# nv-tlabs/GEN3C

Hardware: AMD Instinct MI355X
Metric: denoise-steps/sec (121x1280x704 latent, Cosmos-7B) (higher is better)
Workload: dtype bf16

## Files before the change

### gen3c_amd/_lib.py

```python
from __future__ import annotations

import ctypes as C
from pathlib import Path

_LIB_PATH = Path(__file__).resolve().parent / "lib" / "libgen3c_hip.so"
_lib = None

vp, i64, i32, f32 = C.c_void_p, C.c_int64, C.c_int, C.c_float

G3_OK, G3_ERR_ARG, G3_ERR_LAUNCH, G3_ERR_RESOURCE = 0, 1, 2, 3

SIGNATURES = {
    "g3_last_error": [],
    "g3_abi_version": [],
    "g3_set_option": [C.c_char_p, i32],
    "g3_device_info": [i32, C.POINTER(i32), C.POINTER(i32), C.c_char_p, i32],
    "g3_event_create": [C.POINTER(vp)],
    "g3_event_record": [vp, vp],
    "g3_event_elapsed_ms": [vp, vp, C.POINTER(f32)],
    "g3_event_destroy": [vp],
    "g3_gemm_bf16_nt": [vp, i64, vp, i64, vp, i64, i32, i32, i32, i32, vp, i32, i64, vp, i64, vp],
    "g3_flash_attn_fwd_kvseg_bf16": [vp, i64, i64, i64, vp, i64, i64, i64, vp, i64, i64, i64, i32, i64, vp, i64, i64, i64, i32, i32, i32,
                                     i32, i32, f32, vp],
    "g3_gemm_kernel_name": [i32, i32, i32, i32],
    "g3_quant_mxfp8_bf16": [vp, i64, vp, i64, vp, i64, i32, i32, vp],
    "g3_gemm_mxfp8_nt": [vp, i64, vp, i64, vp, i64, vp, i64, vp, i64, i32, i32, i32, i32, vp, i32, i64, vp, i64, vp],
    "g3_gemm_mxfp8_kernel_name": [i32, i32, i32, i32],
    "g3_gemv_bf16": [vp, i64, vp, i64, vp, i64, vp, i64, i32, i32, i32, i32, vp],
    "g3_flash_attn_kernel_name": [i32, i32, i32, i32],
    "g3_flash_attn_fwd_bf16": [vp, i64, i64, i64, vp, i64, i64, i64, vp, i64, i64, i64, vp, i64, i64, i64, i32, i32, i32,
                               i32, i32, f32, vp],
    "g3_cross_attn_fwd_bf16": [vp, i64, i64, i64, vp, f32, vp, i64, i64, i64, vp, i64, i64, i64, vp, i64, i64, i64, i32, i32, i32, i32, i32,
                               i32, f32, vp],
    "g3_flash_attn_fwd_ex_bf16": [vp, i64, i64, i64, vp, i64, i64, i64, vp, i64, i64, i64, i32, i64, vp, vp, vp, i64, i64, i64, i32, i32, i32,
                                  i32, i32, f32, i32, vp],
    "g3_flash_attn_fwd_carry_bf16": [vp, i64, i64, i64, vp, i64, i64, i64, vp, i64, i64, i64, i32, i64, i32, i32, vp, vp, vp, vp, vp, i64, i64,
                                     i64, i32, i32, i32, i32, i32, f32, i32, vp],
    "g3_flash_attn_kernel_name_ex": [i32, i32, i32, i32, i32],
    "g3_attn_merge_partials_bf16": [vp, vp, i32, i64, i64, i64, vp, i64, i64, i64, i32, i32, i32, i32, vp],
    "g3_transpose_v_bf16": [vp, i64, vp, i64, i32, i32, i32, i32, vp],
    "g3_layernorm_modulate_bf16": [vp, i64, vp, vp, i64, i32, vp, i64, i32, i32, f32, vp],
    "g3_posemb_layernorm_modulate_bf16": [vp, i64, vp, vp, vp, vp, i32, i32, i32, i32, vp, vp, i64, i32, vp, i64, i32, f32, vp],
    "g3_qk_rmsnorm_rope_bf16": [vp, i64, vp, vp, vp, vp, i64, i32, i32, i32, i32, f32, vp],
    "g3_qk_rmsnorm_rope_pair_bf16": [vp, i64, vp, i32, vp, i32, vp, vp, vp, i64, i32, i32, i32, f32, vp],
    "g3_gemm_qk_norm_rope_bf16": [vp, i64, vp, i64, vp, i64, i32, i32, i32, i32, i32, vp, vp, vp, vp, i32, f32, vp, i64, vp],
    "g3_add_inplace_bf16": [vp, vp, i64, vp],
    "g3_warp_project_f32": [vp, vp, vp, vp, vp, vp, vp, vp, vp, i32, i32, i32, i32, vp],
    "g3_warp_splat_f32": [vp, vp, vp, vp, vp, vp, i32, i32, i32, i32, vp],
    "g3_warp_resolve_f32": [vp, vp, vp, vp, i32, i32, i32, vp],
    "g3_warp_windows_workspace_bytes": [i32, i32, i32],
    "g3_warp_splat_resolve_f32": [vp, vp, vp, vp, vp, vp, vp, vp, vp, vp, i32, i32, i32, i32, vp],
    "g3_render_workspace_bytes": [i32, i32, i32, i32],
    "g3_render_workspace_init": [vp, i32, i32, i32, i32, vp],
    "g3_render_items_f32": [vp, vp, vp, vp, vp, vp, vp, vp, vp, vp, vp, vp, vp, i32, i32, i32, i32, i32, vp],
    "g3_mesh_occlusion_f32": [vp, vp, vp, vp, vp, vp, vp, vp, vp, vp, i32, i32, i32, i32, vp],
    "g3_unproject_points_f32": [vp, vp, vp, vp, i32, i32, i32, vp],
    "g3_dit_patchify_bf16": [vp, vp, vp, i32, vp, i32, i32, i32, i32, i32, i32, vp],
    "g3_dit_unpatchify_bf16": [vp, i64, vp, i32, i32, i32, i32, i32, i32, i32, vp],
    "g3_timestep_embedding_bf16": [vp, vp, vp, vp, i32, i32, vp],
    "g3_reliable_depth_mask_f32": [vp, vp, i32, i32, i32, i32, f32, f32, vp],
    "g3_align_depth_workspace_bytes": [i32, i32],
    "g3_align_depth_f32": [vp, vp, vp, vp, vp, i32, i32, f32, f32, vp, vp, C.c_size_t, i32, i32, vp],
    "g3_conv3d_cl_bf16": [vp, i64, vp, i64, vp, vp, i64, vp, i64] + [i32] * 17 + [vp],
    "g3_conv3d_cl_gnstats_bf16": [vp, i64, vp, i64, vp, vp, i64, vp, i64] + [i32] * 17 + [vp, i32, vp],
    "g3_groupnorm_stats_cl_bf16": [vp, i64, vp, i32, i32, i32, vp],
    "g3_groupnorm_apply_cl_bf16": [vp, i64, vp, vp, vp, vp, i64, i32, i32, i32, f32, i32, vp],
    "g3_groupnorm_swish_cl_bf16": [vp, i64, vp, vp, vp, vp, i64, i32, i32, i32, f32, i32, vp],
    "g3_haar3d_patch_bf16": [vp, vp, i32, i32, i32, vp],
    "g3_haar3d_unpatch_bf16": [vp, i64, vp, i32, i32, i32, vp],
    "g3_resample_cl_bf16": [vp, vp, i32, i32, i32, i32, i32, vp],
    "g3_softmax_rows_bf16": [vp, i64, i32, i32, f32, vp],
    "g3_transpose2d_bf16": [vp, i64, vp, i64, i32, i32, vp],
    "g3_temporal_attn_cl_bf16": [vp, vp, vp, vp, i32, i32, i32, f32, vp],
    "g3_spatial_attn_d512_bf16": [vp, vp, vp, i64, i64, vp, i32, i32, f32, vp],
    "g3_edm_prepare_input_bf16": [vp, vp, vp, vp, vp, vp, i64, i32, i32, f32, f32, f32, f32, vp],
    "g3_edm_cfg_euler_step_bf16": [vp, vp, vp, vp, vp, vp, i64, i32, i32, f32, f32, f32, f32, f32, f32, f32, vp],
}
_RESTYPES = {"g3_last_error": C.c_char_p, "g3_flash_attn_kernel_name": C.c_char_p, "g3_gemm_kernel_name": C.c_char_p, "g3_gemm_mxfp8_kernel_name": C.c_char_p, "g3_flash_attn_kernel_name_ex": C.c_char_p, "g3_align_depth_workspace_bytes": C.c_size_t,
             "g3_warp_windows_workspace_bytes": C.c_size_t, "g3_render_workspace_bytes": C.c_size_t}


class Gen3cHipError(RuntimeError):
    pass


def lib_path() -> Path:
    return _LIB_PATH


def load():
    global _lib
    if _lib is not None:
        return _lib
    import torch
    if not _LIB_PATH.exists():
        raise Gen3cHipError(
            f"{_LIB_PATH} is missing: build it with `python -m gen3c_amd.build` (or __graft_entry__.build()). "
            "gen3c_amd has no CPU/PyTorch fallback for its HIP kernels."
        )
    lib = C.CDLL(str(_LIB_PATH))
    for name, argtypes in SIGNATURES.items():
        fn = getattr(lib, name)
        fn.argtypes = argtypes
        fn.restype = _RESTYPES.get(name, C.c_int)
    _lib = lib
    return lib


def last_error() -> str:
    msg = load().g3_last_error()
    return msg.decode() if msg else "?"


def check(rc: int, what: str = ""):
    if rc != 0:
        msg = load().g3_last_error()
# ... 2 lines not shown
```

### gen3c_amd/csrc/api.hip

```cpp
#include "common.hpp"
#include <stdarg.h>
#include <stdio.h>
#include <stdlib.h>
#include <string.h>

namespace {
thread_local char g_err[512] = "";
}

int g3_set_error(int code, const char* fmt, ...) {
    va_list ap;
    va_start(ap, fmt);
    vsnprintf(g_err, sizeof(g_err), fmt, ap);
    va_end(ap);
    return code;
}

int g3_check_launch(const char* what) {
    hipError_t e = hipGetLastError();
    if (e != hipSuccess) return g3_set_error(G3_ERR_LAUNCH, "%s: launch failed: %s", what, hipGetErrorString(e));
    return G3_OK;
}

static int env_int(const char* name, int dflt) {
    const char* e = getenv(name);
    return (e && *e) ? atoi(e) : dflt;
}
int g3_opt_gemm_regstage = env_int("G3_GEMM_REGSTAGE", 0);
int g3_opt_attn_xcd_heads = env_int("G3_ATTN_XCD_HEADS", 1);
int g3_opt_attn_variant = env_int("G3_ATTN_VARIANT", 0);
int g3_opt_gemm_rowmajor_tiles = env_int("G3_GEMM_ROWMAJOR_TILES", 0);
int g3_opt_gemm_wide_store = env_int("G3_GEMM_WIDE_STORE", 1);
int g3_opt_splat_tiled = env_int("G3_SPLAT_TILED", 1);
int g3_opt_render_overlap = env_int("G3_RENDER_OVERLAP", 1);
int g3_opt_render_exclusive = env_int("G3_RENDER_EXCLUSIVE", 0);
int g3_opt_render_full_extent = env_int("G3_RENDER_FULL_EXTENT", 1);
int g3_opt_render_fused = env_int("G3_RENDER_FUSED", 1);
int g3_opt_gemm_pingpong = env_int("G3_GEMM_PINGPONG", 3);
int g3_opt_tok_tattn_px = env_int("G3_TOK_TATTN_PX", 1);
int g3_opt_gemm_persistent = env_int("G3_GEMM_PERSISTENT", 0);
int g3_opt_gemm_deferred = env_int("G3_GEMM_DEFERRED", 1);
int g3_opt_gemm_deferred_grid = env_int("G3_GEMM_DEFERRED_GRID", 0);
int g3_opt_gemm_tokens_first = env_int("G3_GEMM_TOKENS_FIRST", 2);
int g3_opt_conv_w4 = env_int("G3_CONV_W4", 1);
int g3_opt_ln_wave_rows = env_int("G3_LN_WAVE_ROWS", 0);
int g3_opt_norm_octets = env_int("G3_NORM_OCTETS", 1);
int g3_opt_gemm_unpinned = env_int("G3_GEMM_UNPINNED", 1);

extern "C" int g3_set_option(const char* name, int value) {
    if (!name) return g3_set_error(G3_ERR_ARG, "g3_set_option: null name");
    if (!strcmp(name, "gemm_regstage")) { g3_opt_gemm_regstage = value; return G3_OK; }
    if (!strcmp(name, "gemm_wide_store")) { g3_opt_gemm_wide_store = value; return G3_OK; }
    if (!strcmp(name, "splat_tiled")) { g3_opt_splat_tiled = value; return G3_OK; }
    if (!strcmp(name, "render_overlap")) { g3_opt_render_overlap = value; return G3_OK; }
    if (!strcmp(name, "render_fused")) { g3_opt_render_fused = value; return G3_OK; }
    if (!strcmp(name, "render_exclusive")) { g3_opt_render_exclusive = value; return G3_OK; }
    if (!strcmp(name, "render_full_extent")) { g3_opt_render_full_extent = value; return G3_OK; }
    if (!strcmp(name, "gemm_pingpong")) { g3_opt_gemm_pingpong = value; return G3_OK; }
    if (!strcmp(name, "gemm_unpinned")) { g3_opt_gemm_unpinned = value; return G3_OK; }
    if (!strcmp(name, "conv_w4")) { g3_opt_conv_w4 = value; return G3_OK; }
    if (!strcmp(name, "gemm_persistent")) { g3_opt_gemm_persistent = value; return G3_OK; }
    if (!strcmp(name, "gemm_deferred")) { g3_opt_gemm_deferred = value; return G3_OK; }
    if (!strcmp(name, "gemm_tokens_first")) { g3_opt_gemm_tokens_first = value; return G3_OK; }
    if (!strcmp(name, "gemm_deferred_grid")) { g3_opt_gemm_deferred_grid = value; return G3_OK; }
    if (!strcmp(name, "tok_tattn_px")) { g3_opt_tok_tattn_px = value; return G3_OK; }
    if (!strcmp(name, "gemm_rowmajor_tiles")) { g3_opt_gemm_rowmajor_tiles = value; return G3_OK; }
    if (!strcmp(name, "ln_wave_rows")) { g3_opt_ln_wave_rows = value; return G3_OK; }
    if (!strcmp(name, "norm_octets")) { g3_opt_norm_octets = value; return G3_OK; }
    if (!strcmp(name, "attn_variant")) { g3_opt_attn_variant = value; return G3_OK; }
    if (!strcmp(name, "attn_xcd_heads")) { g3_opt_attn_xcd_heads = value; return G3_OK; }
    return g3_set_error(G3_ERR_ARG, "g3_set_option: unknown option %s", name);
}

extern "C" const char* g3_last_error(void) { return g_err; }
extern "C" int g3_abi_version(void) { return 1; }

extern "C" int g3_device_info(int device, int* cu_count, int* is_gfx950, char* arch_name, int arch_name_len) {
    hipDeviceProp_t prop;
    hipError_t e = hipGetDeviceProperties(&prop, device);
    if (e != hipSuccess) return g3_set_error(G3_ERR_LAUNCH, "g3_device_info: %s", hipGetErrorString(e));
    if (cu_count) *cu_count = prop.multiProcessorCount;
    if (is_gfx950) *is_gfx950 = (strncmp(prop.gcnArchName, "gfx950", 6) == 0) ? 1 : 0;
    if (arch_name && arch_name_len > 0) snprintf(arch_name, arch_name_len, "%s", prop.gcnArchName);
    return G3_OK;
}

extern "C" int g3_event_create(void** ev) {
    hipEvent_t e;
    hipError_t r = hipEventCreate(&e);
    if (r != hipSuccess) return g3_set_error(G3_ERR_LAUNCH, "g3_event_create: %s", hipGetErrorString(r));
    *ev = (void*)e;
    return G3_OK;
}
extern "C" int g3_event_record(void* ev, void* stream) {
    hipError_t r = hipEventRecord((hipEvent_t)ev, (hipStream_t)stream);
    if (r != hipSuccess) return g3_set_error(G3_ERR_LAUNCH, "g3_event_record: %s", hipGetErrorString(r));
    return G3_OK;
}
extern "C" int g3_event_elapsed_ms(void* start, void* stop, float* ms) {
    hipError_t r = hipEventSynchronize((hipEvent_t)stop);
    if (r == hipSuccess) r = hipEventElapsedTime(ms, (hipEvent_t)start, (hipEvent_t)stop);
    if (r != hipSuccess) return g3_set_error(G3_ERR_LAUNCH, "g3_event_elapsed_ms: %s", hipGetErrorString(r));
    return G3_OK;
}
extern "C" int g3_event_destroy(void* ev) {
    (void)hipEventDestroy((hipEvent_t)ev);
    return G3_OK;
}
```

### gen3c_amd/csrc/attention.hip

```cpp
#include "common.hpp"
#include <stdlib.h>
#include <mutex>
#include <type_traits>

namespace {

constexpr int HD = 128;
constexpr int QB = 32;
constexpr int NWAVES = 8;
constexpr int BQ = QB * NWAVES;
constexpr int KVB = 64;
constexpr int NTHREADS = 64 * NWAVES;

struct AttnParams {
    const bf16_t* Q; int64_t q_row, q_batch, q_head;
    const bf16_t* K; int64_t k_row, k_batch, k_head;
    const bf16_t* Vt; int64_t vt_row, vt_batch, vt_head;
    bf16_t* O; int64_t o_row, o_batch, o_head;
    int Sq, Skv;
    float scale_log2;
    int vt_seg_len;
    int64_t vt_seg_stride;
    int grid_q, n_hb, n_heads, xcd_heads;
    float* O32;
    float* LSE;
    int kv_dense;
    const bf16_t* q_norm_w;
    float q_norm_eps;
    const float* carry_o;
    const float* carry_lse;
    int kv_skip_begin, kv_skip_len;
    uint32_t kv_skip_vt_bytes;
};

G3_DEVICE int k_off(int row, int chunk) { return row * HD + ((chunk ^ (row & 15)) << 3); }
G3_DEVICE int v_off(int row, int chunk) { return row * KVB + ((chunk ^ ((row >> 1) & 7)) << 3); }
G3_DEVICE int swap23(int i) { return (i & ~12) | ((i & 4) << 1) | ((i & 8) >> 1); }

template <int CTX>
__global__ __launch_bounds__(NTHREADS, 2) void flash_attn_fwd_kernel(AttnParams p) {
    extern __shared__ __attribute__((aligned(16))) char smem_raw[];
    bf16_t* sK = reinterpret_cast<bf16_t*>(smem_raw);
    bf16_t* sV = sK + 2 * KVB * HD;

    const int tid = threadIdx.x;
    const int lane = tid & 63;
    const int wave = tid >> 6;
    const int l31 = lane & 31;
    const int g = lane >> 5;
    const int head = blockIdx.y;
    const int batch = blockIdx.z;

    const bf16_t* Qb = p.Q + batch * p.q_batch + head * p.q_head;
    const bf16_t* Kb = p.K + batch * p.k_batch + head * p.k_head;
    const bf16_t* Vb = p.Vt + batch * p.vt_batch + head * p.vt_head;
    bf16_t* Ob = p.O + batch * p.o_batch + head * p.o_head;

    const int q_idx = blockIdx.x * BQ + wave * QB + l31;
    const bool q_ok = q_idx < p.Sq;
    bf16x8 qf[8];
    {
        const bf16_t* qrow = Qb + (int64_t)(q_ok ? q_idx : 0) * p.q_row + 8 * g;
#pragma unroll
        for (int ks = 0; ks < 8; ++ks) qf[ks] = q_ok ? load_bf16x8(qrow + 16 * ks) : zero_bf16x8();
    }

    bf16x8 rk[2], rv[2];
    auto stage_load = [&](int kv0) {
#pragma unroll
        for (int i = 0; i < 2; ++i) {
            const int idx = tid + NTHREADS * i;
            {
                const int row = idx >> 4, chunk = idx & 15;
                const bool ok = (kv0 + row) < p.Skv;
                rk[i] = ok ? load_bf16x8(Kb + (int64_t)(kv0 + row) * p.k_row + chunk * 8) : zero_bf16x8();
            }
            {
                const int row = idx >> 3, chunk = idx & 7;
                const bool ok = (kv0 + chunk * 8) < p.Skv;
                rv[i] = ok ? load_bf16x8(Vb + (int64_t)row * p.vt_row + kv0 + chunk * 8) : zero_bf16x8();
            }
        }
    };
    auto stage_write = [&](int buf) {
        bf16_t* dK = sK + buf * KVB * HD;
        bf16_t* dV = sV + buf * HD * KVB;
#pragma unroll
        for (int i = 0; i < 2; ++i) {
            const int idx = tid + NTHREADS * i;
            store_bf16x8(dK + k_off(idx >> 4, idx & 15), rk[i]);
            store_bf16x8(dV + v_off(idx >> 3, idx & 7), rv[i]);
        }
    };

    f32x16 accO[4];
#pragma unroll
    for (int d = 0; d < 4; ++d)
#pragma unroll
        for (int r = 0; r < 16; ++r) accO[d][r] = 0.f;
    float m_run = -1e30f;
    float l_run = 0.f;

    const int krow_perm = swap23(l31);
    const int nt = (p.Skv + KVB - 1) / KVB;
    stage_load(0);
    stage_write(0);
    __syncthreads();

    for (int t = 0; t < nt; ++t) {
        const int buf = t & 1;
        const int kv0 = t * KVB;
// ... 19 lines not shown
            for (int mb = 0; mb < 2; ++mb)
#pragma unroll
                for (int r = 0; r < 16; ++r) {
                    const int kv = kv0 + 32 * mb + 16 * (r >> 3) + 8 * g + (r & 7);
                    if (kv >= p.Skv) accS[mb][r] = -INFINITY;
                }
        }

        float mx = accS[0][0];
#pragma unroll
        for (int r = 1; r < 16; ++r) mx = fmaxf(mx, accS[0][r]);
#pragma unroll
        for (int r = 0; r < 16; ++r) mx = fmaxf(mx, accS[1][r]);
        mx = fmaxf(mx, wave_xor_f32(mx, 32));
        const float m_new = fmaxf(m_run, mx * p.scale_log2);
        const float alpha = __builtin_amdgcn_exp2f(m_run - m_new);
        m_run = m_new;

        float psum = 0.f;
        bf16x8 pb[4];
#pragma unroll
        for (int mb = 0; mb < 2; ++mb)
#pragma unroll
            for (int r = 0; r < 16; ++r) {
                const float pv = __builtin_amdgcn_exp2f(__builtin_fmaf(accS[mb][r], p.scale_log2, -m_new));
                psum += pv;
                pb[2 * mb + (r >> 3)][r & 7] = f32_to_bf16(pv);
            }
        l_run = l_run * alpha + psum;
#pragma unroll
        for (int d = 0; d < 4; ++d)
#pragma unroll
            for (int r = 0; r < 16; ++r) accO[d][r] *= alpha;

#pragma unroll
        for (int s = 0; s < 4; ++s) {
#pragma unroll
            for (int d = 0; d < 4; ++d) {
                const bf16x8 vf = load_bf16x8(cV + v_off(32 * d + l31, 2 * s + g));
                accO[d] = __builtin_amdgcn_mfma_f32_32x32x16_bf16(vf, pb[s], accO[d], 0, 0, 0);
            }
        }

        if (t + 1 < nt) stage_write(buf ^ 1);
        __syncthreads();
    }

    const float l_tot = l_run + wave_xor_f32(l_run, 32);
    const float inv = 1.0f / l_tot;
    if (q_ok) {
        bf16_t* orow = Ob + (int64_t)q_idx * p.o_row;
#pragma unroll
        for (int d = 0; d < 4; ++d)
#pragma unroll
            for (int q4 = 0; q4 < 4; ++q4) {
                bf16x4 o;
#pragma unroll
                for (int e = 0; e < 4; ++e) o[e] = f32_to_bf16(accO[d][4 * q4 + e] * inv);
                *reinterpret_cast<bf16x4*>(orow + 32 * d + 8 * q4 + 4 * g) = o;
            }
    }
}


constexpr float RESCALE_THR = 8.0f;

G3_DEVICE float max3(float a, float b, float c) {
    float r;
    asm("v_max3_f32 %0, %1, %2, %3" : "=v"(r) : "v"(a), "v"(b), "v"(c));
    return r;
}
G3_DEVICE void swap_halves(float& a, float& b) {
    asm volatile("s_nop 1\n\tv_permlane32_swap_b32 %0, %1" : "+v"(a), "+v"(b));
}
G3_DEVICE float xor32_max(float x) {
    float a = x, b = x;
    swap_halves(a, b);
    return max3(a, b, b);
}
G3_DEVICE float xor32_sum(float x) {
    float a = x, b = x;
    swap_halves(a, b);
    return a + b;
}

template <int CTX>
__global__ __launch_bounds__(NTHREADS, 2) void flash_attn_fwd_v2_kernel(AttnParams p) {
    extern __shared__ __attribute__((aligned(16))) char smem_raw[];
    bf16_t* sK = reinterpret_cast<bf16_t*>(smem_raw);
    bf16_t* sV = sK + 2 * KVB * HD;

    const int tid = threadIdx.x;
    const int lane = tid & 63;
    const int wave = tid >> 6;
    const int l31 = lane & 31;
    const int g = lane >> 5;
    const int head = blockIdx.y;
    const int batch = blockIdx.z;

    const bf16_t* Qb = p.Q + batch * p.q_batch + head * p.q_head;
    const bf16_t* Kb = p.K + batch * p.k_batch + head * p.k_head;
    const bf16_t* Vb = p.Vt + batch * p.vt_batch + head * p.vt_head;
    bf16_t* Ob = p.O + batch * p.o_batch + head * p.o_head;

    const int q_idx = blockIdx.x * BQ + wave * QB + l31;
    const bool q_ok = q_idx < p.Sq;
    bf16x8 qf[8];
    {
        const bf16_t* qrow = Qb + (int64_t)(q_ok ? q_idx : 0) * p.q_row + 8 * g;
#pragma unroll
        for (int ks = 0; ks < 8; ++ks) qf[ks] = q_ok ? load_bf16x8(qrow + 16 * ks) : zero_bf16x8();
    }

    bf16x8 rk[2], rv[2];
    auto load_k = [&](int kv0) {
#pragma unroll
        for (int i = 0; i < 2; ++i) {
            const int idx = tid + NTHREADS * i;
            const int row = idx >> 4, chunk = idx & 15;
            rk[i] = (kv0 + row) < p.Skv ? load_bf16x8(Kb + (int64_t)(kv0 + row) * p.k_row + chunk * 8) : zero_bf16x8();
        }
    };
    auto load_v = [&](int kv0) {
#pragma unroll
        for (int i = 0; i < 2; ++i) {
            const int idx = tid + NTHREADS * i;
            const int row = idx >> 3, chunk = idx & 7;
            rv[i] = (kv0 + chunk * 8) < p.Skv ? load_bf16x8(Vb + (int64_t)row * p.vt_row + kv0 + chunk * 8) : zero_bf16x8();
        }
    };
    auto write_k = [&](int buf) {
        bf16_t* dK = sK + buf * KVB * HD;
#pragma unroll
        for (int i = 0; i < 2; ++i) {
            const int idx = tid + NTHREADS * i;
            store_bf16x8(dK + k_off(idx >> 4, idx & 15), rk[i]);
        }
    };
    auto write_v = [&](int buf) {
        bf16_t* dV = sV + buf * HD * KVB;
#pragma unroll
        for (int i = 0; i < 2; ++i) {
            const int idx = tid + NTHREADS * i;
            store_bf16x8(dV + v_off(idx >> 3, idx & 7), rv[i]);
        }
    };

    const int krow_perm = swap23(l31);
    int koff[8], voff[4];
#pragma unroll
    for (int ks = 0; ks < 8; ++ks) koff[ks] = k_off(krow_perm, 2 * ks + g);
#pragma unroll
    for (int s4 = 0; s4 < 4; ++s4) voff[s4] = v_off(l31, 2 * s4 + g);
    auto qk = [&](f32x16 (&S)[2], int kbuf) {
        const bf16_t* cK = sK + kbuf * KVB * HD;
#pragma unroll
        for (int mb = 0; mb < 2; ++mb) {
#pragma unroll
            for (int r = 0; r < 16; ++r) S[mb][r] = 0.f;
#pragma unroll
            for (int ks = 0; ks < 8; ++ks) {
                const bf16x8 kf = load_bf16x8(cK + 32 * mb * HD + koff[ks]);
                S[mb] = __builtin_amdgcn_mfma_f32_32x32x16_bf16(kf, qf[ks], S[mb], 0, 0, 0);
            }
        }
    };
// ... 87 lines not shown
            write_v(par ^ 1);
            __syncthreads();
        }
    };

    using True = std::integral_constant<bool, true>;
    using False = std::integral_constant<bool, false>;
    using P0 = std::integral_constant<int, 0>;
    using P1 = std::integral_constant<int, 1>;
    int t = 0;
    for (; t + 2 < nt; t += 2) {
        tile(SA, SB, t, True{}, P0{});
        tile(SB, SA, t + 1, True{}, P1{});
    }
    if (t + 1 < nt) {
        tile(SA, SB, t, True{}, P0{});
        tile(SB, SA, t + 1, False{}, P1{});
    } else {
        tile(SA, SB, t, False{}, P0{});
    }

    const float l_tot = xor32_sum(l_run);
    const float inv = 1.0f / l_tot;
    if (q_ok) {
        bf16_t* orow = Ob + (int64_t)q_idx * p.o_row;
#pragma unroll
        for (int d = 0; d < 4; ++d)
#pragma unroll
            for (int q4 = 0; q4 < 4; ++q4) {
                bf16x4 o;
#pragma unroll
                for (int e = 0; e < 4; ++e) o[e] = f32_to_bf16(accO[d][4 * q4 + e] * inv);
                *reinterpret_cast<bf16x4*>(orow + 32 * d + 8 * q4 + 4 * g) = o;
            }
    }
}


template <int OFF> G3_DEVICE void lds_read_frag(bf16x8& dst, uint32_t addr) {
    static_assert(OFF >= 0 && OFF < 65536, "ds_read offset field is 16 bits");
    asm volatile("ds_read_b128 %0, %1 offset:%2" : "=v"(dst) : "v"(addr), "n"(OFF));
}
G3_DEVICE uint32_t lds_addr_flip128(uint32_t a) {
    uint32_t r;
    asm volatile("v_xor_b32 %0, 0x80, %1" : "=v"(r) : "v"(a));
    return r;
}
template <int N> G3_DEVICE void lds_wait_frag(bf16x8& frag) { asm volatile("s_waitcnt lgkmcnt(%1)" : "+v"(frag) : "n"(N)); }

#define G3_SGB(mask, n) __builtin_amdgcn_sched_group_barrier((mask), (n), 0)
constexpr int SGB_VALU = 0x2, SGB_MFMA = 0x8, SGB_DSR = 0x100, SGB_TRANS = 0x400;

#ifndef G3_AB_ATTN_ABLATE
#define G3_AB_ATTN_ABLATE 0
#endif
template <int CTX, int QA, int QBV, bool FOLD, bool MW = false, int MW_RD = 4, int MW_KREGS = 8>
__global__ __launch_bounds__(NTHREADS, 2) void flash_attn_fwd_v3_kernel(AttnParams p) {
    constexpr bool CP = (CTX & 2) != 0;
    extern __shared__ __attribute__((aligned(16))) char smem_raw[];
    bf16_t* sK = reinterpret_cast<bf16_t*>(smem_raw);
    bf16_t* sV = sK + 2 * KVB * HD;

    const int tid = threadIdx.x;
    const int lane = tid & 63;
    const int wave = tid >> 6;
    const int l31 = lane & 31;
    const int g = lane >> 5;
    const int Skv = p.kv_dense > 0 ? p.kv_dense : p.Skv;
    const int head = blockIdx.y;
    const int batch = blockIdx.z;

    const bf16_t* Qb = p.Q + batch * p.q_batch + head * p.q_head;
    const bf16_t* Kb = p.K + batch * p.k_batch + head * p.k_head;
    const bf16_t* Vb = p.Vt + batch * p.vt_batch + head * p.vt_head;
    bf16_t* Ob = p.O + batch * p.o_batch + head * p.o_head;

    const int q_idx = blockIdx.x * BQ + wave * QB + l31;
    const bool q_ok = q_idx < p.Sq;
    bf16x8 qf[8];
    {
        const bf16_t* qrow = Qb + (int64_t)(q_ok ? q_idx : 0) * p.q_row + 8 * g;
#pragma unroll
        for (int ks = 0; ks < 8; ++ks) qf[ks] = q_ok ? load_bf16x8(qrow + 16 * ks) : zero_bf16x8();
        if (p.q_norm_w) {
            float ss = 0.f;
#pragma unroll
            for (int ks = 0; ks < 8; ++ks)
#pragma unroll
                for (int e = 0; e < 8; ++e) { const float f = (float)qf[ks][e]; ss += f * f; }
            ss = xor32_sum(ss);
            const float rinv = rsqrtf(ss * (1.0f / 128.0f) + p.q_norm_eps);
#pragma unroll
            for (int ks = 0; ks < 8; ++ks) {
                const bf16x8 w8 = load_bf16x8(p.q_norm_w + 16 * ks + 8 * g);
#pragma unroll
                for (int e = 0; e < 8; ++e) qf[ks][e] = f32_to_bf16((float)qf[ks][e] * rinv * (float)w8[e]);
            }
        }
        if (FOLD) {
#pragma unroll
            for (int ks = 0; ks < 8; ++ks)
#pragma unroll
                for (int e = 0; e < 8; ++e) qf[ks][e] = f32_to_bf16((float)qf[ks][e] * p.scale_log2);
        }
    }

    const int k_row0 = tid >> 4, k_src_chunk = (tid & 15) ^ (k_row0 & 15);
    const int v_row0 = tid >> 3, v_src_chunk = (tid & 7) ^ ((v_row0 >> 1) & 7);
    const char* Kbytes = reinterpret_cast<const char*>(Kb);
    const char* Vbytes = reinterpret_cast<const char*>(Vb);
    const uint32_t k_row_bytes = (uint32_t)p.k_row * 2u;
    const uint32_t k_lane = (uint32_t)k_row0 * k_row_bytes + (uint32_t)k_src_chunk * 16u;
    const uint32_t v_lane0 = (uint32_t)v_row0 * (uint32_t)p.vt_row * 2u + (uint32_t)v_src_chunk * 16u;
    const uint32_t v_lane1 = v_lane0 + 64u * (uint32_t)p.vt_row * 2u;
    auto kv_phys = [&](int kv) -> int {
        if constexpr (CP) return kv + (kv >= p.kv_skip_begin ? p.kv_skip_len : 0);
        else return kv;
    };
    const uint32_t k_last = (uint32_t)kv_phys(Skv - 1) * k_row_bytes + (uint32_t)k_src_chunk * 16u;
    auto dma_k = [&](int kv0, int slot) {
        bf16_t* d = sK + slot * KVB * HD + wave * 64 * 8;
        kv0 = kv_phys(kv0);
        uint32_t o0 = k_lane + (uint32_t)kv0 * k_row_bytes;
        uint32_t o1 = o0 + 32u * k_row_bytes;
        o0 = min(o0, k_last | 0u);
        o1 = min(o1, k_last | 0u);
        __builtin_amdgcn_global_load_lds((const __attribute__((address_space(1))) void*)(Kbytes + o0),
                                         (__attribute__((address_space(3))) void*)d, 16, 0, 0);
        __builtin_amdgcn_global_load_lds((const __attribute__((address_space(1))) void*)(Kbytes + o1),
                                         (__attribute__((address_space(3))) void*)(d + 512 * 8), 16, 0, 0);
    };
    const uint32_t seg_len = (uint32_t)p.vt_seg_len, seg_bytes = (uint32_t)p.vt_seg_stride * 2u;
    auto dma_v = [&](int kv0, int slot) {
        bf16_t* d = sV + slot * HD * KVB + wave * 64 * 8;
        kv0 = kv_phys(kv0);
        uint32_t tile_off = (uint32_t)kv0 * 2u;
        if (seg_len) {
            const uint32_t sg = (uint32_t)kv0 / seg_len;
            tile_off = sg * seg_bytes + ((uint32_t)kv0 - sg * seg_len) * 2u;
        }
        const uint32_t o0 = v_lane0 + tile_off, o1 = v_lane1 + tile_off;
        __builtin_amdgcn_global_load_lds((const __attribute__((address_space(1))) void*)(Vbytes + o0),
                                         (__attribute__((address_space(3))) void*)d, 16, 0, 0);
        __builtin_amdgcn_global_load_lds((const __attribute__((address_space(1))) void*)(Vbytes + o1),
                                         (__attribute__((address_space(3))) void*)(d + 512 * 8), 16, 0, 0);
    };

    const int krow_perm = swap23(l31);
    int koff[8], voff[4];
#pragma unroll
    for (int ks = 0; ks < 8; ++ks) koff[ks] = k_off(krow_perm, 2 * ks + g);
#pragma unroll
    for (int s4 = 0; s4 < 4; ++s4) voff[s4] = v_off(l31, 2 * s4 + g);
    const uint32_t lds_k0 = (uint32_t)(uintptr_t)(__attribute__((address_space(3))) bf16_t*)sK;
    const uint32_t lds_v0 = (uint32_t)(uintptr_t)(__attribute__((address_space(3))) bf16_t*)sV;
    uint32_t kaddr[8], vaddr[4];
    if (MW && MW_KREGS < 8 && (lds_k0 & 255u)) __builtin_trap();
#pragma unroll
    for (int ks = 0; ks < 8; ++ks) kaddr[ks] = lds_k0 + 2u * (uint32_t)koff[ks];
#pragma unroll
    for (int s4 = 0; s4 < 4; ++s4) vaddr[s4] = lds_v0 + 2u * (uint32_t)voff[s4];

    f32x16 accO[4];
#pragma unroll
    for (int d = 0; d < 4; ++d)
#pragma unroll
        for (int r = 0; r < 16; ++r) accO[d][r] = 0.f;
    float m_run = -1e30f;
    float l_run = 0.f;
    const float c = p.scale_log2;
    const int nt = (Skv + KVB - 1) / KVB;

    auto row_max = [&](const f32x16 (&S)[2]) -> float {
        if (G3_AB_ATTN_ABLATE & 4) return 0.f;
        float ma = max3(S[0][0], S[0][1], S[0][2]);
        float mb2 = max3(S[1][0], S[1][1], S[1][2]);
#pragma unroll
        for (int r = 3; r < 15; r += 2) {
            ma = max3(ma, S[0][r], S[0][r + 1]);
            mb2 = max3(mb2, S[1][r], S[1][r + 1]);
        }
        return xor32_max(max3(ma, mb2, max3(S[0][15], S[1][15], S[1][15]))) * (FOLD ? 1.0f : c);
    };
    auto mask_tail = [&](f32x16 (&S)[2], int kv0) {
#pragma unroll
        for (int mb = 0; mb < 2; ++mb)
#pragma unroll
            for (int r = 0; r < 16; ++r) {
                const int kv = kv0 + 32 * mb + 16 * (r >> 3) + 8 * g + (r & 7);
                if (kv >= Skv) S[mb][r] = -INFINITY;
            }
    };

    G3_JITTER(wave, blockIdx.x + 5);
    dma_k(0, 0);
    dma_v(0, 0);
    if (nt > 1) dma_k(KVB, 1);
    lds_dma_publish_barrier();
    G3_JITTER(wave + 2, blockIdx.x);
    f32x16 SA[2], SB[2];
    {
        const bf16_t* cK = sK;
#pragma unroll
        for (int mb = 0; mb < 2; ++mb) {
#pragma unroll
            for (int r = 0; r < 16; ++r) SA[mb][r] = 0.f;
#pragma unroll
            for (int ks = 0; ks < 8; ++ks)
                SA[mb] = __builtin_amdgcn_mfma_f32_32x32x16_bf16(load_bf16x8(cK + 32 * mb * HD + koff[ks]), qf[ks], SA[mb], 0, 0, 0);
        }
    }
    G3_JITTER(wave + 1, blockIdx.x);
#ifndef G3_AB_OMIT_PROLOGUE_BARRIER
    __syncthreads();
#endif
    if (nt == 1 && KVB > Skv) mask_tail(SA, 0);
    float mx_cur = row_max(SA);
    f32x16 negm;
    if (FOLD) {
        m_run = mx_cur;
#pragma unroll
        for (int mb = 0; mb < 2; ++mb)
#pragma unroll
            for (int r = 0; r < 16; ++r) SA[mb][r] -= m_run;
#pragma unroll
        for (int r = 0; r < 16; ++r) negm[r] = -m_run;
        mx_cur = 0.f;
    }
#ifndef G3_AB_NO_ATTN_SETPRIO
    if (__builtin_amdgcn_readfirstlane(threadIdx.x) >= 256) __builtin_amdgcn_s_setprio(1);
#endif

    auto tile = [&](f32x16 (&S_cur)[2], f32x16 (&S_next)[2], int t, auto has_next_c, auto par_c) {
        constexpr bool has_next = decltype(has_next_c)::value;
        constexpr int par = decltype(par_c)::value;
        const int kv0 = t * KVB;
        G3_JITTER(wave + blockIdx.x, t);
        if (!has_next && kv0 + KVB > Skv) {
            mask_tail(S_cur, kv0);
            mx_cur = row_max(S_cur);
        }
        if (has_next) {
            if (t + 2 < nt) dma_k(kv0 + 2 * KVB, par);
            dma_v(kv0 + KVB, par ^ 1);
        }
        if (FOLD) {
            if (__any(mx_cur > RESCALE_THR)) {
                const float delta = fmaxf(mx_cur, 0.f);
                const float alpha = __builtin_amdgcn_exp2f(-delta);
                m_run += delta;
                l_run *= alpha;
#pragma unroll
                for (int d = 0; d < 4; ++d)
#pragma unroll
                    for (int r = 0; r < 16; ++r) accO[d][r] *= alpha;
#pragma unroll
                for (int mb = 0; mb < 2; ++mb)
#pragma unroll
                    for (int r = 0; r < 16; ++r) S_cur[mb][r] -= delta;
#pragma unroll
                for (int r = 0; r < 16; ++r) negm[r] = -m_run;
            }
        } else if (__any(mx_cur - m_run > RESCALE_THR)) {
            const float m_new = fmaxf(m_run, mx_cur);
            const float alpha = __builtin_amdgcn_exp2f(m_run - m_new);
            m_run = m_new;
            l_run *= alpha;
#pragma unroll
            for (int d = 0; d < 4; ++d)
#pragma unroll
                for (int r = 0; r < 16; ++r) accO[d][r] *= alpha;
        }
        const float neg_m = -m_run;
        float psum[4] = {0.f, 0.f, 0.f, 0.f};
        bf16x8 pb[4];
        auto softmax_slice = [&](int sl) {
            const int mb = sl >> 1, r0 = (sl & 1) * 8;
#pragma unroll
            for (int j = 0; j < 8; ++j) {
                const float sv = FOLD ? S_cur[mb][r0 + j] : __builtin_fmaf(S_cur[mb][r0 + j], c, neg_m);
// ... 89 lines not shown
                G3_SGB(SGB_TRANS, 1);
            }
            l_run += (psum[0] + psum[1]) + (psum[2] + psum[3]);
            mx_cur = mx_next;
        } else {
            const bf16_t* cV = sV + par * HD * KVB;
            bf16x8 vf[4];
#pragma unroll
            for (int i = 0; i < 3; ++i) vf[i] = load_bf16x8(cV + 32 * (i & 3) * KVB + voff[i >> 2]);
            if (G3_AB_ATTN_ABLATE & 8) vf[3] = vf[0];
            softmax_slice(2);
            float mx_next = 0.f;
#pragma unroll
            for (int i = 0; i < 16; ++i) {
                if (i + 3 < 16 && !(G3_AB_ATTN_ABLATE & 8)) vf[(i + 3) & 3] = load_bf16x8(cV + 32 * ((i + 3) & 3) * KVB + voff[(i + 3) >> 2]);
                accO[i & 3] = __builtin_amdgcn_mfma_f32_32x32x16_bf16(vf[i & 3], pb[i >> 2], accO[i & 3], 0, 0, 0);
                if (i == 3) softmax_slice(3);
                if (has_next && i == 7) mx_next = row_max(S_next);
            }
            G3_SGB(SGB_DSR, 3);
#pragma unroll
            for (int i = 0; i < 16; ++i) {
                G3_SGB(SGB_MFMA, 1);
                if (i + 3 < 16) G3_SGB(SGB_DSR, 1);
                G3_SGB(SGB_VALU, QBV);
                G3_SGB(SGB_TRANS, 1);
            }
            l_run += (psum[0] + psum[1]) + (psum[2] + psum[3]);
            mx_cur = mx_next;
        }
        if (has_next) lds_dma_publish_barrier();
    };

    using True = std::integral_constant<bool, true>;
    using False = std::integral_constant<bool, false>;
    using P0 = std::integral_constant<int, 0>;
    using P1 = std::integral_constant<int, 1>;
    int t = 0;
    for (; t + 2 < nt; t += 2) {
        tile(SA, SB, t, True{}, P0{});
        tile(SB, SA, t + 1, True{}, P1{});
    }
    if (t + 1 < nt) {
        tile(SA, SB, t, True{}, P0{});
        tile(SB, SA, t + 1, False{}, P1{});
    } else {
        tile(SA, SB, t, False{}, P0{});
    }

    float l_tot = xor32_sum(l_run);
    float o_scale = 1.0f;
    if (p.kv_dense > 0 && p.kv_dense < p.Skv) {
        const float m_new = fmaxf(m_run, 0.f);
        o_scale = __builtin_amdgcn_exp2f(m_run - m_new);
        l_tot = l_tot * o_scale + (float)(p.Skv - p.kv_dense) * __builtin_amdgcn_exp2f(-m_new);
        m_run = m_new;
    }
    const float inv = o_scale / l_tot;
    if constexpr (CP) {
        const int q_ld = q_ok ? q_idx : p.Sq - 1;
        const int64_t li = ((int64_t)blockIdx.z * p.n_heads + blockIdx.y) * p.Sq + q_ld;
        const int64_t o_hb = (int64_t)blockIdx.z * p.o_batch + (int64_t)blockIdx.y * p.o_head;
        const float lse_k = m_run + __builtin_amdgcn_logf(l_tot);
        f32x4 oc[4][4];
        float lse_c = -INFINITY;
        if (p.carry_lse) {
            const float* crow = p.carry_o + o_hb + (int64_t)q_ld * p.o_row + 4 * g;
#pragma unroll
            for (int d = 0; d < 4; ++d)
#pragma unroll
                for (int q4 = 0; q4 < 4; ++q4) oc[d][q4] = *reinterpret_cast<const f32x4*>(crow + 32 * d + 8 * q4);
            lse_c = p.carry_lse[li];
        } else {
#pragma unroll
            for (int d = 0; d < 4; ++d)
#pragma unroll
                for (int q4 = 0; q4 < 4; ++q4) oc[d][q4] = f32x4{0.f, 0.f, 0.f, 0.f};
        }
        const float mm = fmaxf(lse_c, lse_k);
        const float wc = __builtin_amdgcn_exp2f(lse_c - mm), wk = __builtin_amdgcn_exp2f(lse_k - mm);
        const float rs = 1.0f / (wc + wk);
        const float fc = wc * rs, fk = (wk * rs) * inv;
        const bool use_c = fc > 0.f;
        if (q_ok) {
            const int64_t ro = o_hb + (int64_t)q_idx * p.o_row;
#pragma unroll
            for (int d = 0; d < 4; ++d)
#pragma unroll
                for (int q4 = 0; q4 < 4; ++q4) {
                    const int64_t off = ro + 32 * d + 8 * q4 + 4 * g;
                    f32x4 o;
#pragma unroll
                    for (int e = 0; e < 4; ++e) o[e] = (use_c ? fc * oc[d][q4][e] : 0.f) + fk * accO[d][4 * q4 + e];
                    if (p.O32) {
                        *reinterpret_cast<f32x4*>(p.O32 + off) = o;
                    } else {
                        bf16x4 ob;
#pragma unroll
                        for (int e = 0; e < 4; ++e) ob[e] = f32_to_bf16(o[e]);
                        *reinterpret_cast<bf16x4*>(p.O + off) = ob;
                    }
                }
            if (p.O32 && g == 0) p.LSE[li] = mm + __builtin_amdgcn_logf(wc + wk);
        }
        return;
    }
    if (p.O32) {
        if (q_ok) {
            float* orow = p.O32 + (int64_t)blockIdx.z * p.o_batch + (int64_t)blockIdx.y * p.o_head + (int64_t)q_idx * p.o_row;
#pragma unroll
            for (int d = 0; d < 4; ++d)
#pragma unroll
                for (int q4 = 0; q4 < 4; ++q4) {
                    f32x4 o;
#pragma unroll
                    for (int e = 0; e < 4; ++e) o[e] = accO[d][4 * q4 + e] * inv;
                    *reinterpret_cast<f32x4*>(orow + 32 * d + 8 * q4 + 4 * g) = o;
                }
            if (g == 0) p.LSE[((int64_t)blockIdx.z * p.n_heads + blockIdx.y) * p.Sq + q_idx] = m_run + __builtin_amdgcn_logf(l_tot);
        }
        return;
    }
    if (q_ok) {
        bf16_t* orow = Ob + (int64_t)q_idx * p.o_row;
#pragma unroll
        for (int d = 0; d < 4; ++d)
#pragma unroll
            for (int q4 = 0; q4 < 4; ++q4) {
                bf16x4 o;
#pragma unroll
                for (int e = 0; e < 4; ++e) o[e] = f32_to_bf16(accO[d][4 * q4 + e] * inv);
                *reinterpret_cast<bf16x4*>(orow + 32 * d + 8 * q4 + 4 * g) = o;
            }
    }
}



#include "attention_w4.hpp"
#define W4B_CP 0
#include "attention_w4b.hpp"
#undef W4B_CP
#define W4B_CP 1
#include "attention_w4b.hpp"
#undef W4B_CP

}

static int attn_resolve_variant(int Sq, int Skv, int B, int H, int requested = 0) {
    int variant = requested ? requested : g3_opt_attn_variant;
    if (variant == 0) {
        const long n_wg = (long)((Sq + 255) / 256) * H * B;
        const long rounds = (n_wg + 255) / 256;
        const bool even_fill = n_wg * 100 >= rounds * 256 * 93;
        variant = (Skv > 2048 && (Skv % KVB) == 0 && even_fill) ? 11 : 4;
    }
    if ((variant == 10 || variant == 11) && (Skv % KVB)) variant = 9;
    return variant;
}

extern "C" const char* g3_flash_attn_kernel_name_ex(int Sq, int Skv, int B, int H, int variant_req) {
    const bool long_ctx = Skv > 2048;
    switch (attn_resolve_variant(Sq, Skv, B, H, variant_req)) {
        case 1: return long_ctx ? "flash_attn_fwd_kernel<0>" : "flash_attn_fwd_kernel<1>";
        case 2: return long_ctx ? "flash_attn_fwd_v2_kernel<0>" : "flash_attn_fwd_v2_kernel<1>";
        case 3: return long_ctx ? "flash_attn_fwd_v3_kernel<0, 6, 8, false>" : "flash_attn_fwd_v3_kernel<1, 6, 8, false>";
        case 5: return long_ctx ? "flash_attn_fwd_v3_kernel<0, 6, 8, true>" : "flash_attn_fwd_v3_kernel<1, 6, 8, true>";
        case 6: return long_ctx ? "flash_attn_fwd_v3_kernel<0, 6, 8, true, true, 4, 4>" : "flash_attn_fwd_v3_kernel<1, 6, 8, false, true>";
        case 7: return long_ctx ? "flash_attn_fwd_v3_kernel<0, 6, 8, true, true, 4, 4>" : "flash_attn_fwd_v3_kernel<1, 6, 8, true, true, 4, 4>";
        case 8: return long_ctx ? "flash_attn_fwd_v3_kernel<0, 6, 8, false, true>" : "flash_attn_fwd_v3_kernel<1, 6, 8, false, true>";
        case 9: return long_ctx ? "flash_attn_fwd_w4_kernel<0>" : "flash_attn_fwd_w4_kernel<1>";
        case 10: return "flash_attn_fwd_w4b_kernel<false>";
        case 11: return "flash_attn_fwd_w4b_kernel<true>";
        default: return long_ctx ? "flash_attn_fwd_v3_kernel<0, 6, 8, true>" : "flash_attn_fwd_v3_kernel<1, 6, 8, false>";
    }
}

extern "C" const char* g3_flash_attn_kernel_name(int Sq, int Skv, int B, int H) { return g3_flash_attn_kernel_name_ex(Sq, Skv, B, H, 0); }

static int flash_attn_launch(const void* q, int64_t q_row, int64_t q_batch, int64_t q_head, const void* k, int64_t k_row, int64_t k_batch,
                             int64_t k_head, const void* vt, int64_t vt_row, int64_t vt_batch, int64_t vt_head, int vt_seg_len,
                             int64_t vt_seg_stride, void* o, int64_t o_row, int64_t o_batch, int64_t o_head, int Sq, int Skv, int B, int H,
                             int head_dim, float softmax_scale, void* stream, int variant_req = 0, float* o_partial = nullptr, float* lse = nullptr, int kv_dense = 0,
                             const void* q_norm_w = nullptr, float q_norm_eps = 0.f, bool cp_form = false, const float* carry_o = nullptr,
                             const float* carry_lse = nullptr, int kv_skip_begin = 0, int kv_skip_len = 0, uint32_t kv_skip_vt_bytes = 0) {
    if (!q || !k || !vt || (!o && !o_partial)) return g3_set_error(G3_ERR_ARG, "g3_flash_attn_fwd_bf16: null operand");
    if ((o_partial != nullptr) != (lse != nullptr)) return g3_set_error(G3_ERR_ARG, "g3_flash_attn_fwd_ex_bf16: o_partial and lse go together");
    if (o_partial && (((uintptr_t)o_partial & 15) || ((uintptr_t)lse & 3))) return g3_set_error(G3_ERR_ARG, "g3_flash_attn_fwd_ex_bf16: misaligned o_partial / lse");
    if (head_dim != HD) return g3_set_error(G3_ERR_ARG, "g3_flash_attn_fwd_bf16: head_dim %d unsupported (128 only)", head_dim);
    if (Sq <= 0 || Skv <= 0 || B <= 0 || H <= 0) return g3_set_error(G3_ERR_ARG, "g3_flash_attn_fwd_bf16: bad shape");
    if ((q_row & 7) || (k_row & 7) || (vt_row & 7) || (o_row & 3) || (q_batch & 7) || (k_batch & 7) || (vt_batch & 7) ||
        (q_head & 7) || (k_head & 7) || (vt_head & 7) || (o_batch & 3) || (o_head & 3))
        return g3_set_error(G3_ERR_ARG, "g3_flash_attn_fwd_bf16: strides must keep 16-byte (q,k,vt) / 8-byte (o) alignment");
    if ((((uintptr_t)q | (uintptr_t)k | (uintptr_t)vt) & 15) || ((uintptr_t)o & 7))
        return g3_set_error(G3_ERR_ARG, "g3_flash_attn_fwd_bf16: misaligned pointer");
    const int skv_phys = Skv + kv_skip_len;
    const int kv_span = vt_seg_len > 0 ? vt_seg_len : skv_phys;
    if (vt_seg_len < 0 || (vt_seg_len > 0 && ((vt_seg_len % KVB) || (skv_phys % vt_seg_len) || (vt_seg_stride & 7) || vt_seg_stride <= 0)))
        return g3_set_error(G3_ERR_ARG, "g3_flash_attn_fwd_kvseg_bf16: segments must be a multiple of 64 keys, tile S_kv exactly, 16-byte aligned stride");
    if (vt_row < ((kv_span + 7) & ~7)) return g3_set_error(G3_ERR_ARG, "g3_flash_attn_fwd_bf16: vt leading dim %lld < keys per row rounded to 8", (long long)vt_row);
    AttnParams p;
    p.Q = (const bf16_t*)q; p.q_row = q_row; p.q_batch = q_batch; p.q_head = q_head;
    p.K = (const bf16_t*)k; p.k_row = k_row; p.k_batch = k_batch; p.k_head = k_head;
    p.Vt = (const bf16_t*)vt; p.vt_row = vt_row; p.vt_batch = vt_batch; p.vt_head = vt_head;
    p.O = (bf16_t*)o; p.o_row = o_row; p.o_batch = o_batch; p.o_head = o_head;
    p.Sq = Sq; p.Skv = Skv;
    p.scale_log2 = softmax_scale * 1.4426950408889634f;
    p.vt_seg_len = vt_seg_len; p.vt_seg_stride = vt_seg_stride;
    p.grid_q = 0; p.n_hb = 0; p.n_heads = H; p.xcd_heads = 0;
    p.O32 = o_partial; p.LSE = lse;
    p.kv_dense = 0;
    if (kv_dense > 0) {
        const int kd = ((kv_dense + KVB - 1) / KVB) * KVB;
        if (kv_dense > Skv) return g3_set_error(G3_ERR_ARG, "g3_cross_attn_fwd_bf16: kv_dense %d > S_kv %d", kv_dense, Skv);
        if (kd < Skv) p.kv_dense = kd;
    }
    p.q_norm_w = (const bf16_t*)q_norm_w; p.q_norm_eps = q_norm_eps;
    p.carry_o = carry_o; p.carry_lse = carry_lse;
    p.kv_skip_begin = kv_skip_begin; p.kv_skip_len = kv_skip_len; p.kv_skip_vt_bytes = kv_skip_vt_bytes;
    if (q_norm_w && ((uintptr_t)q_norm_w & 15)) return g3_set_error(G3_ERR_ARG, "g3_cross_attn_fwd_bf16: misaligned q_norm_weight");
    const size_t smem = (size_t)2 * (KVB * HD + HD * KVB) * sizeof(bf16_t);
    static bool attr_set[64] = {};
    static std::mutex attr_mu;
    int variant = attn_resolve_variant(Sq, Skv, B, H, variant_req);
    if (cp_form && variant != 4 && variant != 11)
        return g3_set_error(G3_ERR_ARG, "g3_flash_attn_fwd_carry_bf16: the carry / key-skip form exists for the 8-wave (4) and one-wave-per-SIMD (11) kernels only "
                                        "(variant %d chosen; 11 needs S_kv %% 64 == 0)", variant);
    if (o_partial && variant == 9) variant = 4;
    if ((p.kv_dense || p.q_norm_w) && (variant < 3 || variant >= 9)) variant = 4;
    if (variant >= 3 && vt_row < ((kv_span + KVB - 1) / KVB) * KVB) variant = 2;
    if (variant >= 3) {
        const uint64_t k_max = (uint64_t)(skv_phys - 1 + 2 * KVB) * (uint64_t)k_row * 2u + 256u;
        const uint64_t n_seg = vt_seg_len > 0 ? (uint64_t)(skv_phys / vt_seg_len) : 1u;
        const uint64_t v_max = (uint64_t)(HD - 1) * (uint64_t)vt_row * 2u + (n_seg - 1) * (uint64_t)vt_seg_stride * 2u + ((uint64_t)kv_span + KVB) * 2u + 256u;
        if (k_max > 0xFFFFFFFFull || v_max > 0xFFFFFFFFull) {
            if (cp_form)
                return g3_set_error(G3_ERR_ARG, "g3_flash_attn_fwd_carry_bf16: K / V^T span (skipped keys included) exceeds the kernel's 32-bit byte offsets (k %llu, vt %llu bytes); "
                                                "the 64-bit-addressing kernel has no carry form", (unsigned long long)k_max, (unsigned long long)v_max);
            if (vt_seg_len > 0)
                return g3_set_error(G3_ERR_ARG, "g3_flash_attn_fwd_kvseg_bf16: K / V^T span exceeds the kernel's 32-bit byte offsets (k %llu, vt %llu bytes)",
                                    (unsigned long long)k_max, (unsigned long long)v_max);
            variant = 2;
        }
    }
    if (cp_form && variant < 3)
        return g3_set_error(G3_ERR_ARG, "g3_flash_attn_fwd_carry_bf16: V^T leading dimension %lld below ceil64 of the keys it spans forces the 64-bit-addressing kernel, which has "
                                        "no carry form", (long long)vt_row);
    if (vt_seg_len > 0 && variant < 3)
        return g3_set_error(G3_ERR_ARG, "g3_flash_attn_fwd_kvseg_bf16: segmented V^T is implemented by the default (v3) kernel only");
    if (o_partial && variant < 3)
        return g3_set_error(G3_ERR_ARG, "g3_flash_attn_fwd_ex_bf16: split-KV partial outputs are implemented by the v3 / w4b kernels only (variant %d chosen)", variant);
    if ((p.kv_dense || p.q_norm_w) && variant < 3)
        return g3_set_error(G3_ERR_ARG, "g3_cross_attn_fwd_bf16: the Q norm / zero-tail form is implemented by the v3 kernels only (variant %d chosen: V^T leading dimension below "
                                        "ceil64(S_kv), or operands beyond the kernel's 32-bit byte offsets)", variant);
    int dev_id = 0;
    if (hipGetDevice(&dev_id) != hipSuccess || dev_id < 0 || dev_id >= 64) return g3_set_error(G3_ERR_LAUNCH, "flash_attn: hipGetDevice failed");
    {
      std::lock_guard<std::mutex> attr_lock(attr_mu);
      if (!attr_set[dev_id]) {
        const void* fns[19] = {reinterpret_cast<const void*>(&flash_attn_fwd_w4b_carry_kernel<true>),
                               reinterpret_cast<const void*>(&flash_attn_fwd_v3_kernel<2, 6, 8, true>), reinterpret_cast<const void*>(&flash_attn_fwd_v3_kernel<3, 6, 8, false>),
                               reinterpret_cast<const void*>(&flash_attn_fwd_w4b_kernel<false>), reinterpret_cast<const void*>(&flash_attn_fwd_w4b_kernel<true>),
                               reinterpret_cast<const void*>(&flash_attn_fwd_kernel<0>), reinterpret_cast<const void*>(&flash_attn_fwd_kernel<1>),
                               reinterpret_cast<const void*>(&flash_attn_fwd_v2_kernel<0>), reinterpret_cast<const void*>(&flash_attn_fwd_v2_kernel<1>),
                               reinterpret_cast<const void*>(&flash_attn_fwd_v3_kernel<0, 6, 8, false>), reinterpret_cast<const void*>(&flash_attn_fwd_v3_kernel<1, 6, 8, false>),
                               reinterpret_cast<const void*>(&flash_attn_fwd_v3_kernel<0, 6, 8, true>), reinterpret_cast<const void*>(&flash_attn_fwd_v3_kernel<1, 6, 8, true>),
                               reinterpret_cast<const void*>(&flash_attn_fwd_v3_kernel<0, 6, 8, true, true, 4, 4>), reinterpret_cast<const void*>(&flash_attn_fwd_v3_kernel<1, 6, 8, true, true, 4, 4>),
                               reinterpret_cast<const void*>(&flash_attn_fwd_v3_kernel<0, 6, 8, false, true>), reinterpret_cast<const void*>(&flash_attn_fwd_v3_kernel<1, 6, 8, false, true>),
                               reinterpret_cast<const void*>(&flash_attn_fwd_w4_kernel<0>), reinterpret_cast<const void*>(&flash_attn_fwd_w4_kernel<1>)};
        for (int i = 0; i < 19; ++i) {
            hipError_t e = hipFuncSetAttribute(fns[i], hipFuncAttributeMaxDynamicSharedMemorySize, (int)smem);
            if (e != hipSuccess) return g3_set_error(G3_ERR_LAUNCH, "flash_attn: hipFuncSetAttribute: %s", hipGetErrorString(e));
        }
        attr_set[dev_id] = true;
      }
    }
    dim3 grid((Sq + BQ - 1) / BQ, H, B);
    const bool long_ctx = Skv > 2048;
    hipStream_t st = (hipStream_t)stream;
    if (variant == 10 || variant == 11) {
        dim3 grid4((Sq + W4_BQ - 1) / W4_BQ, H, B);
        p.grid_q = (int)grid4.x; p.n_hb = H * B; p.n_heads = H;
        p.xcd_heads = (g3_opt_attn_xcd_heads && (H * B) % 8 == 0) ? 1 : 0;
        if (p.xcd_heads) grid4 = dim3(grid4.x * H * B, 1, 1);
        if (cp_form) hipLaunchKernelGGL(flash_attn_fwd_w4b_carry_kernel<true>, grid4, dim3(W4_THREADS), smem, st, p);
        else if (variant == 11) hipLaunchKernelGGL(flash_attn_fwd_w4b_kernel<true>, grid4, dim3(W4_THREADS), smem, st, p);
        else hipLaunchKernelGGL(flash_attn_fwd_w4b_kernel<false>, grid4, dim3(W4_THREADS), smem, st, p);
        return g3_check_launch("g3_flash_attn_fwd_bf16");
    }
    if (variant == 9) {
        dim3 grid4((Sq + W4_BQ - 1) / W4_BQ, H, B);
        if (long_ctx) hipLaunchKernelGGL(flash_attn_fwd_w4_kernel<0>, grid4, dim3(W4_THREADS), smem, st, p);
        else hipLaunchKernelGGL(flash_attn_fwd_w4_kernel<1>, grid4, dim3(W4_THREADS), smem, st, p);
        return g3_check_launch("g3_flash_attn_fwd_bf16");
    }
#define G3_LAUNCH_ATTN(KERNEL0, KERNEL1) do { if (long_ctx) hipLaunchKernelGGL(KERNEL0, grid, dim3(NTHREADS), smem, st, p); else hipLaunchKernelGGL(KERNEL1, grid, dim3(NTHREADS), smem, st, p); } while (0)
    if (cp_form) G3_LAUNCH_ATTN((flash_attn_fwd_v3_kernel<2, 6, 8, true>), (flash_attn_fwd_v3_kernel<3, 6, 8, false>));
    else if (variant == 1) G3_LAUNCH_ATTN(flash_attn_fwd_kernel<0>, flash_attn_fwd_kernel<1>);
    else if (variant == 2) G3_LAUNCH_ATTN(flash_attn_fwd_v2_kernel<0>, flash_attn_fwd_v2_kernel<1>);
    else if (variant == 3) G3_LAUNCH_ATTN((flash_attn_fwd_v3_kernel<0, 6, 8, false>), (flash_attn_fwd_v3_kernel<1, 6, 8, false>));
    else if (variant == 5) G3_LAUNCH_ATTN((flash_attn_fwd_v3_kernel<0, 6, 8, true>), (flash_attn_fwd_v3_kernel<1, 6, 8, true>));
    else if (variant == 6) G3_LAUNCH_ATTN((flash_attn_fwd_v3_kernel<0, 6, 8, true, true, 4, 4>), (flash_attn_fwd_v3_kernel<1, 6, 8, false, true>));
    else if (variant == 7) G3_LAUNCH_ATTN((flash_attn_fwd_v3_kernel<0, 6, 8, true, true, 4, 4>), (flash_attn_fwd_v3_kernel<1, 6, 8, true, true, 4, 4>));
    else if (variant == 8) G3_LAUNCH_ATTN((flash_attn_fwd_v3_kernel<0, 6, 8, false, true>), (flash_attn_fwd_v3_kernel<1, 6, 8, false, true>));
    else G3_LAUNCH_ATTN((flash_attn_fwd_v3_kernel<0, 6, 8, true>), (flash_attn_fwd_v3_kernel<1, 6, 8, false>));
#undef G3_LAUNCH_ATTN
    return g3_check_launch("g3_flash_attn_fwd_bf16");
}

extern "C" int g3_flash_attn_fwd_bf16(const void* q, int64_t q_row, int64_t q_batch, int64_t q_head, const void* k,
                                      int64_t k_row, int64_t k_batch, int64_t k_head, const void* vt, int64_t vt_row,
                                      int64_t vt_batch, int64_t vt_head, void* o, int64_t o_row, int64_t o_batch,
                                      int64_t o_head, int Sq, int Skv, int B, int H, int head_dim, float softmax_scale,
                                      void* stream) {
    return flash_attn_launch(q, q_row, q_batch, q_head, k, k_row, k_batch, k_head, vt, vt_row, vt_batch, vt_head, 0, 0, o, o_row, o_batch, o_head,
                             Sq, Skv, B, H, head_dim, softmax_scale, stream);
}

extern "C" int g3_flash_attn_fwd_kvseg_bf16(const void* q, int64_t q_row, int64_t q_batch, int64_t q_head, const void* k, int64_t k_row,
                                            int64_t k_batch, int64_t k_head, const void* vt, int64_t vt_row, int64_t vt_batch,
                                            int64_t vt_head, int vt_seg_len, int64_t vt_seg_stride, void* o, int64_t o_row, int64_t o_batch,
                                            int64_t o_head, int Sq, int Skv, int B, int H, int head_dim, float softmax_scale, void* stream) {
    if (vt_seg_len <= 0) return g3_set_error(G3_ERR_ARG, "g3_flash_attn_fwd_kvseg_bf16: vt_seg_len must be positive");
    return flash_attn_launch(q, q_row, q_batch, q_head, k, k_row, k_batch, k_head, vt, vt_row, vt_batch, vt_head, vt_seg_len, vt_seg_stride, o, o_row,
                             o_batch, o_head, Sq, Skv, B, H, head_dim, softmax_scale, stream);
}

extern "C" int g3_cross_attn_fwd_bf16(const void* q, int64_t q_row, int64_t q_batch, int64_t q_head, const void* q_norm_weight, float q_norm_eps, const void* k,
                                      int64_t k_row, int64_t k_batch, int64_t k_head, const void* vt, int64_t vt_row, int64_t vt_batch, int64_t vt_head, void* o,
                                      int64_t o_row, int64_t o_batch, int64_t o_head, int Sq, int Skv, int kv_dense, int B, int H, int head_dim,
                                      float softmax_scale, void* stream) {
    if (kv_dense < 0) return g3_set_error(G3_ERR_ARG, "g3_cross_attn_fwd_bf16: kv_dense must be >= 0 (0 = every key through the loop)");
    return flash_attn_launch(q, q_row, q_batch, q_head, k, k_row, k_batch, k_head, vt, vt_row, vt_batch, vt_head, 0, 0, o, o_row, o_batch, o_head, Sq, Skv, B, H,
                             head_dim, softmax_scale, stream, 0, nullptr, nullptr, kv_dense, q_norm_weight, q_norm_eps);
}

extern "C" int g3_flash_attn_fwd_ex_bf16(const void* q, int64_t q_row, int64_t q_batch, int64_t q_head, const void* k, int64_t k_row,
                                         int64_t k_batch, int64_t k_head, const void* vt, int64_t vt_row, int64_t vt_batch, int64_t vt_head,
                                         int vt_seg_len, int64_t vt_seg_stride, void* o, float* o_partial, float* lse, int64_t o_row,
                                         int64_t o_batch, int64_t o_head, int Sq, int Skv, int B, int H, int head_dim, float softmax_scale,
                                         int variant, void* stream) {
    if (variant < 0 || variant > 11) return g3_set_error(G3_ERR_ARG, "g3_flash_attn_fwd_ex_bf16: variant %d out of range", variant);
    if (o && o_partial) return g3_set_error(G3_ERR_ARG, "g3_flash_attn_fwd_ex_bf16: pass either o (bf16 result) or o_partial + lse, not both");
    if (o_partial && ((o_row & 3) || (o_batch & 3) || (o_head & 3))) return g3_set_error(G3_ERR_ARG, "g3_flash_attn_fwd_ex_bf16: o_partial strides must be multiples of 4");
    return flash_attn_launch(q, q_row, q_batch, q_head, k, k_row, k_batch, k_head, vt, vt_row, vt_batch, vt_head, vt_seg_len, vt_seg_stride, o, o_row,
                             o_batch, o_head, Sq, Skv, B, H, head_dim, softmax_scale, stream, variant, o_partial, lse);
}

extern "C" int g3_flash_attn_fwd_carry_bf16(const void* q, int64_t q_row, int64_t q_batch, int64_t q_head, const void* k, int64_t k_row,
                                            int64_t k_batch, int64_t k_head, const void* vt, int64_t vt_row, int64_t vt_batch, int64_t vt_head,
                                            int vt_seg_len, int64_t vt_seg_stride, int kv_skip_begin, int kv_skip_len, const float* carry_o,
                                            const float* carry_lse, void* o, float* o_partial, float* lse, int64_t o_row, int64_t o_batch,
                                            int64_t o_head, int Sq, int Skv, int B, int H, int head_dim, float softmax_scale, int variant,
                                            void* stream) {
    const char* fn = "g3_flash_attn_fwd_carry_bf16";
    if (variant < 0 || variant > 11) return g3_set_error(G3_ERR_ARG, "%s: variant %d out of range", fn, variant);
    if (o && o_partial) return g3_set_error(G3_ERR_ARG, "%s: pass either o (bf16 result) or o_partial + lse, not both", fn);
    if (!q || !k || !vt || (!o && !o_partial)) return g3_set_error(G3_ERR_ARG, "%s: null operand", fn);
    if ((o_row & 3) || (o_batch & 3) || (o_head & 3)) return g3_set_error(G3_ERR_ARG, "%s: o / o_partial / carry_o strides must be multiples of 4", fn);
    if ((carry_o != nullptr) != (carry_lse != nullptr)) return g3_set_error(G3_ERR_ARG, "%s: carry_o and carry_lse go together", fn);
    if (carry_o && (((uintptr_t)carry_o & 15) || ((uintptr_t)carry_lse & 3))) return g3_set_error(G3_ERR_ARG, "%s: misaligned carry_o (16 B) / carry_lse (4 B)", fn);
    if (Skv <= 0) return g3_set_error(G3_ERR_ARG, "%s: bad shape", fn);
    if (kv_skip_begin < 0 || kv_skip_len < 0 || (kv_skip_begin % KVB) || (kv_skip_len % KVB) || kv_skip_begin > Skv)
        return g3_set_error(G3_ERR_ARG, "%s: kv_skip (begin %d, len %d) must be multiples of 64 with 0 <= begin <= S_kv %d", fn, kv_skip_begin, kv_skip_len, Skv);
    if (vt_seg_len > 0 && kv_skip_len > 0 && ((kv_skip_begin % vt_seg_len) || (kv_skip_len % vt_seg_len)))
        return g3_set_error(G3_ERR_ARG, "%s: kv_skip (begin %d, len %d) must cover whole V^T segments of %d keys", fn, kv_skip_begin, kv_skip_len, vt_seg_len);
    if ((int64_t)Skv + kv_skip_len > 0x7fffffff) return g3_set_error(G3_ERR_ARG, "%s: S_kv + kv_skip_len overflows", fn);
    const int64_t vt_jump = vt_seg_len > 0 ? (int64_t)(kv_skip_len / vt_seg_len) * vt_seg_stride : (int64_t)kv_skip_len;
    if (vt_seg_len > 0 && vt_seg_stride <= 0) return g3_set_error(G3_ERR_ARG, "%s: vt_seg_stride must be positive", fn);
    if (vt_seg_len == 0 && vt_row < ((int64_t)Skv + kv_skip_len + KVB - 1) / KVB * KVB)
        return g3_set_error(G3_ERR_ARG, "%s: V^T leading dim %lld below ceil64(S_kv + kv_skip_len) forces the 64-bit-addressing kernel, which has no carry form", fn,
                            (long long)vt_row);
    if (kv_skip_len > 0 && kv_skip_begin == 0) {
        k = (const bf16_t*)k + (int64_t)kv_skip_len * k_row;
        vt = (const bf16_t*)vt + vt_jump;
        kv_skip_len = 0;
    }
    if (kv_skip_begin == Skv) kv_skip_len = 0;
    if (kv_skip_len == 0) kv_skip_begin = 0;
    const int64_t vt_jump_bytes = (vt_seg_len > 0 ? (int64_t)(kv_skip_len / vt_seg_len) * vt_seg_stride : (int64_t)kv_skip_len) * 2;
    if (vt_jump_bytes > 0xFFFFFFFFll) return g3_set_error(G3_ERR_ARG, "%s: the skipped V^T range exceeds the kernel's 32-bit byte offsets", fn);
    return flash_attn_launch(q, q_row, q_batch, q_head, k, k_row, k_batch, k_head, vt, vt_row, vt_batch, vt_head, vt_seg_len, vt_seg_stride, o, o_row,
                             o_batch, o_head, Sq, Skv, B, H, head_dim, softmax_scale, stream, variant, o_partial, lse, 0, nullptr, 0.f, true, carry_o,
                             carry_lse, kv_skip_begin, kv_skip_len, (uint32_t)vt_jump_bytes);
}

namespace {
constexpr int MERGE_MAX_PARTS = 8;
struct MergeParams {
    const float* o[MERGE_MAX_PARTS];
    const float* lse[MERGE_MAX_PARTS];
    int n_parts;
    int64_t p_row, p_batch, p_head;
    bf16_t* out; int64_t o_row, o_batch, o_head;
    int Sq, B, H;
};
__global__ __launch_bounds__(256) void attn_merge_partials_kernel(MergeParams p) {
    const int64_t idx = (int64_t)blockIdx.x * 256 + threadIdx.x;
    const int c = (int)(idx & 15);
    int64_t r = idx >> 4;
    const int h = (int)(r % p.H); r /= p.H;
    const int b = (int)(r % p.B);
    const int64_t qi = r / p.B;
    if (qi >= p.Sq) return;
    const int64_t li = ((int64_t)b * p.H + h) * p.Sq + qi;
    float l[MERGE_MAX_PARTS], mx = -INFINITY;
#pragma unroll
    for (int i = 0; i < MERGE_MAX_PARTS; ++i)
        if (i < p.n_parts) { l[i] = p.lse[i][li]; mx = fmaxf(mx, l[i]); }
    float wsum = 0.f;
#pragma unroll
    for (int i = 0; i < MERGE_MAX_PARTS; ++i)
        if (i < p.n_parts) { l[i] = __builtin_amdgcn_exp2f(l[i] - mx); wsum += l[i]; }
    const float inv = 1.0f / wsum;
    float acc[8] = {0.f, 0.f, 0.f, 0.f, 0.f, 0.f, 0.f, 0.f};
    const int64_t poff = qi * p.p_row + (int64_t)b * p.p_batch + (int64_t)h * p.p_head + 8 * c;
#pragma unroll
// ... 36 lines not shown
```

### gen3c_amd/csrc/attention_w4b.hpp

```cpp

#ifndef G3_ATTENTION_W4B_HELPERS
#define G3_ATTENTION_W4B_HELPERS
#define W4B_RING_AGPRS "a192","a193","a194","a195","a196","a197","a198","a199","a200","a201","a202","a203","a204","a205","a206","a207","a208","a209","a210","a211","a212","a213","a214","a215","a216","a217","a218","a219","a220","a221","a222","a223","a224","a225","a226","a227","a228","a229","a230","a231","a232","a233","a234","a235","a236","a237","a238","a239","a240","a241","a242","a243","a244","a245","a246","a247","a248","a249","a250","a251","a252","a253","a254","a255"
#define W4B_OWNED W4_OWNED_AGPRS, W4B_RING_AGPRS
constexpr int W4B_RING0 = 192;
constexpr int W4B_D = 6;

#if G3_AB_ATTN_ABLATE & 32
#define W4B_READ ""
#else
#define W4B_READ "ds_read_b128 a[%c[ra]:%c[rb]], %[addr] offset:%c[off]\n\t"
#endif
#define W4B_QK(h) "v_mfma_f32_32x32x16_bf16 %[s" #h "], a[%c[fa]:%c[fb]], a[%c[q" #h "]:%c[e" #h "]], %[s" #h "]\n\t"
#define W4B_QK0(h) "v_mfma_f32_32x32x16_bf16 %[s" #h "], a[%c[fa]:%c[fb]], a[%c[q" #h "]:%c[e" #h "]], %[c" #h "]\n\t"
#define W4B_PV(h) "v_mfma_f32_32x32x16_bf16 a[%c[o" #h "]:%c[g" #h "]], a[%c[fa]:%c[fb]], %[pf" #h "], a[%c[o" #h "]:%c[g" #h "]]\n\t"
#if G3_AB_ATTN_ABLATE & 128
#define W4B_M0 ""
#define W4B_DMA ""
#else
#define W4B_M0 "s_mov_b32 m0, %[m0v]\n\t"
#define W4B_DMA "global_load_lds_dwordx4 %[voff], %[sbase]\n\t"
#endif
#if G3_AB_ATTN_ABLATE & 256
#define W4B_MAXP(k) ""
// ... 89 lines not shown
        static_assert(!READ && !UNIT && MX == 0, "w4b_step_pv: combination not laid out");
        asm volatile(W4_WAIT W4B_PV(0) W4B_PV(1) : : W4B_B_IN);
    }
#undef W4B_B_RD
#undef W4B_B_UO
#undef W4B_B_UI
#undef W4B_B_M0
}
template <int I, int WN, bool READ = false, int ROFF = 0>
G3_DEVICE void w4b_step_pv_fold(const u32x4& pf0, const u32x4& pf1, float& a0, float& b0, float& c0, float& d0, float& a1, float& b1, float& c1, float& d1, float& t0,
                                 float& t1, uint32_t addr = 0u) {
    constexpr int D = I & 3;
    constexpr int o0 = 16 * D, o1 = 16 * (4 + D);
    constexpr int fa = W4B_RING0 + 4 * ((16 + I) & 15), ra = W4B_RING0 + 4 * ((16 + I + W4B_D) & 15);
    if constexpr (READ && I == 14)
        asm volatile(W4B_READ W4_WAIT W4B_PV(0) "v_max3_f32 %[a0], %[a0], %[b0], %[c0]\n\tv_max3_f32 %[a1], %[a1], %[b1], %[c1]\n\tv_max_f32 %[a0], %[a0], %[d0]\n\tv_max_f32 %[a1], %[a1], %[d1]\n\t"
                     W4B_PV(1) "v_mov_b32 %[t0], %[a0]\n\tv_mov_b32 %[t1], %[a1]\n\t"
                     : [a0] "+v"(a0), [a1] "+v"(a1), [t0] "=&v"(t0), [t1] "=&v"(t1)
                     : W4B_B_IN, [b0] "v"(b0), [c0] "v"(c0), [d0] "v"(d0), [b1] "v"(b1), [c1] "v"(c1), [d1] "v"(d1), [addr] "v"(addr), [off] "n"(ROFF), [ra] "n"(ra), [rb] "n"(ra + 3));
    else if constexpr (READ)
        asm volatile(W4B_READ W4_WAIT W4B_PV(0) "v_permlane32_swap_b32 %[t0], %[a0]\n\tv_permlane32_swap_b32 %[t1], %[a1]\n\t" W4B_PV(1)
                     "v_max_f32 %[a0], %[a0], %[t0]\n\tv_max_f32 %[a1], %[a1], %[t1]\n\t"
                     : [a0] "+v"(a0), [a1] "+v"(a1), [t0] "+v"(t0), [t1] "+v"(t1) : W4B_B_IN, [addr] "v"(addr), [off] "n"(ROFF), [ra] "n"(ra), [rb] "n"(ra + 3));
    else if constexpr (I == 14)
        asm volatile(W4_WAIT W4B_PV(0) "v_max3_f32 %[a0], %[a0], %[b0], %[c0]\n\tv_max3_f32 %[a1], %[a1], %[b1], %[c1]\n\tv_max_f32 %[a0], %[a0], %[d0]\n\tv_max_f32 %[a1], %[a1], %[d1]\n\t"
                     W4B_PV(1) "v_mov_b32 %[t0], %[a0]\n\tv_mov_b32 %[t1], %[a1]\n\t"
                     : [a0] "+v"(a0), [a1] "+v"(a1), [t0] "=&v"(t0), [t1] "=&v"(t1)
                     : W4B_B_IN, [b0] "v"(b0), [c0] "v"(c0), [d0] "v"(d0), [b1] "v"(b1), [c1] "v"(c1), [d1] "v"(d1));
    else
        asm volatile(W4_WAIT W4B_PV(0) "v_permlane32_swap_b32 %[t0], %[a0]\n\tv_permlane32_swap_b32 %[t1], %[a1]\n\t" W4B_PV(1)
                     "v_max_f32 %[a0], %[a0], %[t0]\n\tv_max_f32 %[a1], %[a1], %[t1]\n\t"
                     : [a0] "+v"(a0), [a1] "+v"(a1), [t0] "+v"(t0), [t1] "+v"(t1) : W4B_B_IN);
}
#undef W4B_B_IN

G3_DEVICE void w4b_fence_acc() { asm volatile("s_nop 7\n\ts_nop 3" ::: W4B_OWNED); }
template <int R> G3_DEVICE void w4b_sub_inplace(f32x16& x, float d) {
    float t = x[R];
    asm volatile("v_sub_f32 %0, %0, %1" : "+v"(t) : "v"(d));
    x[R] = t;
}
template <int R> G3_DEVICE void w4b_set_inplace(f32x16& x, float v) {
    float t = x[R];
    asm volatile("v_mov_b32 %0, %1" : "+v"(t) : "v"(v));
    x[R] = t;
}
G3_DEVICE void w4b_mul_inplace(float& x, float a) { asm volatile("v_mul_f32 %0, %0, %1" : "+v"(x) : "v"(a)); }

#endif

#if W4B_CP
#define W4B_KERNEL flash_attn_fwd_w4b_carry_kernel
#else
#define W4B_KERNEL flash_attn_fwd_w4b_kernel
#endif
template <bool XB>
__global__ __launch_bounds__(W4_THREADS, 1) void W4B_KERNEL(AttnParams p) {
    constexpr bool CP = W4B_CP;
    extern __shared__ __attribute__((aligned(16))) char smem_raw[];
    bf16_t* sK = reinterpret_cast<bf16_t*>(smem_raw);
    bf16_t* sV = sK + 2 * KVB * HD;

    const int tid = threadIdx.x;
    const int lane = tid & 63;
    const int wave = __builtin_amdgcn_readfirstlane(tid >> 6);
    const int l31 = lane & 31;
    const int g = lane >> 5;
    int qblk = blockIdx.x, head = blockIdx.y, batch = blockIdx.z;
    if (p.xcd_heads) {
        const int xcd = blockIdx.x & 7, slot = blockIdx.x >> 3;
        const int hb = xcd + 8 * (slot / p.grid_q);
        qblk = slot - (slot / p.grid_q) * p.grid_q;
        head = hb % p.n_heads;
        batch = hb / p.n_heads;
    }

    const bf16_t* Qb = p.Q + batch * p.q_batch + head * p.q_head;
    const bf16_t* Kb = p.K + batch * p.k_batch + head * p.k_head;
    const bf16_t* Vb = p.Vt + batch * p.vt_batch + head * p.vt_head;
    bf16_t* Ob = p.O + batch * p.o_batch + head * p.o_head;
    float* o32_base = p.O32;
    float* lse_base = p.LSE;
    asm volatile("" : "+s"(o32_base), "+s"(lse_base));
    const float* carry_o = nullptr;
    const float* carry_lse = nullptr;
    uint32_t skip_t0 = 0u, skip_nt = 0u, v_skip = 0u;
    if constexpr (CP) {
        carry_o = p.carry_o;
        carry_lse = p.carry_lse;
        skip_t0 = (uint32_t)p.kv_skip_begin / KVB;
        skip_nt = (uint32_t)p.kv_skip_len / KVB;
        v_skip = p.kv_skip_vt_bytes;
        asm volatile("" : "+s"(carry_o), "+s"(carry_lse), "+s"(skip_t0), "+s"(skip_nt), "+s"(v_skip));
    }
    auto k_tile = [&](uint32_t t) -> uint32_t {
        if constexpr (CP) return t + (t >= skip_t0 ? skip_nt : 0u);
        else return t;
    };

    static_for<0, 16>([&](auto fc) {
        constexpr int f = decltype(fc)::value, h = f >> 3, ks = f & 7;
        const int q_idx = qblk * W4_BQ + wave * 64 + 32 * h + l31;
        const bool q_ok = q_idx < p.Sq;
        bf16x8 qv = q_ok ? load_bf16x8(Qb + (int64_t)q_idx * p.q_row + 8 * g + 16 * ks) : zero_bf16x8();
#pragma unroll
        for (int e = 0; e < 8; ++e) qv[e] = f32_to_bf16((float)qv[e] * p.scale_log2);
        const u32x4 qw = __builtin_bit_cast(u32x4, qv);
        w4_acc_write<W4_QBASE + 4 * f + 0>(qw[0]);
        w4_acc_write<W4_QBASE + 4 * f + 1>(qw[1]);
        w4_acc_write<W4_QBASE + 4 * f + 2>(qw[2]);
        w4_acc_write<W4_QBASE + 4 * f + 3>(qw[3]);
    });
    static_for<0, 128>([&](auto rc) { w4_acc_zero<decltype(rc)::value>(); });

    const int k_row0 = tid >> 4, k_src_chunk = (tid & 15) ^ (k_row0 & 15);
    const int v_row0 = tid >> 3, v_src_chunk = (tid & 7) ^ ((v_row0 >> 1) & 7);
    const char* Kbytes = reinterpret_cast<const char*>(Kb);
    const char* Vbytes = reinterpret_cast<const char*>(Vb);
    const uint32_t k_row_bytes = (uint32_t)p.k_row * 2u;
    const uint32_t v_row_bytes = (uint32_t)p.vt_row * 2u;
    uint32_t dma_off[8];
#pragma unroll
    for (int j = 0; j < 4; ++j) {
        dma_off[j] = ((uint32_t)k_row0 + 16u * j) * k_row_bytes + (uint32_t)k_src_chunk * 16u;
        dma_off[4 + j] = ((uint32_t)v_row0 + 32u * j) * v_row_bytes + (uint32_t)v_src_chunk * 16u;
    }
#pragma unroll
    for (int j = 0; j < 8; ++j) asm volatile("" : "+v"(dma_off[j]));
    const uint32_t k_tile_bytes = (uint32_t)KVB * k_row_bytes;
    const uint32_t seg_len = (uint32_t)p.vt_seg_len, seg_bytes = (uint32_t)p.vt_seg_stride * 2u;
    auto v_tile_off = [&](uint32_t kv0) -> uint32_t {
        if (!seg_len) return kv0 * 2u;
        const uint32_t sg = kv0 / seg_len;
        return sg * seg_bytes + (kv0 - sg * seg_len) * 2u;
    };
    auto dma_tile_builtin = [&](const char* base, const uint32_t* off, bf16_t* dst) {
#pragma unroll
        for (int i = 0; i < 4; ++i)
            __builtin_amdgcn_global_load_lds((const __attribute__((address_space(1))) void*)(base + off[i]),
                                             (__attribute__((address_space(3))) void*)(dst + wave * 64 * 8 + 256 * 8 * i), 16, 0, 0);
    };

    const int krow_perm = swap23(l31);
    const uint32_t lds_k0 = (uint32_t)(uintptr_t)(__attribute__((address_space(3))) bf16_t*)sK;
    const uint32_t lds_v0 = (uint32_t)(uintptr_t)(__attribute__((address_space(3))) bf16_t*)sV;
    uint32_t kaddr[8], vaddr[4];
#pragma unroll
    for (int ks = 0; ks < 8; ++ks) kaddr[ks] = lds_k0 + 2u * (uint32_t)k_off(krow_perm, 2 * ks + g);
#pragma unroll
    for (int s4 = 0; s4 < 4; ++s4) vaddr[s4] = lds_v0 + 2u * (uint32_t)v_off(l31, 2 * s4 + g);

    float m_run[2], mx_cur[2];
    float psum[2][4];
#pragma unroll
    for (int h = 0; h < 2; ++h)
#pragma unroll
        for (int k = 0; k < 4; ++k) psum[h][k] = 0.f;
    float ta[2] = {0.f, 0.f}, tb[2] = {0.f, 0.f};
    float pe[2][2] = {{0.f, 0.f}, {0.f, 0.f}};
    float xa[2], xb[2];
    const int nt = p.Skv / KVB;

    dma_tile_builtin(Kbytes, dma_off, sK);
    dma_tile_builtin(Vbytes, dma_off + 4, sV);
    if (nt > 1) dma_tile_builtin(Kbytes + k_tile(1u) * k_tile_bytes, dma_off, sK + KVB * HD);
    G3_JITTER(wave, blockIdx.x + 5);
    lds_dma_publish_barrier();
    G3_JITTER(wave + 2, blockIdx.x);
    f32x16 SA[2][2], SB[2][2];
    f32x16 negm[2];
    {
        f32x16 zero;
#pragma unroll
        for (int r = 0; r < 16; ++r) zero[r] = 0.f;
        static_for<0, 16>([&](auto ic) {
            constexpr int i = decltype(ic)::value, mb = i >> 3, ks = i & 7;
            const bf16x8 kf = load_bf16x8(sK + 32 * mb * HD + k_off(krow_perm, 2 * ks + g));
            if constexpr (ks == 0) {
                w4_qk0<0, -1>(SA[0][mb], kf, zero);
                w4_qk0<8, -1>(SA[1][mb], kf, zero);
            } else {
                w4_qk<ks, -1>(SA[0][mb], kf);
                w4_qk<8 + ks, -1>(SA[1][mb], kf);
            }
        });
    }
    w4_fence_v(SA[0][0], SA[0][1], SA[1][0], SA[1][1]);
    __syncthreads();
#pragma unroll
    for (int h = 0; h < 2; ++h) {
        float ma = max3(SA[h][0][0], SA[h][0][1], SA[h][0][2]);
        float mb2 = max3(SA[h][1][0], SA[h][1][1], SA[h][1][2]);
#pragma unroll
        for (int r = 3; r < 15; r += 2) {
            ma = max3(ma, SA[h][0][r], SA[h][0][r + 1]);
// ... 141 lines not shown
#define W4B_SN(mb, r) (has_next ? sn(H{}, std::integral_constant<int, mb>{}, std::integral_constant<int, (r)>{}) : 0.f)
                if constexpr (XB && has_next && I == 10) {
                    if (!(G3_AB_ATTN_ABLATE & 64)) asm volatile("s_waitcnt vmcnt(0)\n\ts_barrier" ::: "memory");
                }
                uint32_t k1 = 0;
                w4b_step_pv<I, rd_off(NR{}), rd, rd ? D : 15 - I, unit, mxk>(rd_addr(NR{}), pb[0][I >> 2], pb[1][I >> 2], ux(U{}), uy(U{}), k1, psum[hu][pa], psum[hu][pa + 1],
                                                                          cx[mh][I & 1], cy[mh][I & 1], W4B_SN(0, 2 * k0), W4B_SN(0, 2 * k0 + 1), W4B_SN(1, 2 * k0),
                                                                          W4B_SN(1, 2 * k0 + 1), W4B_SN(0, 2 * k1i), W4B_SN(0, 2 * k1i + 1), W4B_SN(1, 2 * k1i),
                                                                          W4B_SN(1, 2 * k1i + 1), W4B_SN(0, 2 * k2i), W4B_SN(0, 2 * k2i + 1), W4B_SN(1, 2 * k2i),
                                                                          W4B_SN(1, 2 * k2i + 1), ta[I & 1], tb[I & 1]);
#undef W4B_SN
                if constexpr (unit) uput(U{}, k1);
            });
            if constexpr (has_next) {
                if constexpr (XB) {
                    using N14 = std::integral_constant<int, 16 + 14 + D>;
                    using N15 = std::integral_constant<int, 16 + 15 + D>;
                    w4b_step_pv_fold<14, D, true, rd_off(N14{})>(pb[0][3], pb[1][3], cx[0][0], cy[0][0], cx[0][1], cy[0][1], cx[1][0], cy[1][0], cx[1][1], cy[1][1], tx[0], tx[1],
                                                                 rd_addr(N14{}));
                    w4b_step_pv_fold<15, D, true, rd_off(N15{})>(pb[0][3], pb[1][3], cx[0][0], cy[0][0], cx[0][1], cy[0][1], cx[1][0], cy[1][0], cx[1][1], cy[1][1], tx[0], tx[1],
                                                                 rd_addr(N15{}));
                } else {
                    w4b_step_pv_fold<14, 1>(pb[0][3], pb[1][3], cx[0][0], cy[0][0], cx[0][1], cy[0][1], cx[1][0], cy[1][0], cx[1][1], cy[1][1], tx[0], tx[1]);
                    w4b_step_pv_fold<15, 0>(pb[0][3], pb[1][3], cx[0][0], cy[0][0], cx[0][1], cy[0][1], cx[1][0], cy[1][0], cx[1][1], cy[1][1], tx[0], tx[1]);
                }
                mx_cur[0] = cx[0][0];
                mx_cur[1] = cx[1][0];
            } else {
                float d0 = 0.f, d1 = 0.f;
                uint32_t kd = 0;
                w4b_step_pv<14, 0, false, 1, false, 0>(0u, pb[0][3], pb[1][3], 0.f, 0.f, kd, d0, d1, d0, d1, 0, 0, 0, 0, 0, 0, 0, 0, 0, 0, 0, 0, d0, d1);
                w4b_step_pv<15, 0, false, 0, false, 0>(0u, pb[0][3], pb[1][3], 0.f, 0.f, kd, d0, d1, d0, d1, 0, 0, 0, 0, 0, 0, 0, 0, 0, 0, 0, 0, d0, d1);
            }
        }
        if (!XB && has_next && !(G3_AB_ATTN_ABLATE & 64)) lds_dma_publish_barrier();
    };

    using True = std::integral_constant<bool, true>;
    using False = std::integral_constant<bool, false>;
    using P0 = std::integral_constant<int, 0>;
    using P1 = std::integral_constant<int, 1>;
    int t = 0;
    for (; t + 2 < nt; t += 2) {
        tile(SA, SB, t, True{}, P0{});
        tile(SB, SA, t + 1, True{}, P1{});
    }
    if (t + 1 < nt) {
        tile(SA, SB, t, True{}, P0{});
        tile(SB, SA, t + 1, False{}, P1{});
    } else {
        tile(SA, SB, t, False{}, P0{});
    }

    w4b_fence_acc();
    static_for<0, 2>([&](auto hc) {
        constexpr int h = decltype(hc)::value;
        const float extra = (XB && h == 0) ? (pe[0][0] + pe[0][1]) + (pe[1][0] + pe[1][1]) : 0.f;
        const float inv = 1.0f / xor32_sum(((psum[h][0] + psum[h][1]) + (psum[h][2] + psum[h][3])) + extra);
        const int q_idx = qblk * W4_BQ + wave * 64 + 32 * h + l31;
        if constexpr (CP) {
            const bool q_ok = q_idx < p.Sq;
            const int q_ld = q_ok ? q_idx : p.Sq - 1;
            const int64_t li = ((int64_t)batch * p.n_heads + head) * p.Sq + q_ld;
            const int64_t ro = (int64_t)batch * p.o_batch + (int64_t)head * p.o_head + (int64_t)q_idx * p.o_row;
            const int64_t ro_ld = (int64_t)batch * p.o_batch + (int64_t)head * p.o_head + (int64_t)q_ld * p.o_row;
            const float lse_k = m_run[h] - __builtin_amdgcn_logf(inv);
            f32x4 oc[16];
            float lse_c = -INFINITY;
            if (carry_lse) {
                using gf32x4 = const __attribute__((address_space(1))) f32x4;
                gf32x4* crow = (gf32x4*)(carry_o + ro_ld + 4 * g);
#pragma unroll
                for (int c = 0; c < 16; ++c) oc[c] = crow[(32 * (c >> 2) + 8 * (c & 3)) / 4];
                lse_c = ((const __attribute__((address_space(1))) float*)carry_lse)[li];
            } else {
#pragma unroll
                for (int c = 0; c < 16; ++c) oc[c] = f32x4{0.f, 0.f, 0.f, 0.f};
            }
            const float mm = fmaxf(lse_c, lse_k);
            const float wc = __builtin_amdgcn_exp2f(lse_c - mm), wk = __builtin_amdgcn_exp2f(lse_k - mm);
            const float rs = 1.0f / (wc + wk);
            const float fc = wc * rs, fk = (wk * rs) * inv;
            const bool use_c = fc > 0.f;
            static_for<0, 16>([&](auto cc) {
                constexpr int c = decltype(cc)::value, d = c >> 2, q4 = c & 3;
                constexpr int R = 16 * (4 * h + d) + 4 * q4;
                const int64_t off = ro + 32 * d + 8 * q4 + 4 * g;
                float o[4];
                o[0] = (use_c ? fc * oc[c][0] : 0.f) + fk * w4_acc_read<R + 0>();
                o[1] = (use_c ? fc * oc[c][1] : 0.f) + fk * w4_acc_read<R + 1>();
                o[2] = (use_c ? fc * oc[c][2] : 0.f) + fk * w4_acc_read<R + 2>();
                o[3] = (use_c ? fc * oc[c][3] : 0.f) + fk * w4_acc_read<R + 3>();
                if (!q_ok) return;
                if (o32_base) {
                    *reinterpret_cast<f32x4*>(o32_base + off) = f32x4{o[0], o[1], o[2], o[3]};
                } else {
                    bf16x4 ob;
#pragma unroll
                    for (int e = 0; e < 4; ++e) ob[e] = f32_to_bf16(o[e]);
                    *reinterpret_cast<bf16x4*>(p.O + off) = ob;
                }
            });
            if (o32_base && g == 0 && q_ok) lse_base[li] = mm + __builtin_amdgcn_logf(wc + wk);
            return;
        }
        if (o32_base) {
            float* prow = o32_base + (int64_t)batch * p.o_batch + (int64_t)head * p.o_head + (int64_t)q_idx * p.o_row;
            static_for<0, 16>([&](auto cc) {
                constexpr int d = decltype(cc)::value >> 2, q4 = decltype(cc)::value & 3;
                constexpr int R = 16 * (4 * h + d) + 4 * q4;
                f32x4 o;
                o[0] = w4_acc_read<R + 0>() * inv;
                o[1] = w4_acc_read<R + 1>() * inv;
                o[2] = w4_acc_read<R + 2>() * inv;
                o[3] = w4_acc_read<R + 3>() * inv;
                if (q_idx < p.Sq) *reinterpret_cast<f32x4*>(prow + 32 * d + 8 * q4 + 4 * g) = o;
            });
            if (g == 0 && q_idx < p.Sq) lse_base[((int64_t)batch * p.n_heads + head) * p.Sq + q_idx] = m_run[h] - __builtin_amdgcn_logf(inv);
            return;
        }
        bf16_t* orow = Ob + (int64_t)q_idx * p.o_row;
        static_for<0, 16>([&](auto cc) {
            constexpr int d = decltype(cc)::value >> 2, q4 = decltype(cc)::value & 3;
            constexpr int R = 16 * (4 * h + d) + 4 * q4;
            bf16x4 o;
            o[0] = f32_to_bf16(w4_acc_read<R + 0>() * inv);
            o[1] = f32_to_bf16(w4_acc_read<R + 1>() * inv);
            o[2] = f32_to_bf16(w4_acc_read<R + 2>() * inv);
            o[3] = f32_to_bf16(w4_acc_read<R + 3>() * inv);
            if (q_idx < p.Sq) *reinterpret_cast<bf16x4*>(orow + 32 * d + 8 * q4 + 4 * g) = o;
        });
    });
}
#undef W4B_KERNEL
```

### gen3c_amd/csrc/common.hpp

```cpp
#pragma once
#include <type_traits>
#include <hip/hip_runtime.h>
#include <stdint.h>

typedef __bf16 bf16_t;
typedef __bf16 bf16x2 __attribute__((ext_vector_type(2)));
typedef __bf16 bf16x4 __attribute__((ext_vector_type(4)));
typedef __bf16 bf16x8 __attribute__((ext_vector_type(8)));
typedef float f32x2 __attribute__((ext_vector_type(2)));
typedef float f32x4 __attribute__((ext_vector_type(4)));
typedef float f32x16 __attribute__((ext_vector_type(16)));
typedef uint32_t u32x2 __attribute__((ext_vector_type(2)));
typedef uint32_t u32x4 __attribute__((ext_vector_type(4)));

#define G3_DEVICE __device__ __forceinline__

#define G3_OK 0
#define G3_ERR_ARG 1
#define G3_ERR_LAUNCH 2
#define G3_ERR_RESOURCE 3

int g3_set_error(int code, const char* fmt, ...);
int g3_check_launch(const char* what);

extern int g3_opt_gemm_regstage;
extern int g3_opt_gemm_rowmajor_tiles;
extern int g3_opt_gemm_unpinned;
extern int g3_opt_tok_tattn_px;
extern int g3_opt_gemm_persistent;
extern int g3_opt_gemm_deferred;
extern int g3_opt_gemm_deferred_grid;
extern int g3_opt_gemm_tokens_first;
extern int g3_opt_conv_w4;
extern int g3_opt_gemm_pingpong;
extern int g3_opt_gemm_wide_store;
extern int g3_opt_render_exclusive;
extern int g3_opt_render_full_extent;
extern int g3_opt_render_fused;
extern int g3_opt_render_overlap;
extern int g3_opt_splat_tiled;
extern int g3_opt_attn_xcd_heads;
extern int g3_opt_ln_wave_rows;
extern int g3_opt_norm_octets;
extern int g3_opt_attn_variant;

G3_DEVICE float bf16_to_f32(bf16_t v) { return (float)v; }
G3_DEVICE bf16_t f32_to_bf16(float v) { return (bf16_t)v; }

G3_DEVICE bf16x8 load_bf16x8(const bf16_t* p) { return *reinterpret_cast<const bf16x8*>(p); }
G3_DEVICE void store_bf16x8(bf16_t* p, bf16x8 v) { *reinterpret_cast<bf16x8*>(p) = v; }
G3_DEVICE bf16x8 zero_bf16x8() {
    u32x4 z = {0u, 0u, 0u, 0u};
    return __builtin_bit_cast(bf16x8, z);
}

G3_DEVICE float wave_xor_f32(float v, int mask) { return __shfl_xor(v, mask, 64); }

G3_DEVICE float gelu_erf(float x) { return 0.5f * x * (1.0f + erff(x * 0.70710678118654752440f)); }
G3_DEVICE float gelu_erf_fast(float x) {
    const float ax = fabsf(x);
    const float t = __builtin_amdgcn_rcpf(__builtin_fmaf(0.3275911f * 0.70710678118654752440f, ax, 1.0f));
    float poly = __builtin_fmaf(0.5f * 1.061405429f, t, 0.5f * -1.453152027f);
    poly = __builtin_fmaf(poly, t, 0.5f * 1.421413741f);
    poly = __builtin_fmaf(poly, t, 0.5f * -0.284496736f);
    poly = __builtin_fmaf(poly, t, 0.5f * 0.254829592f);
    const float ex = __builtin_amdgcn_exp2f((x * x) * (-0.5f * 1.44269504088896340736f));
    const float a = ((poly * t) * ex) * ax;
    return fmaxf(x, 0.0f) - a;
}
template <int I, int N, class F> G3_DEVICE void static_for(F&& f) {
    if constexpr (I < N) {
        f(std::integral_constant<int, I>{});
        static_for<I + 1, N>(f);
    }
}

#ifdef G3_AB_JITTER
#define G3_JITTER(a, b) do { if (((((int)(a)) * 7 + ((int)(b)) * 3) & 15) == 5) __builtin_amdgcn_s_sleep(G3_AB_JITTER); } while (0)
#else
#define G3_JITTER(a, b) ((void)0)
#endif

G3_DEVICE void lds_dma_publish_barrier() {
    asm volatile("s_waitcnt vmcnt(0)" ::: "memory");
    __syncthreads();
}
G3_DEVICE float silu(float x) { return x / (1.0f + __expf(-x)); }
```

### gen3c_amd/csrc/norm_rope.hip

```cpp
#include "common.hpp"

namespace {

constexpr int LN_THREADS = 256;
constexpr int LN_MAX_CHUNKS = 4;

struct PosEmbArgs {
    const bf16_t* pe_t; const bf16_t* pe_h; const bf16_t* pe_w; const bf16_t* norm;
    int Hp, Wp, B;
};

template <int POS>
__global__ __launch_bounds__(LN_THREADS) void ln_modulate_kernel(bf16_t* __restrict__ x, int64_t ldx,
                                                                 const bf16_t* __restrict__ shift,
                                                                 const bf16_t* __restrict__ scale, int64_t ldmod,
                                                                 int mod_rows, bf16_t* __restrict__ out, int64_t ldo,
                                                                 int rows, int D, float eps, PosEmbArgs pe) {
    __shared__ float red[2][LN_THREADS / 64];
    const int row = blockIdx.x;
    if (row >= rows) return;
    const int tid = threadIdx.x;
    const int nchunk = D >> 3;
    bf16_t* xr = x + (int64_t)row * ldx;
    const bf16_t *pt = nullptr, *ph = nullptr, *pw = nullptr;
// ... 212 lines not shown
        rmsnorm_rope_head<false>(a, b, wa, wb, t, eps, oa, ob);
    }
    bf16_t* dst = out + row * ld_out + head * 128;
    store_bf16x8(dst + sl * 8, oa);
    store_bf16x8(dst + 64 + sl * 8, ob);
}

template <bool ROPE>
__global__ __launch_bounds__(256) void qk_rmsnorm_rope_octet_kernel(const bf16_t* in, int64_t ld_in, const bf16_t* __restrict__ w_a, int h_a,
                                                                    const bf16_t* __restrict__ w_b, int h_b, const float* __restrict__ cos_t,
                                                                    const float* __restrict__ sin_t, bf16_t* out, int64_t ld_out, int64_t rows, int B,
                                                                    float eps) {
    const int sl = threadIdx.x & 7;
    const int noct = (h_a + h_b) >> 3;
    const int64_t gid = (int64_t)blockIdx.x * 32 + (threadIdx.x >> 3);
    const int64_t row = gid / noct;
    if (row >= rows) return;
    const int oct = (int)(gid - row * noct);
    const int head0 = oct * 8;
    const bf16_t* w = head0 < h_a ? w_a : w_b;
    const bf16x8 wa = load_bf16x8(w + sl * 8);
    const bf16x8 wb = load_bf16x8(w + 64 + sl * 8);
    RopeRow t{};
    if (ROPE) t = load_rope_row(cos_t, sin_t, row / B, sl);
    const bf16_t* src = in + row * ld_in + head0 * 128 + sl * 8;
    bf16_t* dst = out + row * ld_out + head0 * 128 + sl * 8;
#pragma unroll
    for (int half = 0; half < 2; ++half) {
        bf16x8 a[4], b[4];
#pragma unroll
        for (int hh = 0; hh < 4; ++hh) {
            a[hh] = load_bf16x8(src + (half * 4 + hh) * 128);
            b[hh] = load_bf16x8(src + (half * 4 + hh) * 128 + 64);
        }
#pragma unroll
        for (int hh = 0; hh < 4; ++hh) {
            bf16x8 oa, ob;
            rmsnorm_rope_head<ROPE>(a[hh], b[hh], wa, wb, t, eps, oa, ob);
            store_bf16x8(dst + (half * 4 + hh) * 128, oa);
            store_bf16x8(dst + (half * 4 + hh) * 128 + 64, ob);
        }
    }
}

__global__ __launch_bounds__(256) void transpose_v_kernel(const bf16_t* __restrict__ v, int64_t ld_in,
                                                          bf16_t* __restrict__ vt, int64_t ldvt, int S, int B, int H) {
    __shared__ bf16_t tile[64][128 + 2];
    const int tid = threadIdx.x;
    const int kv0 = blockIdx.x * 64;
    const int head = blockIdx.y;
    const int batch = blockIdx.z;
#pragma unroll
    for (int i = 0; i < 4; ++i) {
        const int idx = tid + 256 * i;
        const int r = idx >> 4, c = idx & 15;
        const int s = kv0 + r;
        bf16x8 t = zero_bf16x8();
        if (s < S) t = load_bf16x8(v + ((int64_t)s * B + batch) * ld_in + head * 128 + c * 8);
#pragma unroll
        for (int e = 0; e < 8; ++e) tile[r][c * 8 + e] = t[e];
    }
    __syncthreads();
    bf16_t* dst = vt + ((int64_t)batch * H + head) * 128 * ldvt;
#pragma unroll
    for (int i = 0; i < 4; ++i) {
        const int idx = tid + 256 * i;
        const int d = idx >> 3, c = idx & 7;
        const int kv = kv0 + c * 8;
        if (kv < ldvt) {
            bf16x8 t;
#pragma unroll
            for (int e = 0; e < 8; ++e) t[e] = tile[c * 8 + e][d];
            store_bf16x8(dst + (int64_t)d * ldvt + kv, t);
        }
    }
}

constexpr int GEMV_MAX_M = 8;

template <int ACT_IN>
__global__ __launch_bounds__(256) void gemv_kernel(const bf16_t* __restrict__ a, int64_t lda,
                                                   const bf16_t* __restrict__ w, int64_t ldw,
                                                   const bf16_t* __restrict__ add, int64_t ldadd,
                                                   bf16_t* __restrict__ out, int64_t ldo, int M, int N, int K) {
    const int wave = threadIdx.x >> 6;
    const int lane = threadIdx.x & 63;
    const int n = blockIdx.x * 4 + wave;
    if (n >= N) return;
    float acc[GEMV_MAX_M];
#pragma unroll
    for (int m = 0; m < GEMV_MAX_M; ++m) acc[m] = 0.f;
    const bf16_t* wr = w + (int64_t)n * ldw;
    for (int k = lane * 8; k < K; k += 64 * 8) {
        const bf16x8 wv = load_bf16x8(wr + k);
        float wf[8];
#pragma unroll
        for (int e = 0; e < 8; ++e) wf[e] = (float)wv[e];
#pragma unroll
        for (int m = 0; m < GEMV_MAX_M; ++m) {
            if (m < M) {
                const bf16x8 av = load_bf16x8(a + (int64_t)m * lda + k);
#pragma unroll
                for (int e = 0; e < 8; ++e) {
                    float x = (float)av[e];
                    if (ACT_IN == 1) x = (float)f32_to_bf16(silu(x));
                    acc[m] += x * wf[e];
                }
            }
        }
    }
#pragma unroll
    for (int m = 0; m < GEMV_MAX_M; ++m) {
        if (m < M) {
            float s = acc[m];
#pragma unroll
            for (int o = 32; o > 0; o >>= 1) s += __shfl_xor(s, o, 64);
            if (lane == 0) {
                if (add) s = (float)f32_to_bf16(s) + (float)add[(int64_t)m * ldadd + n];
                out[(int64_t)m * ldo + n] = f32_to_bf16(s);
            }
        }
    }
}

__global__ __launch_bounds__(256) void add_inplace_kernel(bf16_t* __restrict__ x, const bf16_t* __restrict__ y,
                                                          int64_t nchunks) {
    for (int64_t c = (int64_t)blockIdx.x * 256 + threadIdx.x; c < nchunks; c += (int64_t)gridDim.x * 256) {
        const bf16x8 a = load_bf16x8(x + c * 8);
        const bf16x8 b = load_bf16x8(y + c * 8);
        bf16x8 o;
#pragma unroll
        for (int e = 0; e < 8; ++e) o[e] = f32_to_bf16((float)a[e] + (float)b[e]);
        store_bf16x8(x + c * 8, o);
    }
}

}

extern "C" int g3_layernorm_modulate_bf16(const void* x, int64_t ldx, const void* shift, const void* scale,
                                          int64_t ldmod, int mod_rows, void* out, int64_t ldo, int rows, int D,
                                          float eps, void* stream) {
    if (!x || !shift || !scale || !out) return g3_set_error(G3_ERR_ARG, "g3_layernorm_modulate_bf16: null operand");
    if (rows <= 0 || D <= 0 || (D & 7) || D > LN_THREADS * 8 * LN_MAX_CHUNKS)
        return g3_set_error(G3_ERR_ARG, "g3_layernorm_modulate_bf16: D=%d must be a multiple of 8 and <= %d", D, LN_THREADS * 8 * LN_MAX_CHUNKS);
    if ((ldx & 7) || (ldo & 7) || (ldmod & 7) || mod_rows <= 0)
        return g3_set_error(G3_ERR_ARG, "g3_layernorm_modulate_bf16: leading dims must be multiples of 8");
    if (D == 4096 && g3_opt_ln_wave_rows)
        hipLaunchKernelGGL(ln_modulate_wave_kernel<0>, dim3((rows + 3) / 4), dim3(256), 0, (hipStream_t)stream, (bf16_t*)const_cast<void*>(x), ldx,
                           (const bf16_t*)shift, (const bf16_t*)scale, ldmod, mod_rows, (bf16_t*)out, ldo, rows, eps, PosEmbArgs{});
    else
        hipLaunchKernelGGL(ln_modulate_kernel<0>, dim3(rows), dim3(LN_THREADS), 0, (hipStream_t)stream, (bf16_t*)const_cast<void*>(x), ldx,
                           (const bf16_t*)shift, (const bf16_t*)scale, ldmod, mod_rows, (bf16_t*)out, ldo, rows, D, eps, PosEmbArgs{});
    return g3_check_launch("g3_layernorm_modulate_bf16");
}

extern "C" int g3_posemb_layernorm_modulate_bf16(void* x, int64_t ldx, const void* pe_t, const void* pe_h, const void* pe_w,
                                                 const void* pos_norm, int T, int Hp, int Wp, int B, const void* shift,
                                                 const void* scale, int64_t ldmod, int mod_rows, void* out, int64_t ldo, int D,
                                                 float eps, void* stream) {
    const bool materialised = pe_t && !pe_h && !pe_w && !pos_norm;
    if (!x || !pe_t || !shift || !scale || !out || (!materialised && (!pe_h || !pe_w || !pos_norm)))
        return g3_set_error(G3_ERR_ARG, "g3_posemb_layernorm_modulate_bf16: null operand");
    if (T <= 0 || Hp <= 0 || Wp <= 0 || B <= 0 || D <= 0 || (D & 7) || D > LN_THREADS * 8 * LN_MAX_CHUNKS)
        return g3_set_error(G3_ERR_ARG, "g3_posemb_layernorm_modulate_bf16: bad shape (T=%d Hp=%d Wp=%d B=%d D=%d)", T, Hp, Wp, B, D);
    if ((ldx & 7) || (ldo & 7) || (ldmod & 7) || mod_rows <= 0)
        return g3_set_error(G3_ERR_ARG, "g3_posemb_layernorm_modulate_bf16: leading dims must be multiples of 8");
    const int64_t rows64 = (int64_t)T * Hp * Wp * B;
    if (rows64 > 0x7fffffff) return g3_set_error(G3_ERR_ARG, "g3_posemb_layernorm_modulate_bf16: too many rows");
    const int rows = (int)rows64;
    PosEmbArgs pe{(const bf16_t*)pe_t, (const bf16_t*)pe_h, (const bf16_t*)pe_w, (const bf16_t*)pos_norm, Hp, Wp, B};
    if (materialised && D == 4096 && g3_opt_ln_wave_rows)
        hipLaunchKernelGGL(ln_modulate_wave_kernel<2>, dim3((rows + 3) / 4), dim3(256), 0, (hipStream_t)stream, (bf16_t*)x, ldx, (const bf16_t*)shift, (const bf16_t*)scale,
                           ldmod, mod_rows, (bf16_t*)out, ldo, rows, eps, pe);
    else if (materialised)
        hipLaunchKernelGGL(ln_modulate_kernel<2>, dim3(rows), dim3(LN_THREADS), 0, (hipStream_t)stream, (bf16_t*)x, ldx,
                           (const bf16_t*)shift, (const bf16_t*)scale, ldmod, mod_rows, (bf16_t*)out, ldo, rows, D, eps, pe);
    else
        hipLaunchKernelGGL(ln_modulate_kernel<1>, dim3(rows), dim3(LN_THREADS), 0, (hipStream_t)stream, (bf16_t*)x, ldx,
                           (const bf16_t*)shift, (const bf16_t*)scale, ldmod, mod_rows, (bf16_t*)out, ldo, rows, D, eps, pe);
    return g3_check_launch("g3_posemb_layernorm_modulate_bf16");
}

static int qk_rmsnorm_rope_launch(const char* what, const void* in, int64_t ld_in, const void* w_a, int h_a, const void* w_b, int h_b, const float* cos_table,
                                  const float* sin_table, void* out, int64_t ld_out, int S, int B, int head_dim, float eps, void* stream) {
    if (!in || !w_a || !out || (h_b > 0 && !w_b)) return g3_set_error(G3_ERR_ARG, "%s: null operand", what);
    if (head_dim != 128) return g3_set_error(G3_ERR_ARG, "%s: head_dim must be 128", what);
    if ((cos_table == nullptr) != (sin_table == nullptr)) return g3_set_error(G3_ERR_ARG, "%s: need both cos and sin tables or neither", what);
    if ((ld_in & 7) || (ld_out & 7)) return g3_set_error(G3_ERR_ARG, "%s: leading dims must be multiples of 8", what);
    if (S <= 0 || B <= 0 || h_a <= 0 || h_b < 0) return g3_set_error(G3_ERR_ARG, "%s: bad shape", what);
    const int64_t rows = (int64_t)S * B;
    if (g3_opt_norm_octets && (h_a % 8) == 0 && (h_b % 8) == 0) {
        const int64_t ngroups = rows * ((h_a + h_b) >> 3);
        const int64_t nblk = (ngroups + 31) / 32;
        if (nblk > 0x7fffffff) return g3_set_error(G3_ERR_ARG, "%s: too many rows", what);
        if (cos_table)
            hipLaunchKernelGGL(qk_rmsnorm_rope_octet_kernel<true>, dim3((unsigned)nblk), dim3(256), 0, (hipStream_t)stream, (const bf16_t*)in, ld_in, (const bf16_t*)w_a, h_a,
                               (const bf16_t*)w_b, h_b, cos_table, sin_table, (bf16_t*)out, ld_out, rows, B, eps);
        else
            hipLaunchKernelGGL(qk_rmsnorm_rope_octet_kernel<false>, dim3((unsigned)nblk), dim3(256), 0, (hipStream_t)stream, (const bf16_t*)in, ld_in, (const bf16_t*)w_a, h_a,
                               (const bf16_t*)w_b, h_b, cos_table, sin_table, (bf16_t*)out, ld_out, rows, B, eps);
        return g3_check_launch(what);
    }
    for (int region = 0; region < (h_b > 0 ? 2 : 1); ++region) {
        const int H = region ? h_b : h_a;
        const int64_t col0 = region ? (int64_t)h_a * 128 : 0;
        const int64_t n_pairs = rows * H;
        const int64_t nblk = (n_pairs * 8 + 255) / 256;
        hipLaunchKernelGGL(qk_rmsnorm_rope_kernel, dim3((unsigned)nblk), dim3(256), 0, (hipStream_t)stream, (const bf16_t*)in + col0, ld_in,
                           (const bf16_t*)(region ? w_b : w_a), cos_table, sin_table, (bf16_t*)out + col0, ld_out, n_pairs, H, B, eps);
        const int rc = g3_check_launch(what);
        if (rc) return rc;
    }
    return G3_OK;
}

extern "C" int g3_qk_rmsnorm_rope_bf16(const void* in, int64_t ld_in, const void* weight, const float* cos_table,
                                       const float* sin_table, void* out, int64_t ld_out, int S, int B, int H,
                                       int head_dim, float eps, void* stream) {
    return qk_rmsnorm_rope_launch("g3_qk_rmsnorm_rope_bf16", in, ld_in, weight, H, nullptr, 0, cos_table, sin_table, out, ld_out, S, B, head_dim, eps, stream);
}

extern "C" int g3_qk_rmsnorm_rope_pair_bf16(const void* in, int64_t ld_in, const void* weight_q, int H_q, const void* weight_k, int H_k, const float* cos_table,
                                            const float* sin_table, void* out, int64_t ld_out, int S, int B, int head_dim, float eps, void* stream) {
    if (H_k <= 0) return g3_set_error(G3_ERR_ARG, "g3_qk_rmsnorm_rope_pair_bf16: H_k must be positive (one region: g3_qk_rmsnorm_rope_bf16)");
    return qk_rmsnorm_rope_launch("g3_qk_rmsnorm_rope_pair_bf16", in, ld_in, weight_q, H_q, weight_k, H_k, cos_table, sin_table, out, ld_out, S, B, head_dim, eps, stream);
}

extern "C" int g3_transpose_v_bf16(const void* v, int64_t ld_in, void* vt, int64_t ldvt, int S, int B, int H,
                                   int head_dim, void* stream) {
    if (!v || !vt) return g3_set_error(G3_ERR_ARG, "g3_transpose_v_bf16: null operand");
    if (head_dim != 128) return g3_set_error(G3_ERR_ARG, "g3_transpose_v_bf16: head_dim must be 128");
    if ((ld_in & 7) || (ldvt & 7) || ldvt < S) return g3_set_error(G3_ERR_ARG, "g3_transpose_v_bf16: bad leading dims");
    dim3 grid((unsigned)((ldvt + 63) / 64), H, B);
    hipLaunchKernelGGL(transpose_v_kernel, grid, dim3(256), 0, (hipStream_t)stream, (const bf16_t*)v, ld_in, (bf16_t*)vt,
                       ldvt, S, B, H);
    return g3_check_launch("g3_transpose_v_bf16");
}

extern "C" int g3_gemv_bf16(const void* a, int64_t lda, const void* w, int64_t ldw, const void* add, int64_t ldadd,
                            void* out, int64_t ldo, int M, int N, int K, int act_in, void* stream) {
    if (!a || !w || !out) return g3_set_error(G3_ERR_ARG, "g3_gemv_bf16: null operand");
    if (M <= 0 || M > GEMV_MAX_M || N <= 0 || K <= 0 || (K & 7) || (lda & 7) || (ldw & 7))
        return g3_set_error(G3_ERR_ARG, "g3_gemv_bf16: need 1<=M<=8, K,lda,ldw %% 8 == 0 (M=%d N=%d K=%d)", M, N, K);
    dim3 grid((N + 3) / 4);
    if (act_in == 0)
        hipLaunchKernelGGL(gemv_kernel<0>, grid, dim3(256), 0, (hipStream_t)stream, (const bf16_t*)a, lda, (const bf16_t*)w, ldw,
                           (const bf16_t*)add, ldadd, (bf16_t*)out, ldo, M, N, K);
    else if (act_in == 1)
        hipLaunchKernelGGL(gemv_kernel<1>, grid, dim3(256), 0, (hipStream_t)stream, (const bf16_t*)a, lda, (const bf16_t*)w, ldw,
                           (const bf16_t*)add, ldadd, (bf16_t*)out, ldo, M, N, K);
    else
        return g3_set_error(G3_ERR_ARG, "g3_gemv_bf16: unknown act_in %d", act_in);
    return g3_check_launch("g3_gemv_bf16");
}

extern "C" int g3_add_inplace_bf16(void* x, const void* y, int64_t n, void* stream) {
    if (!x || !y) return g3_set_error(G3_ERR_ARG, "g3_add_inplace_bf16: null operand");
    if (n <= 0 || (n & 7)) return g3_set_error(G3_ERR_ARG, "g3_add_inplace_bf16: n must be a positive multiple of 8");
    const int64_t nchunks = n >> 3;
    int64_t nblk = (nchunks + 255) / 256;
    if (nblk > 256 * 16) nblk = 256 * 16;
    hipLaunchKernelGGL(add_inplace_kernel, dim3((unsigned)nblk), dim3(256), 0, (hipStream_t)stream, (bf16_t*)x, (const bf16_t*)y, nchunks);
    return g3_check_launch("g3_add_inplace_bf16");
}
```

### gen3c_amd/dit.py

```python
from __future__ import annotations

import math
from enum import Enum
from typing import Dict, List, Optional, Tuple

import torch
from torch import nn

from . import ops
from .parallel import ContextParallelAttention, split_inputs_cp

_FUSE_QKV_EPILOGUE = __import__("os").environ.get("G3_FUSE_QKV_EPILOGUE", "0") != "0"


_V_OPERAND_SWAP = __import__("os").environ.get("G3_V_OPERAND_SWAP", "1") != "0"


_CROSS_Q_NORM_IN_ATTENTION = __import__("os").environ.get("G3_CROSS_Q_NORM_IN_ATTENTION", "1") != "0"


def _project_norm_rope(h, w, n_q, n_k, norm_q, norm_k, cos, sin, S, B, nH_total, hq=None, wq=None):
    if wq is not None:
        y = ops.gemm_mxfp8_nt(hq[0], hq[1], wq[0], wq[1])
    elif _FUSE_QKV_EPILOGUE:
        return ops.gemm_qk_norm_rope(h, w, n_q, n_k, norm_q, norm_k, cos, sin, S, B)
    else:
        y = ops.gemm_nt(h, w)
    if n_q and n_k:
        ops.qk_rmsnorm_rope_pair(y[:, :n_q + n_k], norm_q, n_q // 128, norm_k, n_k // 128, cos, sin, S, B)
    elif n_q:
        ops.qk_rmsnorm_rope(y[:, :n_q], norm_q, cos, sin, S, B, n_q // 128, out=y[:, :n_q])
    elif n_k:
        ops.qk_rmsnorm_rope(y[:, n_q:n_q + n_k], norm_k, cos, sin, S, B, n_k // 128, out=y[:, n_q:n_q + n_k])
    return y


LINEAR_PRECISIONS = ("bf16", "mxfp8")
MXFP8_LINEARS = ("fa_qkv", "fa_out", "ca_q", "ca_out", "w1", "w2")


def _mx_rows(blk: dict, name: str, rows: slice):
    mx = blk.get("mx")
    return None if mx is None else (mx[name][0][rows], mx[name][1][rows])


class DataType(Enum):
    IMAGE = "image"
    VIDEO = "video"


def tensor_version(t: torch.Tensor) -> Optional[int]:
    return None if t.is_inference() else t._version


def cacheable(*tensors) -> bool:
    return all(not (isinstance(t, torch.Tensor) and t.is_inference()) for t in tensors)


def _is_video(data_type) -> bool:
    v = getattr(data_type, "value", data_type)
    return str(v).lower().endswith("video")


class _Node(nn.Module):
    """Anonymous container used to reproduce the reference's parameter names (e.g. `to_q.0.weight`)."""


def _register(root: nn.Module, dotted: str, tensor: torch.Tensor, buffer: bool = False):
    *path, leaf = dotted.split(".")
    mod = root
    for p in path:
        if p not in mod._modules:
            mod.add_module(p, _Node())
        mod = mod._modules[p]
    if buffer:
        mod.register_buffer(leaf, tensor, persistent=True)
    else:
        mod.register_parameter(leaf, nn.Parameter(tensor, requires_grad=False))


def _xavier_uniform_(t: torch.Tensor):
    fan_out, fan_in = t.shape
    a = math.sqrt(6.0 / (fan_in + fan_out))
    return t.uniform_(-a, a)


class VideoExtendGeneralDIT(nn.Module):
    def __init__(
        self,
        max_img_h: int = 240,
        max_img_w: int = 240,
        max_frames: int = 128,
        in_channels: int = 16 + 1,
        out_channels: int = 16,
        patch_spatial: int = 2,
        patch_temporal: int = 1,
        concat_padding_mask: bool = True,
        block_config: str = "FA-CA-MLP",
        model_channels: int = 4096,
        num_blocks: int = 28,
        num_heads: int = 32,
# ... 101 lines not shown
            self.initialize_weights()

    @torch.no_grad()
    def initialize_weights(self, randomize_adaln: bool = False, seed: Optional[int] = None):
        gen = None
        if seed is not None:
            gen = torch.Generator(device=self.affline_norm.weight.device)
            gen.manual_seed(seed)
        for name, p in self.named_parameters():
            if name.endswith(".to_q.1.weight") or name.endswith(".to_k.1.weight") or name == "affline_norm.weight":
                p.fill_(1.0)
            elif name.startswith("extra_pos_embedder."):
                tmp = torch.empty(p.shape, dtype=torch.float32, device=p.device)
                nn.init.trunc_normal_(tmp, std=0.02, a=-2.0, b=2.0, generator=gen)
                p.copy_(tmp)
            elif name.startswith("t_embedder."):
                p.normal_(0.0, 0.02, generator=gen)
            elif name.endswith("adaLN_modulation.2.weight") and not name.startswith("final_layer."):
                if randomize_adaln:
                    p.normal_(0.0, 0.02, generator=gen)
                else:
                    p.zero_()
            else:
                fan_out, fan_in = p.shape
                a = math.sqrt(6.0 / (fan_in + fan_out))
                p.uniform_(-a, a, generator=gen)
        self._packed = None
        self._tables.clear()

    def load_state_dict(self, state_dict, strict: bool = True, assign: bool = False):
        sd = {k: v for k, v in state_dict.items() if not k.endswith("_extra_state")}
        out = super().load_state_dict(sd, strict=strict, assign=assign)
        self._packed = None
        self._tables.clear()
        return out

    def _apply(self, fn, *args, **kwargs):
        out = super()._apply(fn, *args, **kwargs)
        self._packed = None
        self._tables.clear()
        return out

    def set_linear_precision(self, precision: str) -> None:
        if precision not in LINEAR_PRECISIONS:
            raise ValueError(f"linear_precision must be one of {LINEAR_PRECISIONS}, got {precision!r}")
        if precision != self.linear_precision:
            self._packed = None
        self.linear_precision = precision

    def _linear(self, a: torch.Tensor, blk: dict, name: str, **kw) -> torch.Tensor:
        mx = blk.get("mx")
        if mx is None:
            return ops.gemm_nt(a, blk[name], **kw)
        aq, as_ = ops.quant_mxfp8(a)
        return ops.gemm_mxfp8_nt(aq, as_, mx[name][0], mx[name][1], **kw)

    def _weights_key(self) -> tuple:
        return tuple((p.data_ptr(), tensor_version(p)) for p in self.parameters())

    def _pack(self):
        key = self._weights_key()
        if (self._packed is not None and self._packed["key"] == key and self._packed["versioned"]
                and self._packed["precision"] == self.linear_precision):
            return self._packed
        if self._packed is not None and self._packed["key"] != key:
            self._tables.clear()
        P = dict(self.named_parameters())
        blocks = []
        for i in range(self.num_blocks):
            pre = f"blocks.block{i}.blocks"
            fa, ca, mlp = f"{pre}.0", f"{pre}.1", f"{pre}.2"
            blocks.append(dict(
                fa_qkv=torch.cat([P[f"{fa}.block.attn.to_q.0.weight"], P[f"{fa}.block.attn.to_k.0.weight"],
                                  P[f"{fa}.block.attn.to_v.0.weight"]], dim=0).contiguous(),
                fa_qn=P[f"{fa}.block.attn.to_q.1.weight"], fa_kn=P[f"{fa}.block.attn.to_k.1.weight"],
                fa_out=P[f"{fa}.block.attn.to_out.0.weight"],
                ca_q=P[f"{ca}.block.attn.to_q.0.weight"],
                ca_kv=torch.cat([P[f"{ca}.block.attn.to_k.0.weight"], P[f"{ca}.block.attn.to_v.0.weight"]], dim=0).contiguous(),
                ca_qn=P[f"{ca}.block.attn.to_q.1.weight"], ca_kn=P[f"{ca}.block.attn.to_k.1.weight"],
                ca_out=P[f"{ca}.block.attn.to_out.0.weight"],
                w1=P[f"{mlp}.block.layer1.weight"], w2=P[f"{mlp}.block.layer2.weight"],
                ada=[(P[f"{pre}.{j}.adaLN_modulation.1.weight"], P[f"{pre}.{j}.adaLN_modulation.2.weight"]) for j in range(3)],
            ))
        if self.linear_precision == "mxfp8":
            for blk in blocks:
                blk["mx"] = {n: ops.quant_mxfp8(blk[n]) for n in MXFP8_LINEARS}
        self._packed = dict(blocks=blocks, P=P, key=key, versioned=cacheable(*P.values()), precision=self.linear_precision)
        return self._packed

    def enable_context_parallel(self, cp_group):
        import torch.distributed as dist
        self.cp_group = cp_group
        self.cp_size = dist.get_world_size(cp_group)
        self._cp_attn = ContextParallelAttention(cp_group, head_groups=4, schedule="local_first")
        cfg = __import__("os").environ.get("G3_CP_CONFIG")
        if cfg:
            g_, kern_, sched_ = (c.strip() for c in cfg.split(","))
            self._cp_attn.configure(head_groups=int(g_), kernel=kern_, schedule=sched_)
        self._tables.clear()

    def _cp_fused_qkv(self) -> bool:
        return self._cp_attn is not None and self._cp_attn.schedule in ("local_first", "local_carry")

    def disable_context_parallel(self):
        self.cp_group = None
        self.cp_size = None
        self._cp_attn = None
        self._tables.clear()

    @property
    def is_context_parallel_enabled(self) -> bool:
        return self.cp_group is not None

    @torch.no_grad()
    def _position_tables(self, B: int, T: int, Hp: int, Wp: int, fps: Optional[torch.Tensor], device) -> tuple:
        fps_val = None if fps is None else float(fps.flatten()[0])
        cp = self.cp_size or 1
        rank = 0
        if self.cp_group is not None:
            import torch.distributed as dist
            rank = dist.get_rank(self.cp_group)
        key = (B, T, Hp, Wp, fps_val, cp, rank, str(device))
        if key in self._tables:
            return self._tables[key]
        Tg = T * cp
        dim_t, dim_h, dim_w = self._rope_dims
        seq = self.pos_embedder.seq.to(device=device, dtype=torch.float32)
        rng_s = torch.arange(0, dim_h, 2, device=device)[: dim_h // 2].float() / dim_h
        rng_t = torch.arange(0, dim_t, 2, device=device)[: dim_t // 2].float() / dim_t
        h_freqs = 1.0 / ((10000.0 * self.h_ntk_factor) ** rng_s)
        w_freqs = 1.0 / ((10000.0 * self.w_ntk_factor) ** rng_s)
        t_freqs = 1.0 / ((10000.0 * self.t_ntk_factor) ** rng_t)
        assert Hp <= self.max_img_h // self.patch_spatial and Wp <= self.max_img_w // self.patch_spatial
        half_h = torch.outer(seq[:Hp], h_freqs)
        half_w = torch.outer(seq[:Wp], w_freqs)
        if fps_val is None:
            assert Tg == 1, "T should be 1 for image batch."
            half_t = torch.outer(seq[:Tg], t_freqs)
        else:
            half_t = torch.outer(seq[:Tg] / fps_val * self.base_fps, t_freqs)
        half = torch.cat([
            half_t[:, None, None, :].expand(Tg, Hp, Wp, -1),
            half_h[None, :, None, :].expand(Tg, Hp, Wp, -1),
            half_w[None, None, :, :].expand(Tg, Hp, Wp, -1),
        ], dim=-1)
        freqs = torch.cat([half, half], dim=-1)
        freqs = freqs[rank * T:(rank + 1) * T].reshape(T * Hp * Wp, 128).float()
        cos, sin = torch.cos(freqs).contiguous(), torch.sin(freqs).contiguous()

        pe_t = self.extra_pos_embedder.pos_emb_t[:Tg][rank * T:(rank + 1) * T].contiguous()
        pe_h = self.extra_pos_embedder.pos_emb_h[:Hp].contiguous()
        pe_w = self.extra_pos_embedder.pos_emb_w[:Wp].contiguous()
        emb = (pe_t[:, None, None, :] + pe_h[None, :, None, :]) + pe_w[None, None, :, :]
        norm = torch.linalg.vector_norm(emb, dim=-1, keepdim=True, dtype=torch.float32)
        norm = torch.add(1e-6, norm, alpha=math.sqrt(1.0 / emb.shape[-1]))
        pos = dict(pe_t=pe_t, pe_h=pe_h, pe_w=pe_w, norm=norm.to(emb.dtype).reshape(T * Hp * Wp).contiguous())
        del emb
        self._tables[key] = (cos, sin, pos)
        return self._tables[key]

    def position_embedding_rows(self, B: int, T: int, Hp: int, Wp: int, fps, device) -> torch.Tensor:
        pos = self._position_tables(B, T, Hp, Wp, fps, device)[2]
        emb = (pos["pe_t"][:, None, None, :] + pos["pe_h"][None, :, None, :]) + pos["pe_w"][None, None, :, :]
        emb = emb / pos["norm"].reshape(T, Hp, Wp, 1)
        D = emb.shape[-1]
        return emb.reshape(T * Hp * Wp, 1, D).expand(-1, B, -1).reshape(T * Hp * Wp * B, D).contiguous()

    @torch.no_grad()
    def forward(
        self,
        x: torch.Tensor,
        timesteps: torch.Tensor,
        crossattn_emb: torch.Tensor,
        crossattn_mask: Optional[torch.Tensor] = None,
        fps: Optional[torch.Tensor] = None,
        image_size: Optional[torch.Tensor] = None,
        padding_mask: Optional[torch.Tensor] = None,
        scalar_feature: Optional[torch.Tensor] = None,
        data_type=DataType.VIDEO,
        video_cond_bool: Optional[torch.Tensor] = None,
        condition_video_indicator: Optional[torch.Tensor] = None,
        condition_video_input_mask: Optional[torch.Tensor] = None,
        condition_video_augment_sigma: Optional[torch.Tensor] = None,
        condition_video_pose: Optional[torch.Tensor] = None,
        **kwargs,
    ) -> torch.Tensor:
        if scalar_feature is not None:
            raise NotImplementedError("Scalar feature is not implemented yet.")
        B, C, T, H, W = x.shape
        dev = x.device
        sources = [(x.to(torch.bfloat16).contiguous(), True)]
        if _is_video(data_type):
            assert condition_video_input_mask is not None, "condition_video_input_mask is required for video data type"
            if self.cp_group is not None:
                condition_video_input_mask = split_inputs_cp(condition_video_input_mask, 2, self.cp_group)
                if condition_video_indicator is not None:
                    condition_video_indicator = split_inputs_cp(condition_video_indicator, 2, self.cp_group)
                if condition_video_pose is not None:
                    condition_video_pose = split_inputs_cp(condition_video_pose, 2, self.cp_group)
            sources.append((condition_video_input_mask.to(torch.bfloat16).contiguous(), True))
            if condition_video_pose is not None:
                sources.append((condition_video_pose.to(torch.bfloat16).contiguous(), True))
        if self.concat_padding_mask:
            pm = _nearest_resize(padding_mask, (H, W)).to(torch.bfloat16)
            sources.append((pm.reshape(B, 1, H, W).contiguous(), False))
        c_in = sum(t.shape[1] for t, _ in sources)
        assert c_in * self.patch_spatial ** 2 * self.patch_temporal == self.patch_dim, f"channel mismatch: got {c_in} input channels"

        ps, pt = self.patch_spatial, self.patch_temporal
        Tp, Hp, Wp = T // pt, H // ps, W // ps
        S = Tp * Hp * Wp
        D = self.model_channels
        patches = ops.dit_patchify(sources, B, T, H, W, pt, ps)

        pk = self._pack()
        P = pk["P"]
        cos, sin, pos = self._position_tables(B, Tp, Hp, Wp, fps, dev)

        xs = ops.gemm_nt(patches, P["x_embedder.proj.1.weight"])

        ts = timesteps.flatten().to(torch.float32)
        if ts.shape[0] != B:
            ts = ts.expand(B)
        t_sin, emb = ops.timestep_embedding(ts.contiguous(), P["affline_norm.weight"], D)
        h1 = ops.gemv(t_sin, P["t_embedder.1.linear_1.weight"])
        adaln_lora = ops.gemv(h1, P["t_embedder.1.linear_2.weight"], act_in=1)

        M = crossattn_emb.shape[1]
        nH = self.num_heads
        ca_kv, ca_dense = self._cross_attention_kv(pk, crossattn_emb)
        if not self.cross_attention_skip_zero_context:
            ca_dense = 0
        for bi, blk in enumerate(pk["blocks"][: self._tune_blocks] if self._tune_blocks else pk["blocks"]):
            shift, scale, gate = self._modulation(emb, blk["ada"][0], adaln_lora, 3)
            if "full" not in pos:
                pe_sum = (pos["pe_t"][:, None, None, :] + pos["pe_h"][None, :, None, :]) + pos["pe_w"][None, None, :, :]
                pos["full"] = (pe_sum / pos["norm"].reshape(Tp, Hp, Wp, 1)).reshape(S, D).contiguous()
                del pe_sum
            h = ops.posemb_layernorm_modulate(xs, pos["full"], None, None, None, Tp, Hp, Wp, B, shift, scale)
            hq = ops.quant_mxfp8(h) if "mx" in blk else None
            if self._cp_fused_qkv():
                qkv = _project_norm_rope(h, blk["fa_qkv"], D, D, blk["fa_qn"], blk["fa_kn"], cos, sin, S, B, nH, hq=hq,
                                         wq=_mx_rows(blk, "fa_qkv", slice(None)))
                pending = self._cp_attn.start(qkv[:, D:2 * D], qkv[:, 2 * D:], S, B, nH)
                o = self._cp_attn.finish(qkv[:, :D], pending)
            elif self._cp_attn is not None:
                kv = _project_norm_rope(h, blk["fa_qkv"][D:], 0, D, None, blk["fa_kn"], cos, sin, S, B, nH, hq=hq,
                                        wq=_mx_rows(blk, "fa_qkv", slice(D, None)))
                pending = self._cp_attn.start(kv[:, :D], kv[:, D:], S, B, nH)
                q = _project_norm_rope(h, blk["fa_qkv"][:D], D, 0, blk["fa_qn"], None, cos, sin, S, B, nH, hq=hq,
                                       wq=_mx_rows(blk, "fa_qkv", slice(0, D)))
                o = self._cp_attn.finish(q, pending)
            else:
                if hq is not None:
                    qkv = ops.gemm_mxfp8_nt(hq[0], hq[1], *blk["mx"]["fa_qkv"])
                    ops.qk_rmsnorm_rope_pair(qkv[:, :2 * D], blk["fa_qn"], nH, blk["fa_kn"], nH, cos, sin, S, B)
                    q, k = qkv[:, :D], qkv[:, D:2 * D]
                    vt = ops.transpose_v(qkv[:, 2 * D:], S, B, nH, out=self._vt_buffer(S, B, nH, dev))
                elif _FUSE_QKV_EPILOGUE:
                    vt = self._vt_buffer(S, B, nH, dev)
                    qkv = ops.gemm_qk_norm_rope(h, blk["fa_qkv"], D, D, blk["fa_qn"], blk["fa_kn"], cos, sin, S, B, vt=vt)
                    q, k = qkv[:, :D], qkv[:, D:2 * D]
                elif _V_OPERAND_SWAP:
                    qk = ops.gemm_nt(h, blk["fa_qkv"][:2 * D])
                    ops.qk_rmsnorm_rope_pair(qk, blk["fa_qn"], nH, blk["fa_kn"], nH, cos, sin, S, B)
                    q, k = qk[:, :D], qk[:, D:]
                    vt = self._vt_buffer(S, B, nH, dev)
                    hv = h.view(S, B, D)
                    for b_ in range(B):
                        ops.gemm_nt(blk["fa_qkv"][2 * D:], hv[:, b_], out=vt[b_].view(D, -1)[:, :S])
                else:
                    qkv = ops.gemm_nt(h, blk["fa_qkv"])
                    ops.qk_rmsnorm_rope_pair(qkv[:, :2 * D], blk["fa_qn"], nH, blk["fa_kn"], nH, cos, sin, S, B)
                    q, k = qkv[:, :D], qkv[:, D:2 * D]
                    vt = ops.transpose_v(qkv[:, 2 * D:], S, B, nH, out=self._vt_buffer(S, B, nH, dev))
                o = ops.flash_attn(q, k, vt, S, S, B, nH)
            self._linear(o, blk, "fa_out", out=xs, epilogue=ops.EPI_GATED_RESIDUAL, gate=gate, residual=xs)
            shift, scale, gate = self._modulation(emb, blk["ada"][1], adaln_lora, 3)
            h = ops.layernorm_modulate(xs, shift, scale)
            k, vt = ca_kv[bi]
            if _CROSS_Q_NORM_IN_ATTENTION:
                o = ops.flash_attn(self._linear(h, blk, "ca_q"), k, vt, S, M, B, nH, kv_dense=ca_dense, q_norm_weight=blk["ca_qn"])
            else:
                q = _project_norm_rope(h, blk["ca_q"], D, 0, blk["ca_qn"], None, None, None, S, B, nH,
                                       hq=ops.quant_mxfp8(h) if "mx" in blk else None, wq=_mx_rows(blk, "ca_q", slice(None)))
                o = ops.flash_attn(q, k, vt, S, M, B, nH, kv_dense=ca_dense)
            self._linear(o, blk, "ca_out", out=xs, epilogue=ops.EPI_GATED_RESIDUAL, gate=gate, residual=xs)
            shift, scale, gate = self._modulation(emb, blk["ada"][2], adaln_lora, 3)
            h = ops.layernorm_modulate(xs, shift, scale)
            u = self._linear(h, blk, "w1", epilogue=ops.EPI_GELU)
            self._linear(u, blk, "w2", out=xs, epilogue=ops.EPI_GATED_RESIDUAL, gate=gate, residual=xs)

        fl = (P["final_layer.adaLN_modulation.1.weight"], P["final_layer.adaLN_modulation.2.weight"])
        shift, scale = self._modulation(emb, fl, adaln_lora[:, : 2 * D], 2)
        h = ops.layernorm_modulate(xs, shift, scale)
        y = ops.gemm_nt(h, P["final_layer.linear.weight"])
        return ops.dit_unpatchify(y, B, self.out_channels, T, H, W, pt, ps)

    def _vt_buffer(self, S: int, B: int, H: int, dev) -> torch.Tensor:
        key = (S, B, H, str(dev))
        buf = getattr(self, "_vt_cache", None)
        if buf is None or buf[0] != key:
            buf = self._vt_cache = (key, torch.zeros((B, H, 128, ops.ceil_to(S, 64)), dtype=torch.bfloat16, device=dev))
        return buf[1]

    def _cross_attention_kv(self, pk, crossattn_emb: torch.Tensor):
        use_cache = cacheable(crossattn_emb) and pk["versioned"]
        key = (crossattn_emb.data_ptr(), tensor_version(crossattn_emb), tuple(crossattn_emb.shape), crossattn_emb.dtype, pk["key"])
        cache = self.__dict__.setdefault("_ca_kv_cache", {})
        hit = cache.get(key) if use_cache else None
        if hit is not None and hit[0] is crossattn_emb:
            return hit[1], hit[2]
        B, M = crossattn_emb.shape[:2]
        D, nH = self.model_channels, self.num_heads
        ctx = crossattn_emb.to(torch.bfloat16).permute(1, 0, 2).reshape(M * B, -1).contiguous()
        per_block = []
        for blk in pk["blocks"]:
            kv = ops.gemm_nt(ctx, blk["ca_kv"])
            per_block.append((ops.qk_rmsnorm_rope(kv[:, :D], blk["ca_kn"], None, None, M, B, nH), ops.transpose_v(kv[:, D:], M, B, nH)))
        if not use_cache:
            return per_block, 0
        dense = 0
        live = (crossattn_emb != 0).any(dim=-1).any(dim=0)
        n_live = int(live.nonzero().max()) + 1 if bool(live.any()) else 1
        cand = min(M, ops.ceil_to(n_live, 64))
        if cand < M:
            dirty = torch.zeros((), dtype=torch.bool, device=crossattn_emb.device)
            for k_, vt_ in per_block:
                dirty |= (k_[cand * B:] != 0).any() | (vt_[..., cand:M] != 0).any()
            if not bool(dirty):
                dense = cand
        while len(cache) >= 4:
            cache.pop(next(iter(cache)))
        cache[key] = (crossattn_emb, per_block, dense)
        return per_block, dense

    def _modulation(self, emb, ada, lora, n):
        w1, w2 = ada
        mid = ops.gemv(emb, w1, act_in=1)
        mod = ops.gemv(mid, w2, add=lora)
        D = self.model_channels
        return tuple(mod[:, i * D:(i + 1) * D] for i in range(n))


def _nearest_resize(mask: torch.Tensor, size: Tuple[int, int]) -> torch.Tensor:
    m = mask
    squeeze = False
    if m.dim() == 3:
        m = m.unsqueeze(1)
        squeeze = True
    if tuple(m.shape[-2:]) != tuple(size):
        m = torch.nn.functional.interpolate(m.float(), size=size, mode="nearest").to(mask.dtype)
    return m[:, 0] if (m.dim() == 4) else m
```

### gen3c_amd/ops.py

```python
from __future__ import annotations

import math
from typing import Optional

import torch

from . import _lib

EPI_NONE, EPI_GELU, EPI_GATED_RESIDUAL, EPI_BIAS = 0, 1, 2, 3

_KERNEL_TIMERS = None


def set_option(name: str, value: int):
    _lib.check(_lib.load().g3_set_option(name.encode(), int(value)), "g3_set_option")


def enable_kernel_timers(on: bool = True):
    global _KERNEL_TIMERS
    _KERNEL_TIMERS = [] if on else None


def collected_kernel_timers():
    return list(_KERNEL_TIMERS or [])
# ... 37 lines not shown
        assert (rm, rn) == (M, N)
        rp = _dev(residual, "residual")
    lib = _lib.load()
    timer = None
    if _KERNEL_TIMERS is not None and M >= 4096:
        timer = HipTimer()
        timer.start()
    _lib.check(lib.g3_gemm_bf16_nt(_dev(a, "a"), lda, _dev(w, "w"), ldw, _dev(out, "out"), ldc, M, N, K, epilogue, gp, grows,
                                   ldg, rp, ldr, _stream()), "g3_gemm_bf16_nt")
    if timer is not None:
        timer.stop()
        _KERNEL_TIMERS.append(("gemm_nt", dict(M=M, N=N, K=K, epilogue=epilogue), timer))
    return out


def quant_mxfp8(x: torch.Tensor, out=None):
    M, K, ldx = _rowmajor2d(x, "x")
    if out is None:
        out = (torch.empty((M, K), dtype=torch.float8_e4m3fn, device=x.device), torch.empty((M, K // 32), dtype=torch.uint8, device=x.device))
    q, s = out
    Mq, Kq, ldq = _rowmajor2d(q, "q")
    Ms, Ks, lds = _rowmajor2d(s, "scales")
    if (Mq, Kq) != (M, K) or (Ms, Ks) != (M, K // 32):
        raise _lib.Gen3cHipError(f"quant_mxfp8: output shapes {tuple(q.shape)} / {tuple(s.shape)} do not match x {tuple(x.shape)}")
    lib = _lib.load()
    _lib.check(lib.g3_quant_mxfp8_bf16(_dev(x, "x"), ldx, _dev(q, "q", torch.float8_e4m3fn), ldq, _dev(s, "scales", torch.uint8), lds, M, K,
                                       _stream()), "g3_quant_mxfp8_bf16")
    return q, s


def gemm_mxfp8_nt(aq: torch.Tensor, as_: torch.Tensor, wq: torch.Tensor, ws: torch.Tensor, out: Optional[torch.Tensor] = None,
                  epilogue: int = EPI_NONE, gate: Optional[torch.Tensor] = None, residual: Optional[torch.Tensor] = None) -> torch.Tensor:
    M, K, lda = _rowmajor2d(aq, "aq")
    N, Kw, ldw = _rowmajor2d(wq, "wq")
    if K != Kw:
        raise _lib.Gen3cHipError(f"gemm_mxfp8_nt: K mismatch {K} vs {Kw}")
    Ma, Ka, ldas = _rowmajor2d(as_, "as_")
    Nw, Kws, ldws = _rowmajor2d(ws, "ws")
    if (Ma, Nw) != (M, N) or Ka * 32 != K or Kws * 32 != K:
        raise _lib.Gen3cHipError(f"gemm_mxfp8_nt: scale shapes {tuple(as_.shape)} / {tuple(ws.shape)} do not match operands [{M}, {K}] / [{N}, {K}]")
    if out is None:
        out = torch.empty((M, N), dtype=torch.bfloat16, device=aq.device)
    Mo, No, ldc = _rowmajor2d(out, "out")
    assert (Mo, No) == (M, N)
    gp, grows, ldg, rp, ldr = 0, 1, 0, 0, 0
    if gate is not None:
        grows, gn, ldg = _rowmajor2d(gate, "gate")
        assert gn == N
        gp = _dev(gate, "gate")
    if residual is not None:
        rm, rn, ldr = _rowmajor2d(residual, "residual")
        assert (rm, rn) == (M, N)
        rp = _dev(residual, "residual")
    lib = _lib.load()
    timer = None
    if _KERNEL_TIMERS is not None and M >= 4096:
        timer = HipTimer()
        timer.start()
    f8 = torch.float8_e4m3fn
    _lib.check(lib.g3_gemm_mxfp8_nt(_dev(aq, "aq", f8), lda, _dev(as_, "as_", torch.uint8), ldas, _dev(wq, "wq", f8), ldw,
                                    _dev(ws, "ws", torch.uint8), ldws, _dev(out, "out"), ldc, M, N, K, epilogue, gp, grows, ldg, rp, ldr,
                                    _stream()), "g3_gemm_mxfp8_nt")
    if timer is not None:
        timer.stop()
        _KERNEL_TIMERS.append(("gemm_mxfp8_nt", dict(M=M, N=N, K=K, epilogue=epilogue), timer))
    return out


def gemv(a: torch.Tensor, w: torch.Tensor, add: Optional[torch.Tensor] = None, act_in: int = 0,
         out: Optional[torch.Tensor] = None) -> torch.Tensor:
    M, K, lda = _rowmajor2d(a, "a")
    N, Kw, ldw = _rowmajor2d(w, "w")
    assert K == Kw
    if out is None:
        out = torch.empty((M, N), dtype=torch.bfloat16, device=a.device)
    ap, ldadd = 0, 0
    if add is not None:
        am, an, ldadd = _rowmajor2d(add, "add")
        assert (am, an) == (M, N)
        ap = _dev(add, "add")
    lib = _lib.load()
    _lib.check(lib.g3_gemv_bf16(_dev(a, "a"), lda, _dev(w, "w"), ldw, ap, ldadd, _dev(out, "out"), out.stride(0), M, N, K,
                                act_in, _stream()), "g3_gemv_bf16")
    return out


def layernorm_modulate(x: torch.Tensor, shift: torch.Tensor, scale: torch.Tensor, out: Optional[torch.Tensor] = None,
                       eps: float = 1e-6) -> torch.Tensor:
    rows, D, ldx = _rowmajor2d(x, "x")
    B, Ds, ldmod = _rowmajor2d(shift, "shift")
    assert Ds == D and scale.shape == shift.shape and scale.stride(0) == ldmod
    if out is None:
        out = torch.empty((rows, D), dtype=torch.bfloat16, device=x.device)
    lib = _lib.load()
    _lib.check(lib.g3_layernorm_modulate_bf16(_dev(x, "x"), ldx, _dev(shift, "shift"), _dev(scale, "scale"), ldmod, B,
                                              _dev(out, "out"), out.stride(0), rows, D, eps, _stream()),
               "g3_layernorm_modulate_bf16")
    return out


def posemb_layernorm_modulate(x: torch.Tensor, pe_t: torch.Tensor, pe_h: Optional[torch.Tensor], pe_w: Optional[torch.Tensor],
                              pos_norm: Optional[torch.Tensor], T: int, Hp: int, Wp: int, B: int, shift: torch.Tensor, scale: torch.Tensor,
                              out: Optional[torch.Tensor] = None, eps: float = 1e-6) -> torch.Tensor:
    rows, D, ldx = _rowmajor2d(x, "x")
    assert rows == T * Hp * Wp * B
    if pe_h is None:
        assert pe_w is None and pos_norm is None and pe_t.shape == (T * Hp * Wp, D) and pe_t.is_contiguous()
    else:
        for t, n in ((pe_t, T), (pe_h, Hp), (pe_w, Wp)):
            assert t.dim() == 2 and t.shape[0] >= n and t.shape[1] == D and t.is_contiguous()
        assert pos_norm.numel() == T * Hp * Wp and pos_norm.is_contiguous()
    Bm, Ds, ldmod = _rowmajor2d(shift, "shift")
    assert Ds == D and scale.shape == shift.shape and scale.stride(0) == ldmod
    if out is None:
        out = torch.empty((rows, D), dtype=torch.bfloat16, device=x.device)
    lib = _lib.load()
    _lib.check(lib.g3_posemb_layernorm_modulate_bf16(_dev(x, "x"), ldx, _dev(pe_t, "pe_t"), _dev(pe_h, "pe_h") if pe_h is not None else 0,
                                                     _dev(pe_w, "pe_w") if pe_w is not None else 0, _dev(pos_norm, "pos_norm") if pos_norm is not None else 0,
                                                     T, Hp, Wp, B, _dev(shift, "shift"), _dev(scale, "scale"), ldmod, Bm,
                                                     _dev(out, "out"), out.stride(0), D, eps, _stream()), "g3_posemb_layernorm_modulate_bf16")
    return out


def qk_rmsnorm_rope(x: torch.Tensor, weight: torch.Tensor, cos: Optional[torch.Tensor], sin: Optional[torch.Tensor],
                    S: int, B: int, H: int, out: Optional[torch.Tensor] = None, eps: float = 1e-6) -> torch.Tensor:
    rows, width, ld_in = _rowmajor2d(x, "x")
    assert rows == S * B and width == H * 128
    if out is None:
        out = torch.empty((rows, H * 128), dtype=torch.bfloat16, device=x.device)
    cp = sp = 0
    if cos is not None:
        assert cos.shape == (S, 128) and sin.shape == (S, 128) and cos.is_contiguous() and sin.is_contiguous()
        cp, sp = _dev(cos, "cos", torch.float32), _dev(sin, "sin", torch.float32)
    lib = _lib.load()
    _lib.check(lib.g3_qk_rmsnorm_rope_bf16(_dev(x, "x"), ld_in, _dev(weight, "weight"), cp, sp, _dev(out, "out"),
                                           out.stride(0), S, B, H, 128, eps, _stream()), "g3_qk_rmsnorm_rope_bf16")
    return out


def qk_rmsnorm_rope_pair(x: torch.Tensor, weight_q: torch.Tensor, H_q: int, weight_k: torch.Tensor, H_k: int, cos: Optional[torch.Tensor],
                         sin: Optional[torch.Tensor], S: int, B: int, out: Optional[torch.Tensor] = None, eps: float = 1e-6) -> torch.Tensor:
    rows, width, ld_in = _rowmajor2d(x, "x")
    assert rows == S * B and width == (H_q + H_k) * 128
    if out is None:
        out = x
    cp = sp = 0
    if cos is not None:
        assert cos.shape == (S, 128) and sin.shape == (S, 128) and cos.is_contiguous() and sin.is_contiguous()
        cp, sp = _dev(cos, "cos", torch.float32), _dev(sin, "sin", torch.float32)
    lib = _lib.load()
    _lib.check(lib.g3_qk_rmsnorm_rope_pair_bf16(_dev(x, "x"), ld_in, _dev(weight_q, "weight_q"), H_q, _dev(weight_k, "weight_k"), H_k, cp, sp, _dev(out, "out"),
                                                out.stride(0), S, B, 128, eps, _stream()), "g3_qk_rmsnorm_rope_pair_bf16")
    return out


def gemm_qk_norm_rope(a: torch.Tensor, w: torch.Tensor, n_q: int, n_k: int, norm_q: Optional[torch.Tensor], norm_k: Optional[torch.Tensor],
                      cos: Optional[torch.Tensor], sin: Optional[torch.Tensor], S: int, B: int, out: Optional[torch.Tensor] = None,
                      eps: float = 1e-6, vt: Optional[torch.Tensor] = None) -> torch.Tensor:
    M, K, lda = _rowmajor2d(a, "a")
    N, Kw, ldw = _rowmajor2d(w, "w")
    assert K == Kw and M == S * B
    if out is None:
        out = torch.empty((M, N), dtype=torch.bfloat16, device=a.device)
    Mo, No, ldc = _rowmajor2d(out, "out")
    assert (Mo, No) == (M, N)
    cp = sp = 0
    if cos is not None:
        assert cos.shape == (S, 128) and sin.shape == (S, 128) and cos.is_contiguous() and sin.is_contiguous()
        cp, sp = _dev(cos, "cos", torch.float32), _dev(sin, "sin", torch.float32)
    lib = _lib.load()
    timer = None
    if _KERNEL_TIMERS is not None and M >= 4096:
        timer = HipTimer()
        timer.start()
    vtp, vt_ld = 0, 0
    if vt is not None:
        n_v = N - n_q - n_k
        assert n_v > 0 and vt.dim() == 4 and vt.shape[:3] == (B, n_v // 128, 128) and vt.shape[3] >= S and vt.is_contiguous()
        vtp, vt_ld = _dev(vt, "vt"), vt.shape[3]
    _lib.check(lib.g3_gemm_qk_norm_rope_bf16(_dev(a, "a"), lda, _dev(w, "w"), ldw, _dev(out, "out"), ldc, M, N, K, n_q, n_k,
                                             _dev(norm_q, "norm_q") if n_q else 0, _dev(norm_k, "norm_k") if n_k else 0, cp, sp, B, eps, vtp, vt_ld,
                                             _stream()),
               "g3_gemm_qk_norm_rope_bf16")
    if timer is not None:
        timer.stop()
        _KERNEL_TIMERS.append(("gemm_nt", dict(M=M, N=N, K=K, epilogue=5), timer))
    return out


def ceil_to(x: int, m: int) -> int:
    return (x + m - 1) // m * m


def transpose_v(v: torch.Tensor, S: int, B: int, H: int, out: Optional[torch.Tensor] = None) -> torch.Tensor:
    rows, width, ld_in = _rowmajor2d(v, "v")
    assert rows == S * B and width == H * 128
    ldvt = ceil_to(S, 64)
    if out is None:
        out = torch.empty((B, H, 128, ldvt), dtype=torch.bfloat16, device=v.device)
    assert out.shape == (B, H, 128, ldvt) and out.is_contiguous()
    lib = _lib.load()
    _lib.check(lib.g3_transpose_v_bf16(_dev(v, "v"), ld_in, _dev(out, "out"), ldvt, S, B, H, 128, _stream()),
               "g3_transpose_v_bf16")
    return out


def flash_attn(q: torch.Tensor, k: torch.Tensor, vt: torch.Tensor, Sq: int, Skv: int, B: int, H: int,
               out: Optional[torch.Tensor] = None, softmax_scale: Optional[float] = None, variant: int = 0, partial: bool = False, kv_dense: int = 0,
               q_norm_weight: Optional[torch.Tensor] = None, q_norm_eps: float = 1e-6, carry=None, kv_skip=None):
    if carry is not None or kv_skip is not None or (partial and out is not None):
        return _flash_attn_carry(q, k, vt, Sq, Skv, B, H, out, softmax_scale, variant, partial, carry, kv_skip)
    qr, qw, ldq = _rowmajor2d(q, "q")
    kr, kw, ldk = _rowmajor2d(k, "k")
    assert qr == Sq * B and kr == Skv * B and qw == H * 128 and kw == H * 128
    assert vt.is_contiguous() and vt.dim() in (4, 5) and tuple(vt.shape[-4:-1]) == (B, H, 128)
    ldvt = vt.shape[-1]
    o_part = lse = None
    if partial:
        assert out is None
        o_part = torch.empty((Sq * B, H * 128), dtype=torch.float32, device=q.device)
        lse = torch.empty((B, H, Sq), dtype=torch.float32, device=q.device)
        ldo = o_part.stride(0)
    else:
        if out is None:
            out = torch.empty((Sq * B, H * 128), dtype=torch.bfloat16, device=q.device)
        ldo = out.stride(0)
    if softmax_scale is None:
        softmax_scale = 1.0 / math.sqrt(128)
    lib = _lib.load()
    timer = None
    if _KERNEL_TIMERS is not None:
        timer = HipTimer()
        timer.start()
    n_seg = vt.shape[0] if vt.dim() == 5 else 0
    if n_seg:
        assert Skv % n_seg == 0
    if 0 < kv_dense < Skv or q_norm_weight is not None:
        assert not partial and not n_seg and not variant, "the cross-attention form takes plain V^T, a bf16 output and the automatic kernel choice"
        kd = int(kv_dense) if 0 < kv_dense < Skv else 0
        _lib.check(lib.g3_cross_attn_fwd_bf16(_dev(q, "q"), ldq * B, ldq, 128, _dev(q_norm_weight, "q_norm_weight") if q_norm_weight is not None else 0, float(q_norm_eps),
                                              _dev(k, "k"), ldk * B, ldk, 128, _dev(vt, "vt"), ldvt, H * 128 * ldvt, 128 * ldvt,
                                              _dev(out, "out"), ldo * B, ldo, 128, Sq, Skv, kd, B, H, 128, float(softmax_scale), _stream()),
                   "g3_cross_attn_fwd_bf16")
        if timer is not None:
            timer.stop()
            _KERNEL_TIMERS.append(("flash_attn_fwd", dict(Sq=Sq, Skv=Skv, B=B, H=H, partial=False, kv_dense=kd, q_norm=q_norm_weight is not None,
                                                          kernel=lib.g3_flash_attn_kernel_name_ex(Sq, Skv, B, H, 4).decode()), timer))
        return out
    _lib.check(lib.g3_flash_attn_fwd_ex_bf16(_dev(q, "q"), ldq * B, ldq, 128, _dev(k, "k"), ldk * B, ldk, 128, _dev(vt, "vt"), ldvt, H * 128 * ldvt, 128 * ldvt,
                                             Skv // n_seg if n_seg else 0, B * H * 128 * ldvt if n_seg else 0,
                                             0 if partial else _dev(out, "out"), _dev(o_part, "o_part", torch.float32) if partial else 0,
                                             _dev(lse, "lse", torch.float32) if partial else 0, ldo * B, ldo, 128, Sq, Skv, B, H, 128,
                                             float(softmax_scale), int(variant), _stream()), "g3_flash_attn_fwd_ex_bf16")
    if timer is not None:
        timer.stop()
        _KERNEL_TIMERS.append(("flash_attn_fwd", dict(Sq=Sq, Skv=Skv, B=B, H=H, partial=partial,
                                                      kernel=lib.g3_flash_attn_kernel_name_ex(Sq, Skv, B, H, int(variant)).decode()), timer))
    return (o_part, lse) if partial else out


def _carry_kernel_name(plain: str) -> str:
    return {"flash_attn_fwd_w4b_kernel<true>": "flash_attn_fwd_w4b_carry_kernel<true>",
            "flash_attn_fwd_v3_kernel<0, 6, 8, true>": "flash_attn_fwd_v3_kernel<2, 6, 8, true>",
            "flash_attn_fwd_v3_kernel<1, 6, 8, false>": "flash_attn_fwd_v3_kernel<3, 6, 8, false>"}.get(plain, plain)


def _flash_attn_carry(q, k, vt, Sq, Skv, B, H, out, softmax_scale, variant, partial, carry, kv_skip):
    skip_begin, skip_len = (int(kv_skip[0]), int(kv_skip[1])) if kv_skip is not None else (0, 0)
    skv_all = Skv + skip_len
    qr, qw, ldq = _rowmajor2d(q, "q")
    kr, kw, ldk = _rowmajor2d(k, "k")
    assert qr == Sq * B and kr == skv_all * B and qw == H * 128 and kw == H * 128
    assert vt.is_contiguous() and vt.dim() in (4, 5) and tuple(vt.shape[-4:-1]) == (B, H, 128)
    ldvt = vt.shape[-1]
    n_seg = vt.shape[0] if vt.dim() == 5 else 0
    if n_seg:
        assert skv_all % n_seg == 0
    lse = None
    if partial:
        if out is None:
            out = torch.empty((Sq * B, H * 128), dtype=torch.float32, device=q.device)
        assert out.dtype == torch.float32, "partial=True writes fp32"
        lse = torch.empty((B, H, Sq), dtype=torch.float32, device=q.device)
    elif out is None:
        out = torch.empty((Sq * B, H * 128), dtype=torch.bfloat16, device=q.device)
    orows, ow, ldo = _rowmajor2d(out, "out")
    assert (orows, ow) == (Sq * B, H * 128)
    co = cl = 0
    if carry is not None:
        o_c, l_c = carry
        if o_c.dtype != torch.float32 or o_c.shape != (Sq * B, H * 128) or o_c.stride() != out.stride():
            raise ValueError(f"flash_attn: carry o_part must be fp32 {(Sq * B, H * 128)} with the output's strides {out.stride()} "
                             f"(got {o_c.dtype} {tuple(o_c.shape)} {o_c.stride()})")
        if l_c.dtype != torch.float32 or l_c.shape != (B, H, Sq) or not l_c.is_contiguous():
            raise ValueError(f"flash_attn: carry lse must be contiguous fp32 {(B, H, Sq)}")
        co, cl = _dev(o_c, "carry_o", torch.float32), _dev(l_c, "carry_lse", torch.float32)
    if softmax_scale is None:
        softmax_scale = 1.0 / math.sqrt(128)
    lib = _lib.load()
    timer = None
    if _KERNEL_TIMERS is not None:
        timer = HipTimer()
        timer.start()
    _lib.check(lib.g3_flash_attn_fwd_carry_bf16(_dev(q, "q"), ldq * B, ldq, 128, _dev(k, "k"), ldk * B, ldk, 128, _dev(vt, "vt"), ldvt, H * 128 * ldvt,
                                                128 * ldvt, skv_all // n_seg if n_seg else 0, B * H * 128 * ldvt if n_seg else 0, skip_begin, skip_len, co, cl,
                                                0 if partial else _dev(out, "out"), _dev(out, "o_part", torch.float32) if partial else 0,
                                                _dev(lse, "lse", torch.float32) if partial else 0, ldo * B, ldo, 128, Sq, Skv, B, H, 128,
                                                float(softmax_scale), int(variant), _stream()), "g3_flash_attn_fwd_carry_bf16")
    if timer is not None:
        timer.stop()
        _KERNEL_TIMERS.append(("flash_attn_fwd", dict(Sq=Sq, Skv=Skv, B=B, H=H, partial=partial, carry=carry is not None, kv_skip=skip_len,
                                                      kernel=_carry_kernel_name(lib.g3_flash_attn_kernel_name_ex(Sq, Skv, B, H, int(variant)).decode())), timer))
    return (out, lse) if partial else out


def attn_merge(parts, Sq: int, B: int, H: int, out: Optional[torch.Tensor] = None) -> torch.Tensor:
    import ctypes as C
    n = len(parts)
    assert 1 <= n <= 8
# ... 115 lines not shown
```

### include/gen3c_hip.h

```cpp
#ifndef GEN3C_HIP_H
#define GEN3C_HIP_H

#include <stddef.h>
#include <stdint.h>

#ifdef __cplusplus
extern "C" {
#endif

#define G3_OK 0
#define G3_ERR_ARG 1
#define G3_ERR_LAUNCH 2
#define G3_ERR_RESOURCE 3

#define G3_EPI_NONE 0
#define G3_EPI_GELU 1
#define G3_EPI_GATED_RESIDUAL 2
#define G3_EPI_BIAS 3
#define G3_EPI_BIAS_RESIDUAL 4

const char* g3_last_error(void);
int g3_abi_version(void);
int g3_set_option(const char* name , int value);
int g3_device_info(int device, int* cu_count, int* is_gfx950, char* arch_name , int arch_name_len);

int g3_event_create(void** ev);
int g3_event_record(void* ev, void* stream);
int g3_event_elapsed_ms(void* start, void* stop, float* ms );
int g3_event_destroy(void* ev);

int g3_gemm_bf16_nt(const void* A, int64_t lda, const void* W, int64_t ldw, void* C, int64_t ldc, int M, int N, int K,
                    int epilogue, const void* gate, int gate_rows, int64_t ldg, const void* residual, int64_t ldr,
                    void* stream);

const char* g3_gemm_kernel_name(int M, int N, int K, int epilogue);

int g3_quant_mxfp8_bf16(const void* x, int64_t ldx, void* q, int64_t ldq, void* scales, int64_t lds, int M, int K, void* stream);

int g3_gemm_mxfp8_nt(const void* aq, int64_t lda, const void* as, int64_t ldas, const void* wq, int64_t ldw, const void* ws, int64_t ldws,
                     void* c, int64_t ldc, int M, int N, int K, int epilogue, const void* gate, int gate_rows, int64_t ldg,
                     const void* residual, int64_t ldr, void* stream);

const char* g3_gemm_mxfp8_kernel_name(int M, int N, int K, int epilogue);

int g3_gemv_bf16(const void* a, int64_t lda, const void* w, int64_t ldw, const void* add, int64_t ldadd, void* out,
                 int64_t ldo, int M, int N, int K, int act_in, void* stream);

int g3_flash_attn_fwd_bf16(const void* q, int64_t q_row, int64_t q_batch, int64_t q_head, const void* k, int64_t k_row,
                           int64_t k_batch, int64_t k_head, const void* vt, int64_t vt_row, int64_t vt_batch,
                           int64_t vt_head, void* o, int64_t o_row, int64_t o_batch, int64_t o_head, int Sq, int Skv,
                           int B, int H, int head_dim, float softmax_scale, void* stream);

const char* g3_flash_attn_kernel_name(int Sq, int Skv, int B, int H);

int g3_cross_attn_fwd_bf16(const void* q, int64_t q_row, int64_t q_batch, int64_t q_head, const void* q_norm_weight, float q_norm_eps,
                           const void* k, int64_t k_row, int64_t k_batch, int64_t k_head, const void* vt, int64_t vt_row, int64_t vt_batch,
                           int64_t vt_head, void* o, int64_t o_row, int64_t o_batch, int64_t o_head, int Sq, int Skv, int kv_dense, int B, int H,
                           int head_dim, float softmax_scale, void* stream);

int g3_flash_attn_fwd_kvseg_bf16(const void* q, int64_t q_row, int64_t q_batch, int64_t q_head, const void* k, int64_t k_row,
                                 int64_t k_batch, int64_t k_head, const void* vt, int64_t vt_row, int64_t vt_batch, int64_t vt_head,
                                 int vt_seg_len, int64_t vt_seg_stride, void* o, int64_t o_row, int64_t o_batch, int64_t o_head, int Sq,
                                 int Skv, int B, int H, int head_dim, float softmax_scale, void* stream);

int g3_flash_attn_fwd_ex_bf16(const void* q, int64_t q_row, int64_t q_batch, int64_t q_head, const void* k, int64_t k_row, int64_t k_batch,
                              int64_t k_head, const void* vt, int64_t vt_row, int64_t vt_batch, int64_t vt_head, int vt_seg_len,
                              int64_t vt_seg_stride, void* o, float* o_partial, float* lse, int64_t o_row, int64_t o_batch, int64_t o_head,
                              int Sq, int Skv, int B, int H, int head_dim, float softmax_scale, int variant, void* stream);
const char* g3_flash_attn_kernel_name_ex(int Sq, int Skv, int B, int H, int variant);

int g3_flash_attn_fwd_carry_bf16(const void* q, int64_t q_row, int64_t q_batch, int64_t q_head, const void* k, int64_t k_row, int64_t k_batch,
                                 int64_t k_head, const void* vt, int64_t vt_row, int64_t vt_batch, int64_t vt_head, int vt_seg_len,
                                 int64_t vt_seg_stride, int kv_skip_begin, int kv_skip_len, const float* carry_o, const float* carry_lse,
                                 void* o, float* o_partial, float* lse, int64_t o_row, int64_t o_batch, int64_t o_head, int Sq, int Skv, int B,
                                 int H, int head_dim, float softmax_scale, int variant, void* stream);
int g3_attn_merge_partials_bf16(const float* const* o_parts , const float* const* lse_parts , int n_parts, int64_t p_row,
                                int64_t p_batch, int64_t p_head, void* out, int64_t o_row, int64_t o_batch, int64_t o_head, int Sq, int B,
                                int H, int head_dim, void* stream);

int g3_transpose_v_bf16(const void* v, int64_t ld_in, void* vt, int64_t ldvt, int S, int B, int H, int head_dim,
                        void* stream);

int g3_layernorm_modulate_bf16(const void* x, int64_t ldx, const void* shift, const void* scale, int64_t ldmod,
                               int mod_rows, void* out, int64_t ldo, int rows, int D, float eps, void* stream);

int g3_qk_rmsnorm_rope_bf16(const void* in, int64_t ld_in, const void* weight, const float* cos_table,
                            const float* sin_table, void* out, int64_t ld_out, int S, int B, int H, int head_dim,
                            float eps, void* stream);

int g3_qk_rmsnorm_rope_pair_bf16(const void* in, int64_t ld_in, const void* weight_q, int H_q, const void* weight_k, int H_k,
                                 const float* cos_table, const float* sin_table, void* out, int64_t ld_out, int S, int B, int head_dim,
                                 float eps, void* stream);

int g3_gemm_qk_norm_rope_bf16(const void* A, int64_t lda, const void* W, int64_t ldw, void* C, int64_t ldc, int M, int N, int K,
                              int n_q, int n_k, const void* norm_q, const void* norm_k, const float* cos_table,
                              const float* sin_table, int B, float eps, void* vt, int64_t vt_ld, void* stream);

int g3_posemb_layernorm_modulate_bf16(void* x, int64_t ldx, const void* pe_t, const void* pe_h, const void* pe_w,
                                      const void* pos_norm, int T, int Hp, int Wp, int B, const void* shift, const void* scale,
                                      int64_t ldmod, int mod_rows, void* out, int64_t ldo, int D, float eps, void* stream);

int g3_add_inplace_bf16(void* x, const void* y, int64_t n, void* stream);

int g3_dit_patchify_bf16(const void* const* srcs, const int* chans, const int* has_t, int n_src, void* out, int B, int T, int H,
                         int W, int patch_t, int patch_s, void* stream);
int g3_dit_unpatchify_bf16(const void* y, int64_t ldy, void* out, int B, int C_out, int T, int H, int W, int patch_t, int patch_s,
                           void* stream);
int g3_timestep_embedding_bf16(const float* timesteps, const void* norm_weight, void* t_sin, void* emb, int B, int D, void* stream);

int g3_edm_prepare_input_bf16(const void* xt, const void* gt_latent, const float* noise, const float* indicator,
                              void* new_xt, void* new_xt_scaled, int64_t n, int T, int hw, float augment_sigma,
                              float c_in_aug, float c_in_bf16, float c_in_step, void* stream);
int g3_edm_cfg_euler_step_bf16(const void* out_cond, const void* out_uncond, const void* new_xt, const void* gt_latent,
                               const float* indicator, void* xt_next, int64_t n, int T, int hw, float guidance,
                               float c_skip_bf16, float c_out_bf16, float c_skip, float c_out, float sigma,
                               float sigma_next, void* stream);

int g3_warp_project_f32(const float* points, const float* w2c, const float* K, const float* mask1, float* z, float* flow,
                        float* cam_points, float* maskz, void* group_max, int n, int h, int w, int group_size, void* stream);
int g3_warp_splat_f32(const float* image, const float* z, const float* flow, const float* maskz, const void* group_max,
                      float* accum, int n, int h, int w, int group_size, void* stream);
int g3_warp_resolve_f32(const float* accum, float* frame, float* mask, float* depth, int n, int h, int w, void* stream);

size_t g3_warp_windows_workspace_bytes(int n, int h, int w);
int g3_warp_splat_resolve_f32(const float* image, const float* z, const float* flow, const float* maskz, const void* group_max,
                              float* accum, void* workspace, float* frame, float* mask, float* depth, int n, int h, int w,
                              int group_size, void* stream);
size_t g3_render_workspace_bytes(int n, int h, int w, int group_size);
int g3_render_workspace_init(void* workspace, int n, int h, int w, int group_size, void* stream);
int g3_render_items_f32(const float* points_src, const float* image_src, const float* mask_src, const uint8_t* boundary_src,
                        const int* src_index, const float* w2c, const float* K, const float* Kinv, void* workspace, float* frame, float* mask,
                        float* depth, float* flow_out, int n, int n_src, int h, int w, int group_size, void* stream);
int g3_mesh_occlusion_f32(const float* cam_points, const uint8_t* boundary_mask, const float* K, const float* Kinv,
                          float* pts_ds, uint8_t* mask_ds, void* tmin, float* frame, float* mask, float* depth, int n, int h,
                          int w, int factor, void* stream);
int g3_unproject_points_f32(const float* depth, const float* c2w, const float* Kinv, float* points, int n, int h, int w,
                            void* stream);
int g3_reliable_depth_mask_f32(const float* depth, uint8_t* out, int n, int h, int w, int window, float ratio_thresh,
                               float eps, void* stream);
size_t g3_align_depth_workspace_bytes(int H, int W);
int g3_align_depth_f32(const float* source_depth, const float* target_depth, const uint8_t* target_mask, const float* Kinv_host,
// ... 30 lines not shown
```

Measured before the change: 0.2998.

## Fuse Q RMSNorm+RoPE into self-attention, batch adaLN modulations, widen attention stores

Adds a self-attention entry point that applies the query RMSNorm and rotary embedding inside the w4b/one-wave attention kernels, so the separate Q norm/RoPE pass and its extra round trip through memory go away. Unsupported kernel variants fall back to the old separate kernel. Also replaces the per-block adaLN modulation GEMVs with one batched GEMV computed up front, and adds a wider 16-byte output store in the attention epilogue using permlane swaps. These bundle several unrelated changes, and the fused prologue adds register pressure to the attention kernels.

Result: no change. 0.3019, median of 6 (+0.7%).

```diff
diff --git a/gen3c_amd/_lib.py b/gen3c_amd/_lib.py
--- a/gen3c_amd/_lib.py
+++ b/gen3c_amd/_lib.py
@@ -8,7 +8,7 @@
 
 vp, i64, i32, f32 = C.c_void_p, C.c_int64, C.c_int, C.c_float
 
-G3_OK, G3_ERR_ARG, G3_ERR_LAUNCH, G3_ERR_RESOURCE = 0, 1, 2, 3
+G3_OK, G3_ERR_ARG, G3_ERR_LAUNCH, G3_ERR_RESOURCE, G3_UNSUPPORTED = 0, 1, 2, 3, 4
 
 SIGNATURES = {
     "g3_last_error": [],
@@ -27,11 +27,14 @@
     "g3_gemm_mxfp8_nt": [vp, i64, vp, i64, vp, i64, vp, i64, vp, i64, i32, i32, i32, i32, vp, i32, i64, vp, i64, vp],
     "g3_gemm_mxfp8_kernel_name": [i32, i32, i32, i32],
     "g3_gemv_bf16": [vp, i64, vp, i64, vp, i64, vp, i64, i32, i32, i32, i32, vp],
+    "g3_gemv_batched_bf16": [vp, i64, i64, vp, i64, i64, vp, i64, i64, vp, i64, i64, i32, i32, i32, i32, i32, vp],
     "g3_flash_attn_kernel_name": [i32, i32, i32, i32],
     "g3_flash_attn_fwd_bf16": [vp, i64, i64, i64, vp, i64, i64, i64, vp, i64, i64, i64, vp, i64, i64, i64, i32, i32, i32,
                                i32, i32, f32, vp],
     "g3_cross_attn_fwd_bf16": [vp, i64, i64, i64, vp, f32, vp, i64, i64, i64, vp, i64, i64, i64, vp, i64, i64, i64, i32, i32, i32, i32, i32,
                                i32, f32, vp],
+    "g3_self_attn_fwd_bf16": [vp, i64, i64, i64, vp, f32, vp, vp, vp, i64, i64, i64, vp, i64, i64, i64, vp, i64, i64, i64, i32, i32, i32, i32, i32,
+                              f32, vp],
     "g3_flash_attn_fwd_ex_bf16": [vp, i64, i64, i64, vp, i64, i64, i64, vp, i64, i64, i64, i32, i64, vp, vp, vp, i64, i64, i64, i32, i32, i32,
                                   i32, i32, f32, i32, vp],
     "g3_flash_attn_fwd_carry_bf16": [vp, i64, i64, i64, vp, i64, i64, i64, vp, i64, i64, i64, i32, i64, i32, i32, vp, vp, vp, vp, vp, i64, i64,
diff --git a/gen3c_amd/csrc/api.hip b/gen3c_amd/csrc/api.hip
--- a/gen3c_amd/csrc/api.hip
+++ b/gen3c_amd/csrc/api.hip
@@ -28,6 +28,7 @@
 }
 int g3_opt_gemm_regstage = env_int("G3_GEMM_REGSTAGE", 0);
 int g3_opt_attn_xcd_heads = env_int("G3_ATTN_XCD_HEADS", 1);
+int g3_opt_attn_wide_store = 1;
 int g3_opt_attn_variant = env_int("G3_ATTN_VARIANT", 0);
 int g3_opt_gemm_rowmajor_tiles = env_int("G3_GEMM_ROWMAJOR_TILES", 0);
 int g3_opt_gemm_wide_store = env_int("G3_GEMM_WIDE_STORE", 1);
@@ -68,6 +69,7 @@
     if (!strcmp(name, "ln_wave_rows")) { g3_opt_ln_wave_rows = value; return G3_OK; }
     if (!strcmp(name, "norm_octets")) { g3_opt_norm_octets = value; return G3_OK; }
     if (!strcmp(name, "attn_variant")) { g3_opt_attn_variant = value; return G3_OK; }
+    if (!strcmp(name, "attn_wide_store")) { g3_opt_attn_wide_store = value; return G3_OK; }
     if (!strcmp(name, "attn_xcd_heads")) { g3_opt_attn_xcd_heads = value; return G3_OK; }
     return g3_set_error(G3_ERR_ARG, "g3_set_option: unknown option %s", name);
 }
diff --git a/gen3c_amd/csrc/attention.hip b/gen3c_amd/csrc/attention.hip
--- a/gen3c_amd/csrc/attention.hip
+++ b/gen3c_amd/csrc/attention.hip
@@ -27,6 +27,9 @@
     int kv_dense;
     const bf16_t* q_norm_w;
     float q_norm_eps;
+    const float* rope_cos;
+    const float* rope_sin;
+    int o_wide;
     const float* carry_o;
     const float* carry_lse;
     int kv_skip_begin, kv_skip_len;
@@ -212,6 +215,16 @@
     float a = x, b = x;
     swap_halves(a, b);
     return a + b;
+}
+G3_DEVICE u32x4 wide_o_pair(u32x2 a, u32x2 b) {
+    const auto r0 = __builtin_amdgcn_permlane32_swap(a[0], b[0], false, false);
+    const auto r1 = __builtin_amdgcn_permlane32_swap(a[1], b[1], false, false);
+    return u32x4{r0[0], r1[0], r0[1], r1[1]};
+}
+G3_DEVICE u32x2 pack_bf16x4(float a, float b, float c, float d) {
+    bf16x4 o;
+    o[0] = f32_to_bf16(a); o[1] = f32_to_bf16(b); o[2] = f32_to_bf16(c); o[3] = f32_to_bf16(d);
+    return __builtin_bit_cast(u32x2, o);
 }
 
 template <int CTX>
@@ -465,6 +478,13 @@
         const bf16_t* qrow = Qb + (int64_t)(q_ok ? q_idx : 0) * p.q_row + 8 * g;
 #pragma unroll
         for (int ks = 0; ks < 8; ++ks) qf[ks] = q_ok ? load_bf16x8(qrow + 16 * ks) : zero_bf16x8();
+    }
+    bf16x8 qnw[8];
+    if (p.q_norm_w) {
+#pragma unroll
+        for (int ks = 0; ks < 8; ++ks) qnw[ks] = load_bf16x8(p.q_norm_w + 16 * ks + 8 * g);
+    }
+    auto q_prepare = [&]() {
         if (p.q_norm_w) {
             float ss = 0.f;
 #pragma unroll
@@ -474,11 +494,9 @@
             ss = xor32_sum(ss);
             const float rinv = rsqrtf(ss * (1.0f / 128.0f) + p.q_norm_eps);
 #pragma unroll
-            for (int ks = 0; ks < 8; ++ks) {
-                const bf16x8 w8 = load_bf16x8(p.q_norm_w + 16 * ks + 8 * g);
-#pragma unroll
-                for (int e = 0; e < 8; ++e) qf[ks][e] = f32_to_bf16((float)qf[ks][e] * rinv * (float)w8[e]);
-            }
+            for (int ks = 0; ks < 8; ++ks)
+#pragma unroll
+                for (int e = 0; e < 8; ++e) qf[ks][e] = f32_to_bf16((float)qf[ks][e] * rinv * (float)qnw[ks][e]);
         }
         if (FOLD) {
 #pragma unroll
@@ -486,7 +504,7 @@
 #pragma unroll
                 for (int e = 0; e < 8; ++e) qf[ks][e] = f32_to_bf16((float)qf[ks][e] * p.scale_log2);
         }
-    }
+    };
 
     const int k_row0 = tid >> 4, k_src_chunk = (tid & 15) ^ (k_row0 & 15);
     const int v_row0 = tid >> 3, v_src_chunk = (tid & 7) ^ ((v_row0 >> 1) & 7);
@@ -579,6 +597,7 @@
     dma_k(0, 0);
     dma_v(0, 0);
     if (nt > 1) dma_k(KVB, 1);
+    q_prepare();
     lds_dma_publish_barrier();
     G3_JITTER(wave + 2, blockIdx.x);
     f32x16 SA[2], SB[2];
@@ -834,6 +853,20 @@
         const float rs = 1.0f / (wc + wk);
         const float fc = wc * rs, fk = (wk * rs) * inv;
         const bool use_c = fc > 0.f;
+        if (!p.O32 && p.o_wide) {
+            const int64_t ro = o_hb + (int64_t)q_idx * p.o_row;
+#pragma unroll
+            for (int d = 0; d < 4; ++d)
+#pragma unroll
+                for (int q2 = 0; q2 < 2; ++q2) {
+                    float o[8];
+#pragma unroll
+                    for (int e = 0; e < 8; ++e) o[e] = (use_c ? fc * oc[d][2 * q2 + (e >> 2)][e & 3] : 0.f) + fk * accO[d][8 * q2 + e];
+                    const u32x4 w = wide_o_pair(pack_bf16x4(o[0], o[1], o[2], o[3]), pack_bf16x4(o[4], o[5], o[6], o[7]));
+                    if (q_ok) *reinterpret_cast<u32x4*>(p.O + ro + 32 * d + 16 * q2 + 8 * g) = w;
+                }
+            return;
+        }
         if (q_ok) {
             const int64_t ro = o_hb + (int64_t)q_idx * p.o_row;
 #pragma unroll
@@ -871,6 +904,20 @@
                 }
             if (g == 0) p.LSE[((int64_t)blockIdx.z * p.n_heads + blockIdx.y) * p.Sq + q_idx] = m_run + __builtin_amdgcn_logf(l_tot);
         }
+        return;
+    }
+    if (p.o_wide) {
+        bf16_t* orow = Ob + (int64_t)q_idx * p.o_row;
+#pragma unroll
+        for (int d = 0; d < 4; ++d)
+#pragma unroll
+            for (int q2 = 0; q2 < 2; ++q2) {
+                float o[8];
+#pragma unroll
+                for (int e = 0; e < 8; ++e) o[e] = accO[d][8 * q2 + e] * inv;
+                const u32x4 w = wide_o_pair(pack_bf16x4(o[0], o[1], o[2], o[3]), pack_bf16x4(o[4], o[5], o[6], o[7]));
+                if (q_ok) *reinterpret_cast<u32x4*>(orow + 32 * d + 16 * q2 + 8 * g) = w;
+            }
         return;
     }
     if (q_ok) {
@@ -935,7 +982,8 @@
                              int64_t vt_seg_stride, void* o, int64_t o_row, int64_t o_batch, int64_t o_head, int Sq, int Skv, int B, int H,
                              int head_dim, float softmax_scale, void* stream, int variant_req = 0, float* o_partial = nullptr, float* lse = nullptr, int kv_dense = 0,
                              const void* q_norm_w = nullptr, float q_norm_eps = 0.f, bool cp_form = false, const float* carry_o = nullptr,
-                             const float* carry_lse = nullptr, int kv_skip_begin = 0, int kv_skip_len = 0, uint32_t kv_skip_vt_bytes = 0) {
+                             const float* carry_lse = nullptr, int kv_skip_begin = 0, int kv_skip_len = 0, uint32_t kv_skip_vt_bytes = 0,
+                             const float* rope_cos = nullptr, const float* rope_sin = nullptr, bool self_form = false) {
     if (!q || !k || !vt || (!o && !o_partial)) return g3_set_error(G3_ERR_ARG, "g3_flash_attn_fwd_bf16: null operand");
     if ((o_partial != nullptr) != (lse != nullptr)) return g3_set_error(G3_ERR_ARG, "g3_flash_attn_fwd_ex_bf16: o_partial and lse go together");
     if (o_partial && (((uintptr_t)o_partial & 15) || ((uintptr_t)lse & 3))) return g3_set_error(G3_ERR_ARG, "g3_flash_attn_fwd_ex_bf16: misaligned o_partial / lse");
@@ -971,6 +1019,8 @@
     p.carry_o = carry_o; p.carry_lse = carry_lse;
     p.kv_skip_begin = kv_skip_begin; p.kv_skip_len = kv_skip_len; p.kv_skip_vt_bytes = kv_skip_vt_bytes;
     if (q_norm_w && ((uintptr_t)q_norm_w & 15)) return g3_set_error(G3_ERR_ARG, "g3_cross_attn_fwd_bf16: misaligned q_norm_weight");
+    p.rope_cos = rope_cos; p.rope_sin = rope_sin;
+    p.o_wide = (g3_opt_attn_wide_store && o && !((uintptr_t)o & 15) && !(o_row & 7) && !(o_batch & 7) && !(o_head & 7)) ? 1 : 0;
     const size_t smem = (size_t)2 * (KVB * HD + HD * KVB) * sizeof(bf16_t);
     static bool attr_set[64] = {};
     static std::mutex attr_mu;
@@ -979,7 +1029,7 @@
         return g3_set_error(G3_ERR_ARG, "g3_flash_attn_fwd_carry_bf16: the carry / key-skip form exists for the 8-wave (4) and one-wave-per-SIMD (11) kernels only "
                                         "(variant %d chosen; 11 needs S_kv %% 64 == 0)", variant);
     if (o_partial && variant == 9) variant = 4;
-    if ((p.kv_dense || p.q_norm_w) && (variant < 3 || variant >= 9)) variant = 4;
+    if (!self_form && (p.kv_dense || p.q_norm_w) && (variant < 3 || variant >= 9)) variant = 4;
     if (variant >= 3 && vt_row < ((kv_span + KVB - 1) / KVB) * KVB) variant = 2;
     if (variant >= 3) {
         const uint64_t k_max = (uint64_t)(skv_phys - 1 + 2 * KVB) * (uint64_t)k_row * 2u + 256u;
@@ -1002,6 +1052,7 @@
         return g3_set_error(G3_ERR_ARG, "g3_flash_attn_fwd_kvseg_bf16: segmented V^T is implemented by the default (v3) kernel only");
     if (o_partial && variant < 3)
         return g3_set_error(G3_ERR_ARG, "g3_flash_attn_fwd_ex_bf16: split-KV partial outputs are implemented by the v3 / w4b kernels only (variant %d chosen)", variant);
+    if (self_form && variant != 10 && variant != 11) return G3_UNSUPPORTED;
     if ((p.kv_dense || p.q_norm_w) && variant < 3)
         return g3_set_error(G3_ERR_ARG, "g3_cross_attn_fwd_bf16: the Q norm / zero-tail form is implemented by the v3 kernels only (variant %d chosen: V^T leading dimension below "
                                         "ceil64(S_kv), or operands beyond the kernel's 32-bit byte offsets)", variant);
@@ -1085,6 +1136,18 @@
     if (kv_dense < 0) return g3_set_error(G3_ERR_ARG, "g3_cross_attn_fwd_bf16: kv_dense must be >= 0 (0 = every key through the loop)");
     return flash_attn_launch(q, q_row, q_batch, q_head, k, k_row, k_batch, k_head, vt, vt_row, vt_batch, vt_head, 0, 0, o, o_row, o_batch, o_head, Sq, Skv, B, H,
                              head_dim, softmax_scale, stream, 0, nullptr, nullptr, kv_dense, q_norm_weight, q_norm_eps);
+}
+
+extern "C" int g3_self_attn_fwd_bf16(const void* q, int64_t q_row, int64_t q_batch, int64_t q_head, const void* q_norm_weight, float q_norm_eps,
+                                     const float* rope_cos, const float* rope_sin, const void* k, int64_t k_row, int64_t k_batch, int64_t k_head, const void* vt,
+                                     int64_t vt_row, int64_t vt_batch, int64_t vt_head, void* o, int64_t o_row, int64_t o_batch, int64_t o_head, int Sq, int Skv,
+                                     int B, int H, int head_dim, float softmax_scale, void* stream) {
+    if (!q_norm_weight) return g3_set_error(G3_ERR_ARG, "g3_self_attn_fwd_bf16: q_norm_weight is required (plain launches: g3_flash_attn_fwd_bf16)");
+    if ((rope_cos == nullptr) != (rope_sin == nullptr)) return g3_set_error(G3_ERR_ARG, "g3_self_attn_fwd_bf16: need both cos and sin tables or neither");
+    if (((uintptr_t)rope_cos | (uintptr_t)rope_sin) & 15) return g3_set_error(G3_ERR_ARG, "g3_self_attn_fwd_bf16: misaligned cos / sin table");
+    return flash_attn_launch(q, q_row, q_batch, q_head, k, k_row, k_batch, k_head, vt, vt_row, vt_batch, vt_head, 0, 0, o, o_row, o_batch, o_head, Sq, Skv, B, H,
+                             head_dim, softmax_scale, stream, 0, nullptr, nullptr, 0, q_norm_weight, q_norm_eps, false, nullptr, nullptr, 0, 0, 0, rope_cos, rope_sin,
+                             true);
 }
 
 extern "C" int g3_flash_attn_fwd_ex_bf16(const void* q, int64_t q_row, int64_t q_batch, int64_t q_head, const void* k, int64_t k_row,
diff --git a/gen3c_amd/csrc/attention_w4b.hpp b/gen3c_amd/csrc/attention_w4b.hpp
--- a/gen3c_amd/csrc/attention_w4b.hpp
+++ b/gen3c_amd/csrc/attention_w4b.hpp
@@ -195,6 +195,18 @@
     float* o32_base = p.O32;
     float* lse_base = p.LSE;
     asm volatile("" : "+s"(o32_base), "+s"(lse_base));
+    const bf16_t* qn_w = nullptr;
+    const float* rope_c = nullptr;
+    const float* rope_s = nullptr;
+    uint32_t qn_eps_bits = 0u, o_wide = (uint32_t)p.o_wide;
+    if constexpr (!CP) {
+        qn_w = p.q_norm_w;
+        rope_c = p.rope_cos;
+        rope_s = p.rope_sin;
+        qn_eps_bits = __builtin_bit_cast(uint32_t, p.q_norm_eps);
+        asm volatile("" : "+s"(qn_w), "+s"(rope_c), "+s"(rope_s), "+s"(qn_eps_bits));
+    }
+    asm volatile("" : "+s"(o_wide));
     const float* carry_o = nullptr;
     const float* carry_lse = nullptr;
     uint32_t skip_t0 = 0u, skip_nt = 0u, v_skip = 0u;
@@ -211,6 +223,57 @@
         else return t;
     };
 
+    if (!CP && qn_w) {
+        static_for<0, 2>([&](auto hc) {
+            constexpr int h = decltype(hc)::value;
+            const int q_idx = qblk * W4_BQ + wave * 64 + 32 * h + l31;
+            const bool q_ok = q_idx < p.Sq;
+            const int q_ld = q_ok ? q_idx : 0;
+            bf16x8 qv[8];
+#pragma unroll
+            for (int ks = 0; ks < 8; ++ks) qv[ks] = q_ok ? load_bf16x8(Qb + (int64_t)q_idx * p.q_row + 8 * g + 16 * ks) : zero_bf16x8();
+            float ss = 0.f;
+#pragma unroll
+            for (int ks = 0; ks < 8; ++ks)
+#pragma unroll
+                for (int e = 0; e < 8; ++e) { const float f = (float)qv[ks][e]; ss += f * f; }
+            ss = xor32_sum(ss);
+            const float rinv = rsqrtf(ss * (1.0f / 128.0f) + __builtin_bit_cast(float, qn_eps_bits));
+#pragma unroll
+            for (int ks = 0; ks < 8; ++ks) {
+                const bf16x8 w8 = load_bf16x8(qn_w + 16 * ks + 8 * g);
+#pragma unroll
+                for (int e = 0; e < 8; ++e) qv[ks][e] = f32_to_bf16((float)qv[ks][e] * rinv * (float)w8[e]);
+            }
+            if (rope_c) {
+                const float* cr = rope_c + (int64_t)q_ld * 128 + 8 * g;
+                const float* sr = rope_s + (int64_t)q_ld * 128 + 8 * g;
+#pragma unroll
+                for (int ks = 0; ks < 4; ++ks) {
+                    const f32x4 c0 = *reinterpret_cast<const f32x4*>(cr + 16 * ks), c1 = *reinterpret_cast<const f32x4*>(cr + 16 * ks + 4);
+                    const f32x4 s0 = *reinterpret_cast<const f32x4*>(sr + 16 * ks), s1 = *reinterpret_cast<const f32x4*>(sr + 16 * ks + 4);
+#pragma unroll
+                    for (int e = 0; e < 8; ++e) {
+                        const float c = e < 4 ? c0[e & 3] : c1[e & 3], s = e < 4 ? s0[e & 3] : s1[e & 3];
+                        const float fa = (float)qv[ks][e], fb = (float)qv[ks + 4][e];
+                        qv[ks][e] = f32_to_bf16(fa * c - fb * s);
+                        qv[ks + 4][e] = f32_to_bf16(fb * c + fa * s);
+                    }
+                }
+            }
+            static_for<0, 8>([&](auto kc) {
+                constexpr int ks = decltype(kc)::value, f = 8 * h + ks;
+                bf16x8 qs;
+#pragma unroll
+                for (int e = 0; e < 8; ++e) qs[e] = f32_to_bf16((float)qv[ks][e] * p.scale_log2);
+                const u32x4 qw = __builtin_bit_cast(u32x4, qs);
+                w4_acc_write<W4_QBASE + 4 * f + 0>(qw[0]);
+                w4_acc_write<W4_QBASE + 4 * f + 1>(qw[1]);
+                w4_acc_write<W4_QBASE + 4 * f + 2>(qw[2]);
+                w4_acc_write<W4_QBASE + 4 * f + 3>(qw[3]);
+            });
+        });
+    } else {
     static_for<0, 16>([&](auto fc) {
         constexpr int f = decltype(fc)::value, h = f >> 3, ks = f & 7;
         const int q_idx = qblk * W4_BQ + wave * 64 + 32 * h + l31;
@@ -224,6 +287,7 @@
         w4_acc_write<W4_QBASE + 4 * f + 2>(qw[2]);
         w4_acc_write<W4_QBASE + 4 * f + 3>(qw[3]);
     });
+    }
     static_for<0, 128>([&](auto rc) { w4_acc_zero<decltype(rc)::value>(); });
 
     const int k_row0 = tid >> 4, k_src_chunk = (tid & 15) ^ (k_row0 & 15);
@@ -531,6 +595,19 @@
             const float rs = 1.0f / (wc + wk);
             const float fc = wc * rs, fk = (wk * rs) * inv;
             const bool use_c = fc > 0.f;
+            if (!o32_base && o_wide) {
+                static_for<0, 8>([&](auto cc) {
+                    constexpr int c = 2 * decltype(cc)::value, d = c >> 2, q4 = c & 3;
+                    constexpr int R = 16 * (4 * h + d) + 4 * q4;
+                    const u32x2 a = pack_bf16x4((use_c ? fc * oc[c][0] : 0.f) + fk * w4_acc_read<R + 0>(), (use_c ? fc * oc[c][1] : 0.f) + fk * w4_acc_read<R + 1>(),
+                                                (use_c ? fc * oc[c][2] : 0.f) + fk * w4_acc_read<R + 2>(), (use_c ? fc * oc[c][3] : 0.f) + fk * w4_acc_read<R + 3>());
+                    const u32x2 b = pack_bf16x4((use_c ? fc * oc[c + 1][0] : 0.f) + fk * w4_acc_read<R + 4>(), (use_c ? fc * oc[c + 1][1] : 0.f) + fk * w4_acc_read<R + 5>(),
+                                                (use_c ? fc * oc[c + 1][2] : 0.f) + fk * w4_acc_read<R + 6>(), (use_c ? fc * oc[c + 1][3] : 0.f) + fk * w4_acc_read<R + 7>());
+                    const u32x4 w = wide_o_pair(a, b);
+                    if (q_ok) *reinterpret_cast<u32x4*>(p.O + ro + 32 * d + 8 * q4 + 8 * g) = w;
+                });
+                return;
+            }
             static_for<0, 16>([&](auto cc) {
                 constexpr int c = decltype(cc)::value, d = c >> 2, q4 = c & 3;
                 constexpr int R = 16 * (4 * h + d) + 4 * q4;
@@ -569,6 +646,17 @@
             return;
         }
         bf16_t* orow = Ob + (int64_t)q_idx * p.o_row;
+        if (o_wide) {
+            static_for<0, 8>([&](auto cc) {
+                constexpr int d = decltype(cc)::value >> 1, q4 = 2 * (decltype(cc)::value & 1);
+                constexpr int R = 16 * (4 * h + d) + 4 * q4;
+                const u32x2 a = pack_bf16x4(w4_acc_read<R + 0>() * inv, w4_acc_read<R + 1>() * inv, w4_acc_read<R + 2>() * inv, w4_acc_read<R + 3>() * inv);
+                const u32x2 b = pack_bf16x4(w4_acc_read<R + 4>() * inv, w4_acc_read<R + 5>() * inv, w4_acc_read<R + 6>() * inv, w4_acc_read<R + 7>() * inv);
+                const u32x4 w = wide_o_pair(a, b);
+                if (q_idx < p.Sq) *reinterpret_cast<u32x4*>(orow + 32 * d + 8 * q4 + 8 * g) = w;
+            });
+            return;
+        }
         static_for<0, 16>([&](auto cc) {
             constexpr int d = decltype(cc)::value >> 2, q4 = decltype(cc)::value & 3;
             constexpr int R = 16 * (4 * h + d) + 4 * q4;
diff --git a/gen3c_amd/csrc/common.hpp b/gen3c_amd/csrc/common.hpp
--- a/gen3c_amd/csrc/common.hpp
+++ b/gen3c_amd/csrc/common.hpp
@@ -19,6 +19,7 @@
 #define G3_ERR_ARG 1
 #define G3_ERR_LAUNCH 2
 #define G3_ERR_RESOURCE 3
+#define G3_UNSUPPORTED 4
 
 int g3_set_error(int code, const char* fmt, ...);
 int g3_check_launch(const char* what);
@@ -39,6 +40,7 @@
 extern int g3_opt_render_fused;
 extern int g3_opt_render_overlap;
 extern int g3_opt_splat_tiled;
+extern int g3_opt_attn_wide_store;
 extern int g3_opt_attn_xcd_heads;
 extern int g3_opt_ln_wave_rows;
 extern int g3_opt_norm_octets;
diff --git a/gen3c_amd/csrc/norm_rope.hip b/gen3c_amd/csrc/norm_rope.hip
--- a/gen3c_amd/csrc/norm_rope.hip
+++ b/gen3c_amd/csrc/norm_rope.hip
@@ -318,11 +318,16 @@
 __global__ __launch_bounds__(256) void gemv_kernel(const bf16_t* __restrict__ a, int64_t lda,
                                                    const bf16_t* __restrict__ w, int64_t ldw,
                                                    const bf16_t* __restrict__ add, int64_t ldadd,
-                                                   bf16_t* __restrict__ out, int64_t ldo, int M, int N, int K) {
+                                                   bf16_t* __restrict__ out, int64_t ldo, int M, int N, int K, int64_t a_batch, int64_t w_batch,
+                                                   int64_t add_batch, int64_t out_batch) {
     const int wave = threadIdx.x >> 6;
     const int lane = threadIdx.x & 63;
     const int n = blockIdx.x * 4 + wave;
     if (n >= N) return;
+    a += blockIdx.y * a_batch;
+    w += blockIdx.y * w_batch;
+    if (add) add += blockIdx.y * add_batch;
+    out += blockIdx.y * out_batch;
     float acc[GEMV_MAX_M];
 #pragma unroll
     for (int m = 0; m < GEMV_MAX_M; ++m) acc[m] = 0.f;
@@ -473,21 +478,34 @@
     return g3_check_launch("g3_transpose_v_bf16");
 }
 
+static int gemv_launch(const char* what, const void* a, int64_t lda, int64_t a_batch, const void* w, int64_t ldw, int64_t w_batch, const void* add, int64_t ldadd,
+                       int64_t add_batch, void* out, int64_t ldo, int64_t out_batch, int M, int N, int K, int act_in, int n_batch, void* stream) {
+    if (!a || !w || !out) return g3_set_error(G3_ERR_ARG, "%s: null operand", what);
+    if (M <= 0 || M > GEMV_MAX_M || N <= 0 || K <= 0 || (K & 7) || (lda & 7) || (ldw & 7))
+        return g3_set_error(G3_ERR_ARG, "%s: need 1<=M<=8, K,lda,ldw %% 8 == 0 (M=%d N=%d K=%d)", what, M, N, K);
+    if (n_batch <= 0 || n_batch > 65535 || a_batch < 0 || w_batch < 0 || add_batch < 0 || out_batch < 0 || (a_batch & 7) || (w_batch & 7))
+        return g3_set_error(G3_ERR_ARG, "%s: need 1<=n_batch<=65535, batch strides >= 0, a_batch,w_batch %% 8 == 0 (n_batch=%d)", what, n_batch);
+    dim3 grid((N + 3) / 4, n_batch);
+    if (act_in == 0)
+        hipLaunchKernelGGL(gemv_kernel<0>, grid, dim3(256), 0, (hipStream_t)stream, (const bf16_t*)a, lda, (const bf16_t*)w, ldw,
+                           (const bf16_t*)add, ldadd, (bf16_t*)out, ldo, M, N, K, a_batch, w_batch, add_batch, out_batch);
+    else if (act_in == 1)
+        hipLaunchKernelGGL(gemv_kernel<1>, grid, dim3(256), 0, (hipStream_t)stream, (const bf16_t*)a, lda, (const bf16_t*)w, ldw,
+                           (const bf16_t*)add, ldadd, (bf16_t*)out, ldo, M, N, K, a_batch, w_batch, add_batch, out_batch);
+    else
+        return g3_set_error(G3_ERR_ARG, "%s: unknown act_in %d", what, act_in);
+    return g3_check_launch(what);
+}
+
 extern "C" int g3_gemv_bf16(const void* a, int64_t lda, const void* w, int64_t ldw, const void* add, int64_t ldadd,
                             void* out, int64_t ldo, int M, int N, int K, int act_in, void* stream) {
-    if (!a || !w || !out) return g3_set_error(G3_ERR_ARG, "g3_gemv_bf16: null operand");
-    if (M <= 0 || M > GEMV_MAX_M || N <= 0 || K <= 0 || (K & 7) || (lda & 7) || (ldw & 7))
-        return g3_set_error(G3_ERR_ARG, "g3_gemv_bf16: need 1<=M<=8, K,lda,ldw %% 8 == 0 (M=%d N=%d K=%d)", M, N, K);
-    dim3 grid((N + 3) / 4);
-    if (act_in == 0)
-        hipLaunchKernelGGL(gemv_kernel<0>, grid, dim3(256), 0, (hipStream_t)stream, (const bf16_t*)a, lda, (const bf16_t*)w, ldw,
-                           (const bf16_t*)add, ldadd, (bf16_t*)out, ldo, M, N, K);
-    else if (act_in == 1)
-        hipLaunchKernelGGL(gemv_kernel<1>, grid, dim3(256), 0, (hipStream_t)stream, (const bf16_t*)a, lda, (const bf16_t*)w, ldw,
-                           (const bf16_t*)add, ldadd, (bf16_t*)out, ldo, M, N, K);
-    else
-        return g3_set_error(G3_ERR_ARG, "g3_gemv_bf16: unknown act_in %d", act_in);
-    return g3_check_launch("g3_gemv_bf16");
+    return gemv_launch("g3_gemv_bf16", a, lda, 0, w, ldw, 0, add, ldadd, 0, out, ldo, 0, M, N, K, act_in, 1, stream);
+}
+
+extern "C" int g3_gemv_batched_bf16(const void* a, int64_t lda, int64_t a_batch, const void* w, int64_t ldw, int64_t w_batch, const void* add, int64_t ldadd,
+                                    int64_t add_batch, void* out, int64_t ldo, int64_t out_batch, int M, int N, int K, int act_in, int n_batch, void* stream) {
+    if (n_batch > 1 && out_batch == 0) return g3_set_error(G3_ERR_ARG, "g3_gemv_batched_bf16: out_batch must be positive");
+    return gemv_launch("g3_gemv_batched_bf16", a, lda, a_batch, w, ldw, w_batch, add, ldadd, add_batch, out, ldo, out_batch, M, N, K, act_in, n_batch, stream);
 }
 
 extern "C" int g3_add_inplace_bf16(void* x, const void* y, int64_t n, void* stream) {
diff --git a/gen3c_amd/dit.py b/gen3c_amd/dit.py
--- a/gen3c_amd/dit.py
+++ b/gen3c_amd/dit.py
@@ -17,6 +17,9 @@
 
 
 _CROSS_Q_NORM_IN_ATTENTION = __import__("os").environ.get("G3_CROSS_Q_NORM_IN_ATTENTION", "1") != "0"
+
+
+_SELF_Q_NORM_ROPE_IN_ATTENTION = True
 
 
 def _project_norm_rope(h, w, n_q, n_k, norm_q, norm_k, cos, sin, S, B, nH_total, hq=None, wq=None):
@@ -284,10 +287,17 @@
                 w1=P[f"{mlp}.block.layer1.weight"], w2=P[f"{mlp}.block.layer2.weight"],
                 ada=[(P[f"{pre}.{j}.adaLN_modulation.1.weight"], P[f"{pre}.{j}.adaLN_modulation.2.weight"]) for j in range(3)],
             ))
+        ada = [pair for blk in blocks for pair in blk["ada"]] + [(P["final_layer.adaLN_modulation.1.weight"], P["final_layer.adaLN_modulation.2.weight"])]
+        L, D = ada[0][0].shape
+        assert all(w1.shape == (L, D) for w1, _ in ada) and all(w2.shape == (3 * D, L) for _, w2 in ada[:-1]) and ada[-1][1].shape == (2 * D, L)
+        ada_w1 = torch.cat([w1 for w1, _ in ada], dim=0).contiguous()
+        ada_w2 = torch.zeros((len(ada), 3 * D, L), dtype=ada[0][1].dtype, device=ada[0][1].device)
+        for j, (_, w2) in enumerate(ada):
+            ada_w2[j, : w2.shape[0]].copy_(w2)
         if self.linear_precision == "mxfp8":
             for blk in blocks:
                 blk["mx"] = {n: ops.quant_mxfp8(blk[n]) for n in MXFP8_LINEARS}
-        self._packed = dict(blocks=blocks, P=P, key=key, versioned=cacheable(*P.values()), precision=self.linear_precision)
+        self._packed = dict(blocks=blocks, P=P, ada_w1=ada_w1, ada_w2=ada_w2, key=key, versioned=cacheable(*P.values()), precision=self.linear_precision)
         return self._packed
 
     def enable_context_parallel(self, cp_group):
@@ -433,8 +443,9 @@
         ca_kv, ca_dense = self._cross_attention_kv(pk, crossattn_emb)
         if not self.cross_attention_skip_zero_context:
             ca_dense = 0
+        mods = self._modulations(emb, pk, adaln_lora)
         for bi, blk in enumerate(pk["blocks"][: self._tune_blocks] if self._tune_blocks else pk["blocks"]):
-            shift, scale, gate = self._modulation(emb, blk["ada"][0], adaln_lora, 3)
+            shift, scale, gate = mods[3 * bi]
             if "full" not in pos:
                 pe_sum = (pos["pe_t"][:, None, None, :] + pos["pe_h"][None, :, None, :]) + pos["pe_w"][None, None, :, :]
                 pos["full"] = (pe_sum / pos["norm"].reshape(Tp, Hp, Wp, 1)).reshape(S, D).contiguous()
@@ -454,6 +465,7 @@
                                        wq=_mx_rows(blk, "fa_qkv", slice(0, D)))
                 o = self._cp_attn.finish(q, pending)
             else:
+                fa_q_form = {}
                 if hq is not None:
                     qkv = ops.gemm_mxfp8_nt(hq[0], hq[1], *blk["mx"]["fa_qkv"])
                     ops.qk_rmsnorm_rope_pair(qkv[:, :2 * D], blk["fa_qn"], nH, blk["fa_kn"], nH, cos, sin, S, B)
@@ -465,8 +477,12 @@
                     q, k = qkv[:, :D], qkv[:, D:2 * D]
                 elif _V_OPERAND_SWAP:
                     qk = ops.gemm_nt(h, blk["fa_qkv"][:2 * D])
-                    ops.qk_rmsnorm_rope_pair(qk, blk["fa_qn"], nH, blk["fa_kn"], nH, cos, sin, S, B)
                     q, k = qk[:, :D], qk[:, D:]
+                    if _SELF_Q_NORM_ROPE_IN_ATTENTION:
+                        ops.qk_rmsnorm_rope(k, blk["fa_kn"], cos, sin, S, B, nH, out=k)
+                        fa_q_form = dict(q_norm_weight=blk["fa_qn"], rope=(cos, sin))
+                    else:
+                        ops.qk_rmsnorm_rope_pair(qk, blk["fa_qn"], nH, blk["fa_kn"], nH, cos, sin, S, B)
                     vt = self._vt_buffer(S, B, nH, dev)
                     hv = h.view(S, B, D)
                     for b_ in range(B):
@@ -476,9 +492,9 @@
                     ops.qk_rmsnorm_rope_pair(qkv[:, :2 * D], blk["fa_qn"], nH, blk["fa_kn"], nH, cos, sin, S, B)
                     q, k = qkv[:, :D], qkv[:, D:2 * D]
                     vt = ops.transpose_v(qkv[:, 2 * D:], S, B, nH, out=self._vt_buffer(S, B, nH, dev))
-                o = ops.flash_attn(q, k, vt, S, S, B, nH)
+                o = ops.flash_attn(q, k, vt, S, S, B, nH, **fa_q_form)
             self._linear(o, blk, "fa_out", out=xs, epilogue=ops.EPI_GATED_RESIDUAL, gate=gate, residual=xs)
-            shift, scale, gate = self._modulation(emb, blk["ada"][1], adaln_lora, 3)
+            shift, scale, gate = mods[3 * bi + 1]
             h = ops.layernorm_modulate(xs, shift, scale)
             k, vt = ca_kv[bi]
             if _CROSS_Q_NORM_IN_ATTENTION:
@@ -488,13 +504,12 @@
                                        hq=ops.quant_mxfp8(h) if "mx" in blk else None, wq=_mx_rows(blk, "ca_q", slice(None)))
                 o = ops.flash_attn(q, k, vt, S, M, B, nH, kv_dense=ca_dense)
             self._linear(o, blk, "ca_out", out=xs, epilogue=ops.EPI_GATED_RESIDUAL, gate=gate, residual=xs)
-            shift, scale, gate = self._modulation(emb, blk["ada"][2], adaln_lora, 3)
+            shift, scale, gate = mods[3 * bi + 2]
             h = ops.layernorm_modulate(xs, shift, scale)
             u = self._linear(h, blk, "w1", epilogue=ops.EPI_GELU)
             self._linear(u, blk, "w2", out=xs, epilogue=ops.EPI_GATED_RESIDUAL, gate=gate, residual=xs)
 
-        fl = (P["final_layer.adaLN_modulation.1.weight"], P["final_layer.adaLN_modulation.2.weight"])
-        shift, scale = self._modulation(emb, fl, adaln_lora[:, : 2 * D], 2)
+        shift, scale = mods[-1][:2]
         h = ops.layernorm_modulate(xs, shift, scale)
         y = ops.gemm_nt(h, P["final_layer.linear.weight"])
         return ops.dit_unpatchify(y, B, self.out_channels, T, H, W, pt, ps)
@@ -537,6 +552,12 @@
         cache[key] = (crossattn_emb, per_block, dense)
         return per_block, dense
 
+    def _modulations(self, emb, pk, lora):
+        mid = ops.gemv(emb, pk["ada_w1"], act_in=1)
+        mod = ops.gemv_batched(mid, pk["ada_w2"], add=lora)
+        D = self.model_channels
+        return [tuple(mod[:, (3 * j + i) * D:(3 * j + i + 1) * D] for i in range(3)) for j in range(pk["ada_w2"].shape[0])]
+
     def _modulation(self, emb, ada, lora, n):
         w1, w2 = ada
         mid = ops.gemv(emb, w1, act_in=1)
diff --git a/gen3c_amd/ops.py b/gen3c_amd/ops.py
--- a/gen3c_amd/ops.py
+++ b/gen3c_amd/ops.py
@@ -143,6 +143,22 @@
     lib = _lib.load()
     _lib.check(lib.g3_gemv_bf16(_dev(a, "a"), lda, _dev(w, "w"), ldw, ap, ldadd, _dev(out, "out"), out.stride(0), M, N, K,
                                 act_in, _stream()), "g3_gemv_bf16")
+    return out
+
+
+def gemv_batched(a: torch.Tensor, w: torch.Tensor, add: Optional[torch.Tensor] = None, act_in: int = 0) -> torch.Tensor:
+    n, N, K = w.shape
+    M, Ka, lda = _rowmajor2d(a, "a")
+    assert Ka == n * K and w.is_contiguous()
+    out = torch.empty((M, n * N), dtype=torch.bfloat16, device=a.device)
+    ap, ldadd = 0, 0
+    if add is not None:
+        am, an, ldadd = _rowmajor2d(add, "add")
+        assert (am, an) == (M, N)
+        ap = _dev(add, "add")
+    lib = _lib.load()
+    _lib.check(lib.g3_gemv_batched_bf16(_dev(a, "a"), lda, K, _dev(w, "w"), K, N * K, ap, ldadd, 0, _dev(out, "out"), out.stride(0), N, M, N, K,
+                                        act_in, n, _stream()), "g3_gemv_batched_bf16")
     return out
 
 
@@ -268,7 +284,7 @@
 
 def flash_attn(q: torch.Tensor, k: torch.Tensor, vt: torch.Tensor, Sq: int, Skv: int, B: int, H: int,
                out: Optional[torch.Tensor] = None, softmax_scale: Optional[float] = None, variant: int = 0, partial: bool = False, kv_dense: int = 0,
-               q_norm_weight: Optional[torch.Tensor] = None, q_norm_eps: float = 1e-6, carry=None, kv_skip=None):
+               q_norm_weight: Optional[torch.Tensor] = None, q_norm_eps: float = 1e-6, carry=None, kv_skip=None, rope=None):
     if carry is not None or kv_skip is not None or (partial and out is not None):
         return _flash_attn_carry(q, k, vt, Sq, Skv, B, H, out, softmax_scale, variant, partial, carry, kv_skip)
     qr, qw, ldq = _rowmajor2d(q, "q")
@@ -296,6 +312,25 @@
     n_seg = vt.shape[0] if vt.dim() == 5 else 0
     if n_seg:
         assert Skv % n_seg == 0
+    if rope is not None:
+        assert q_norm_weight is not None and not partial and not n_seg and not variant and not kv_dense, \
+            "the self-attention form takes q_norm_weight, plain V^T, a bf16 output and the automatic kernel choice"
+        cos, sin = rope
+        assert cos.shape == (Sq, 128) and sin.shape == (Sq, 128) and cos.is_contiguous() and sin.is_contiguous()
+        rc = lib.g3_self_attn_fwd_bf16(_dev(q, "q"), ldq * B, ldq, 128, _dev(q_norm_weight, "q_norm_weight"), float(q_norm_eps), _dev(cos, "cos", torch.float32),
+                                       _dev(sin, "sin", torch.float32), _dev(k, "k"), ldk * B, ldk, 128, _dev(vt, "vt"), ldvt, H * 128 * ldvt, 128 * ldvt,
+                                       _dev(out, "out"), ldo * B, ldo, 128, Sq, Skv, B, H, 128, float(softmax_scale), _stream())
+        if rc == _lib.G3_UNSUPPORTED:
+            q = qk_rmsnorm_rope(q, q_norm_weight, cos, sin, Sq, B, H, eps=q_norm_eps)
+            ldq = q.stride(0)
+            q_norm_weight = None
+        else:
+            _lib.check(rc, "g3_self_attn_fwd_bf16")
+            if timer is not None:
+                timer.stop()
+                _KERNEL_TIMERS.append(("flash_attn_fwd", dict(Sq=Sq, Skv=Skv, B=B, H=H, partial=False,
+                                                              kernel=lib.g3_flash_attn_kernel_name_ex(Sq, Skv, B, H, 0).decode()), timer))
+            return out
     if 0 < kv_dense < Skv or q_norm_weight is not None:
         assert not partial and not n_seg and not variant, "the cross-attention form takes plain V^T, a bf16 output and the automatic kernel choice"
         kd = int(kv_dense) if 0 < kv_dense < Skv else 0
diff --git a/include/gen3c_hip.h b/include/gen3c_hip.h
--- a/include/gen3c_hip.h
+++ b/include/gen3c_hip.h
@@ -12,6 +12,7 @@
 #define G3_ERR_ARG 1
 #define G3_ERR_LAUNCH 2
 #define G3_ERR_RESOURCE 3
+#define G3_UNSUPPORTED 4
 
 #define G3_EPI_NONE 0
 #define G3_EPI_GELU 1
@@ -45,6 +46,8 @@
 
 int g3_gemv_bf16(const void* a, int64_t lda, const void* w, int64_t ldw, const void* add, int64_t ldadd, void* out,
                  int64_t ldo, int M, int N, int K, int act_in, void* stream);
+int g3_gemv_batched_bf16(const void* a, int64_t lda, int64_t a_batch, const void* w, int64_t ldw, int64_t w_batch, const void* add, int64_t ldadd,
+                         int64_t add_batch, void* out, int64_t ldo, int64_t out_batch, int M, int N, int K, int act_in, int n_batch, void* stream);
 
 int g3_flash_attn_fwd_bf16(const void* q, int64_t q_row, int64_t q_batch, int64_t q_head, const void* k, int64_t k_row,
                            int64_t k_batch, int64_t k_head, const void* vt, int64_t vt_row, int64_t vt_batch,
@@ -57,6 +60,11 @@
                            const void* k, int64_t k_row, int64_t k_batch, int64_t k_head, const void* vt, int64_t vt_row, int64_t vt_batch,
                            int64_t vt_head, void* o, int64_t o_row, int64_t o_batch, int64_t o_head, int Sq, int Skv, int kv_dense, int B, int H,
                            int head_dim, float softmax_scale, void* stream);
+
+int g3_self_attn_fwd_bf16(const void* q, int64_t q_row, int64_t q_batch, int64_t q_head, const void* q_norm_weight, float q_norm_eps,
+                          const float* rope_cos, const float* rope_sin, const void* k, int64_t k_row, int64_t k_batch, int64_t k_head, const void* vt,
+                          int64_t vt_row, int64_t vt_batch, int64_t vt_head, void* o, int64_t o_row, int64_t o_batch, int64_t o_head, int Sq, int Skv,
+                          int B, int H, int head_dim, float softmax_scale, void* stream);
 
 int g3_flash_attn_fwd_kvseg_bf16(const void* q, int64_t q_row, int64_t q_batch, int64_t q_head, const void* k, int64_t k_row,
                                  int64_t k_batch, int64_t k_head, const void* vt, int64_t vt_row, int64_t vt_batch, int64_t vt_head,
```
